# TrentMahaffey/NeuralStyleTransferV1

Measured on AMD Instinct MI355X. Metric: stylized 1080p frames/sec at 1/2/4/8 MI355X; SSIM vs CPU ref, higher is better.
Workload: dtype bf16; 1 GPU; configs[1]: TransformerNet (Johnson) forward, 1920x1080, batch 8 per GPU, bf16 MFMA / fp32 accumulate, io_preset imagenet_255, uint8 frames in/out resident in HBM; global_batch=8, parallelism=frames round-robin over 1 GPU(s), no data-path collective, ranks_per_gpu=1, step_launch=one HIP-graph replay of the captured forward per step

## Files before the change

include/nst_hip.h:

```cpp
#ifndef NST_HIP_H
#define NST_HIP_H

#include <stddef.h>
#include <stdint.h>

#ifdef __cplusplus
extern "C" {
#endif

#define NST_OK 0
#define NST_E_INVALID (-1)
#define NST_E_PARAM (-2)
#define NST_E_SHAPE (-3)
#define NST_E_HIP (-4)
#define NST_E_WORKSPACE (-5)
#define NST_E_RANGE (-6)

#define NST_ARCH_JOHNSON 0
#define NST_ARCH_NST 1
#define NST_ARCH_RECONET 2
#define NST_ARCH_RECONET_FRN 3
#define NST_ARCH_TORCH7_IN 4
#define NST_ARCH_TORCH7_BN 5

#define NST_DT_F32 0
#define NST_DT_BF16 1
#define NST_DT_F16 2
#define NST_DT_F32S 3
#define NST_DT_F16M 4

#define NST_IO_F32_NCHW 0
#define NST_IO_U8_NHWC 1

#define NST_PRESET_NONE 0
#define NST_PRESET_TANH 1
#define NST_PRESET_IMAGENET_01 2
#define NST_PRESET_IMAGENET_255 3
#define NST_PRESET_CAFFE_BGR 4
#define NST_PRESET_RAW_255 5
#define NST_PRESET_RAW_01 6
#define NST_PRESET_TORCH7 7

typedef struct nst_handle nst_handle;
typedef struct nst_lab nst_lab;

typedef struct nst_param {
  const char* name;
  const float* data;
  int64_t numel;
} nst_param;

const char* nst_last_error(void);

const char* nst_version(void);

int nst_create(int arch, const nst_param* params, int n_params, int compute_dtype, int device,
               nst_handle** out);

#define NST_KSEL_NO_WSTAT 0x1
#define NST_KSEL_NO_WPHASE 0x2
#define NST_KSEL_NO_WS2 0x4
#define NST_KSEL_NO_WS9 0x8
#define NST_KSEL_NO_KYROT 0x10
#define NST_KSEL_NO_PREPAD 0x20
#define NST_KSEL_NO_PERSISTENT 0x40
#define NST_KSEL_UNFUSED_RESIDUAL 0x80
#define NST_KSEL_NO_FOLD 0x100
#define NST_KSEL_F16M_TWO_BLOCKS 0x200
#define NST_KSEL_PAD_DECODER 0x400
#define NST_KSEL_PAD_ENCODER 0x800
#define NST_KSEL_PAD_48 0x1000
#define NST_KSEL_ALL 0x1fff
int nst_create_ex(int arch, const nst_param* params, int n_params, int compute_dtype, int device,
                  unsigned flags, nst_handle** out);
void nst_destroy(nst_handle* h);

int nst_output_hw(const nst_handle* h, int in_h, int in_w, int* out_h, int* out_w);

int nst_input_exact(const nst_handle* h, int x_fmt, int preset, int* exact);

int nst_workspace_bytes(const nst_handle* h, int n, int in_h, int in_w, size_t* out);

int nst_set_stream_split(nst_handle* h, int k);

int nst_forward(nst_handle* h, const void* x, int x_fmt, int n, int in_h, int in_w, int preset,
                void* y, int y_fmt, void* workspace, size_t workspace_bytes, void* stream);

#define NST_BUF_INPUT (-1)
#define NST_BUF_OUTPUT (-2)
typedef struct nst_op_desc {
  int kind;
  int layer;
  int src, dst;
  int in_norm;
  int in_relu;
  int res_buf;
  int res_norm;
  int res_out;
  int relu_out;
  int in_h, in_w;
  int conv_h, conv_w;
  int out_h, out_w;
  int cin_stride, cout_stride;
  int kernel_mode;
  int elem_bytes;
  int in_elem_bytes;
  int res_elem_bytes;
  int kernel_dtype;
} nst_op_desc;
int nst_num_ops(const nst_handle* h);
int nst_set_range_check(nst_handle* h, int enable);
int nst_op_describe(const nst_handle* h, int n, int in_h, int in_w, int op, nst_op_desc* out);
int nst_forward_capture(nst_handle* h, const void* x, int x_fmt, int n, int in_h, int in_w, int preset,
                        void* y, int y_fmt, void* workspace, size_t workspace_bytes, void* const* act,
                        void* const* res, void* const* stats, void* stream);

int nst_decode_resize_u8(const float* y, int n, int h, int w, int preset, uint8_t* out, int out_h,
                         int out_w, void* stream);

int nst_blend_models_u8(const float* const* ys, const int* presets, const float* weights, int m, int n,
                        int h, int w, uint8_t* out, int out_h, int out_w, void* stream);


int nst_lab_create(const uint8_t* rgb2lab, const uint8_t* lab2rgb, int device, nst_lab** out);
void nst_lab_destroy(nst_lab* lab);

int nst_lab_ema_u8(const nst_lab* lab, const uint8_t* rgb_in, uint8_t* rgb_out, int n, int h, int w,
                   int smooth_lightness, float alpha, float one_minus_alpha, int smooth_chroma,
                   float chroma_alpha, float one_minus_chroma_alpha, float* state, int first,
                   void* stream);

int nst_lab_planes_u8(const nst_lab* lab, const uint8_t* rgb_in, int n, int h, int w, int smooth_lightness,
                      int smooth_chroma, uint8_t* planes, void* stream);
int nst_lab_ema_planes(const uint8_t* planes_in, uint8_t* planes_out, int n, int h, int w, int smooth_lightness,
                       float alpha, float one_minus_alpha, int smooth_chroma, float chroma_alpha,
                       float one_minus_chroma_alpha, float* state, int first, void* stream);
int nst_lab_merge_u8(const nst_lab* lab, const uint8_t* rgb_in, const uint8_t* planes, int n, int h, int w,
                     int smooth_lightness, int smooth_chroma, uint8_t* rgb_out, void* stream);

int nst_blend_models_lab_u8(const nst_lab* lab, const uint8_t* const* frames, int m, const float* weights_rest,
                            int n_rest, float w_l, float w_ab, int n, int h, int w, uint8_t* out, void* stream);

int nst_mask_feather(const uint8_t* mask, int n, int h, int w, float sigma, float* scratch, float* alpha,
                     void* stream);

int nst_blend_u8(const uint8_t* styled, const uint8_t* orig, const float* mask, int composite_mode,
                 float blend, float one_minus_blend, uint8_t* out, int n, int h, int w,
                 void* stream);
int nst_blend_mask8_u8(const uint8_t* styled, const uint8_t* orig, const uint8_t* mask, int composite_mode, float blend,
                       float one_minus_blend, uint8_t* out, int n, int h, int w, void* stream);

int nst_profile_begin(nst_handle* h);
int nst_profile_end(nst_handle* h, int n_layers, float* total_ms, int* launches);
int nst_num_layers(const nst_handle* h);
const char* nst_layer_name(const nst_handle* h, int layer);

#define NST_GRAM_CHW 0
#define NST_GRAM_HWC 1
int nst_gram_workspace_bytes(int n, int c, int hw, size_t* out);
int nst_gram(const void* F, int dtype, int layout, int n, int c, int hw, float* G, void* workspace,
             size_t workspace_bytes, void* stream);

typedef struct nst_vgg nst_vgg;
int nst_vgg_create(const nst_param* params, int n_params, int device, nst_vgg** out);
#define NST_VGG_GENERIC_ONLY 0x1
int nst_vgg_create_ex(const nst_param* params, int n_params, int device, unsigned flags, nst_vgg** out);
void nst_vgg_destroy(nst_vgg* v);
int nst_gatys_buffer_bytes(const nst_vgg* v, int h, int w, size_t* workspace, size_t* state);
int nst_vgg_features(nst_vgg* v, const float* image, int h, int w, void* const* feats, void* workspace,
                     size_t workspace_bytes, void* stream);
int nst_gatys_targets(nst_vgg* v, const float* content, const float* style, int h, int w, void* state,
                      void* workspace, size_t workspace_bytes, void* stream);
int nst_gatys_grad(nst_vgg* v, const float* image, int h, int w, const float* style_layer_weights,
                   float content_weight, float style_weight, const void* state, float* grad, float* losses,
                   void* workspace, size_t workspace_bytes, void* stream);
int nst_gatys_grad_capture(nst_vgg* v, const float* image, int h, int w, const float* style_layer_weights,
                           float content_weight, float style_weight, const void* state, float* grad,
                           float* losses, void* workspace, size_t workspace_bytes, void* const* dz,
                           void* stream);
int nst_adam_step(float* x, const float* grad, float* m, float* v, int c, int hw, float lr, float beta1,
                  float beta2, float eps, int step, int clamp01, int grad_is_normalised, void* stream);

#define NST_SEG_RESNET101 0
#define NST_SEG_DRN_D54 1
typedef struct nst_seg nst_seg;
int nst_seg_create(const nst_param* params, int n_params, int num_classes, int compute_dtype, int device,
                   nst_seg** out);
int nst_seg_create_ex(const nst_param* params, int n_params, int num_classes, int compute_dtype, int device,
                      int backbone, nst_seg** out);
void nst_seg_destroy(nst_seg* s);
int nst_seg_num_classes(const nst_seg* s);
int nst_seg_workspace_bytes(const nst_seg* s, int n, int h, int w, size_t* out);
int nst_seg_forward(nst_seg* s, const void* x, int x_fmt, int n, int h, int w, float* logits, uint8_t* pred,
                    void* workspace, size_t workspace_bytes, void* stream);
int nst_seg_mask_scratch_bytes(int n, int h, int w, size_t* out);
int nst_seg_mask(const uint8_t* pred, int n, int h, int w, const int* target_ids, int n_ids, int close_ks,
                 int expand_px, int contract_px, int feather_px, uint8_t* mask, void* scratch, size_t scratch_bytes,
                 void* stream);

#define NST_RESIZE_PIL_LANCZOS 0
#define NST_RESIZE_CV_LINEAR 1
typedef struct nst_resize nst_resize;
int nst_resize_create(int kind, int h, int w, int oh, int ow, int device, nst_resize** out);
void nst_resize_destroy(nst_resize* r);
int nst_resize_scratch_bytes(const nst_resize* r, int n, size_t* out);
int nst_resize_u8(const nst_resize* r, const uint8_t* in, int n, int c, uint8_t* out, void* scratch,
                  size_t scratch_bytes, void* stream);

#define NST_REGION_MAX 32
#define NST_REGION_TERMS 9
#define NST_REGION_MAX_SRC 16
#define NST_RG_RECTS 0
#define NST_RG_DIAGONAL 1
#define NST_RG_VORONOI 2
#define NST_RG_RADIAL 3
#define NST_RG_WAVES 4
#define NST_RG_SPIRAL 5
#define NST_RG_CONCENTRIC 6
int nst_region_masks(int kind, int count, int n_gen, const int* ivals, const double* dvals, const double* lo,
                     const double* hi, const int* rects, const double* points, const double* divisor, int h, int w,
                     float* masks, float* scratch, void* stream);
int nst_region_feather(float* masks, int k, int h, int w, const float* taps, int ks, float* scratch, void* stream);
int nst_region_rotate(const float* in, int k, int h, int w, double angle_deg, float* out, void* stream);
int nst_region_morph_scratch_floats(int k, int h, int w, size_t* out);
int nst_region_morph(const float* in, int k, int h, int w, int mode, double frequency, double time_offset,
                     double max_disp, const double* offsets, float* out, float* scratch, size_t scratch_floats,
                     void* stream);
int nst_region_bbox(const float* masks, int k, int h, int w, float threshold, int* bbox, void* stream);
int nst_region_scratch_floats(int n, int h, int w, int crops, int with_orig, size_t* out);
int nst_region_composite_u8(const float* const* src_y, const int* src_hw, const int* src_preset, int n_src,
                            const int* n_terms, const int* term_src, const float* term_w, int n_regions,
                            const int* boxes, const uint8_t* orig, const float* masks, int n, int h, int w,
                            float* scratch, size_t scratch_floats, uint8_t* out, float* out_f32, void* stream);
int nst_region_crop_input(const uint8_t* frames, int n, int h, int w, const int* box, int out_h, int out_w, float* out,
                          void* stream);
int nst_region_resize(const float* y, int n, int h, int w, int preset, int fit_h, int fit_w, int out_h, int out_w,
                      float* out, void* stream);

int nst_gray_u8(const uint8_t* rgb, int n, int h, int w, uint8_t* gray, void* stream);
int nst_flow_scratch_floats(int h, int w, size_t* out);
int nst_flow_farneback(const uint8_t* prev, const uint8_t* next, int h, int w, double pyr_scale, int levels,
                       int winsize, int iterations, int poly_n, double poly_sigma, float* flow, float* scratch,
                       size_t scratch_floats, void* stream);
int nst_flow_dis_scratch_bytes(int n, int h, int w, size_t* out);
int nst_flow_dis(const uint8_t* prev, const uint8_t* next, int n, int h, int w, float* flow, void* scratch,
                 size_t scratch_bytes, void* stream);
int nst_flow_downscale_gray(const uint8_t* gray, int h, int w, int ds, uint8_t* out, void* stream);
int nst_resize_area_u8(const uint8_t* in, int n, int h, int w, int c, uint8_t* out, int out_h, int out_w, void* stream);
int nst_flow_upscale(const float* flow_small, int hs, int ws, int h, int w, float mul, float* flow, void* stream);
int nst_flow_fuse(const float* curr, const float* prev, const float* flow, int h, int w, float alpha,
                  float one_minus_alpha, float* out, void* stream);
int nst_motion_alpha(const float* flow, int h, int w, float motion_norm, double sigma, float max_alpha, float span,
                     float* alpha, float* scratch, void* stream);

int nst_png_bound(int h, int w, int c, size_t* out_stride);
int nst_png_workspace_bytes(int n, int h, int w, int c, size_t* out);
int nst_png_encode_u8(const uint8_t* frames, int n, int h, int w, int c, uint8_t* out, size_t out_stride,
                      int64_t* sizes, void* workspace, size_t workspace_bytes, void* stream);

#define NST_E_DATA (-7)
#define NST_JPEG_444 0
// ... 18 lines not shown
```

neuralstyletransferv1_amd/_lib.py:

```python
from __future__ import annotations

import ctypes
import os
import threading

import torch

_HERE = os.path.dirname(os.path.abspath(__file__))
LIB_PATH = os.environ.get("NST_HIP_LIB", os.path.join(_HERE, "libnst_hip.so"))

NST_OK = 0
NST_ARCH_JOHNSON, NST_ARCH_NST, NST_ARCH_RECONET, NST_ARCH_RECONET_FRN = 0, 1, 2, 3
NST_ARCH_TORCH7_IN, NST_ARCH_TORCH7_BN = 4, 5
NST_DT_F32, NST_DT_BF16, NST_DT_F16, NST_DT_F32S, NST_DT_F16M = 0, 1, 2, 3, 4
NST_KDT_SW_O32, NST_KDT_SW_O16, NST_KDT_SPLIT_O32, NST_KDT_SPLIT_O16, NST_KDT_SPLITO_O32 = 16, 17, 18, 19, 20
NST_VGG_GENERIC_ONLY = 0x1
NST_IO_F32_NCHW, NST_IO_U8_NHWC = 0, 1
NST_SEG_RESNET101, NST_SEG_DRN_D54 = 0, 1
PRESETS = {
    "none": 0,
    "tanh": 1,
    "imagenet_01": 2,
    "imagenet_255": 3,
    "caffe_bgr": 4,
    "raw_255": 5,
    "raw_01": 6,
}
NST_PRESET_TORCH7 = 7

EXPORTED_SYMBOLS = (
    "nst_last_error", "nst_version", "nst_create", "nst_destroy", "nst_output_hw",
    "nst_workspace_bytes", "nst_forward", "nst_decode_resize_u8", "nst_lab_create",
    "nst_lab_destroy", "nst_lab_ema_u8", "nst_blend_u8", "nst_gram", "nst_profile_begin",
    "nst_profile_end", "nst_num_layers", "nst_layer_name", "nst_blend_models_u8", "nst_blend_models_lab_u8",
    "nst_mask_feather", "nst_create_ex", "nst_num_ops", "nst_op_describe", "nst_forward_capture",
    "nst_gram_workspace_bytes", "nst_vgg_create", "nst_vgg_create_ex", "nst_vgg_destroy", "nst_gatys_buffer_bytes", "nst_vgg_features",
    "nst_gatys_targets", "nst_gatys_grad", "nst_adam_step", "nst_gatys_grad_capture",
    "nst_seg_create", "nst_seg_create_ex", "nst_seg_destroy", "nst_seg_num_classes", "nst_seg_workspace_bytes", "nst_seg_forward",
    "nst_seg_mask_scratch_bytes", "nst_seg_mask", "nst_resize_create", "nst_resize_destroy",
    "nst_resize_scratch_bytes", "nst_resize_u8", "nst_blend_mask8_u8",
    "nst_region_masks", "nst_region_feather", "nst_region_rotate", "nst_region_bbox", "nst_region_scratch_floats",
    "nst_region_composite_u8", "nst_region_crop_input", "nst_region_resize", "nst_region_morph",
    "nst_region_morph_scratch_floats", "nst_gray_u8", "nst_flow_scratch_floats", "nst_flow_farneback",
    "nst_flow_fuse", "nst_motion_alpha", "nst_flow_downscale_gray", "nst_flow_upscale", "nst_resize_area_u8",
    "nst_flow_dis_scratch_bytes", "nst_flow_dis", "nst_set_range_check", "nst_input_exact", "nst_set_stream_split",
    "nst_lab_planes_u8", "nst_lab_ema_planes", "nst_lab_merge_u8",
    "nst_png_bound", "nst_png_workspace_bytes", "nst_png_encode_u8",
    "nst_jpeg_probe", "nst_jpeg_entropy_decode", "nst_jpeg_workspace_bytes", "nst_jpeg_reconstruct_u8",
    "nst_jpeg_enc_bound", "nst_jpeg_enc_workspace_bytes", "nst_jpeg_encode_u8",
)
NST_E_INVALID, NST_E_SHAPE, NST_E_WORKSPACE, NST_E_DATA = -1, -3, -5, -7
NST_JPEG_444, NST_JPEG_422, NST_JPEG_420 = 0, 1, 2
NST_REGION_MAX, NST_REGION_TERMS, NST_REGION_MAX_SRC = 32, 9, 16
RG_KINDS = {"rects": 0, "diagonal": 1, "voronoi": 2, "radial": 3, "waves": 4, "spiral": 5, "concentric": 6}
NST_GRAM_CHW, NST_GRAM_HWC = 0, 1

KSEL = {
    "no_wstat": 0x1, "no_wphase": 0x2, "no_ws2": 0x4, "no_ws9": 0x8, "no_kyrot": 0x10, "no_prepad": 0x20,
    "no_persistent": 0x40, "unfused_residual": 0x80, "no_fold": 0x100, "f16m_two_blocks": 0x200,
    "pad_decoder": 0x400, "pad_encoder": 0x800, "pad_48": 0x1000,
}
NST_BUF_INPUT, NST_BUF_OUTPUT = -1, -2


class NstParam(ctypes.Structure):
    _fields_ = [("name", ctypes.c_char_p), ("data", ctypes.POINTER(ctypes.c_float)), ("numel", ctypes.c_int64)]


class NstOpDesc(ctypes.Structure):
    _fields_ = [(n, ctypes.c_int) for n in (
        "kind", "layer", "src", "dst", "in_norm", "in_relu", "res_buf", "res_norm", "res_out", "relu_out",
        "in_h", "in_w", "conv_h", "conv_w", "out_h", "out_w", "cin_stride", "cout_stride", "kernel_mode",
        "elem_bytes", "in_elem_bytes", "res_elem_bytes", "kernel_dtype")]

    def as_dict(self):
        return {n: getattr(self, n) for n, _ in self._fields_}


_lib = None
_lock = threading.Lock()


class NstError(RuntimeError):
    """Raised for any non-zero status from libnst_hip (message from nst_last_error)."""


TRUNK_KERNEL_SOURCES = ("csrc/conv_wst16.hip", "csrc/conv_ws_common.h", "csrc/conv_impl.h")


def kernel_sha(sources=TRUNK_KERNEL_SOURCES, obj: str = "conv_wstat") -> str:
    import hashlib
    import re
    h = hashlib.sha256()
    for rel in sources:
        with open(os.path.join(_HERE, rel), "rb") as f:
            h.update(f.read())
    pat = r"(HIPCC|ARCH|SLP|CXXFLAGS) |\$\(BUILD\)/" + re.escape(obj) + r"\.hip\.o: *(CXXFLAGS|SLP) "
    with open(os.path.join(_HERE, "..", "Makefile")) as f:
        h.update("".join(l for l in f if re.match(pat, l)).encode())
    return h.hexdigest()[:16]


def trunk_kernel_sha() -> str:
    return kernel_sha(TRUNK_KERNEL_SOURCES, "conv_wst16")


WS2_KERNEL_SOURCES = ("csrc/conv_ws2.hip", "csrc/conv_ws_common.h", "csrc/conv_impl.h")


def ws2_kernel_sha() -> str:
    return kernel_sha(WS2_KERNEL_SOURCES, "conv_ws2")


def lib() -> ctypes.CDLL:
    global _lib
    if _lib is not None:
        return _lib
    with _lock:
        if _lib is not None:
            return _lib
        if not os.path.exists(LIB_PATH):
            raise NstError(
                f"libnst_hip.so not found at {LIB_PATH}: build it with `make` (or __graft_entry__.build()); "
                "there is no CPU fallback")
        L = ctypes.CDLL(LIB_PATH)
        vp, i, f, sz = ctypes.c_void_p, ctypes.c_int, ctypes.c_float, ctypes.c_size_t
        L.nst_last_error.restype = ctypes.c_char_p
        L.nst_version.restype = ctypes.c_char_p
        L.nst_create.argtypes = [i, ctypes.POINTER(NstParam), i, i, i, ctypes.POINTER(vp)]
        L.nst_create_ex.argtypes = [i, ctypes.POINTER(NstParam), i, i, i, ctypes.c_uint, ctypes.POINTER(vp)]
        L.nst_num_ops.argtypes = [vp]
        L.nst_num_ops.restype = i
        L.nst_set_range_check.argtypes = [vp, i]
        L.nst_set_range_check.restype = i
        L.nst_set_stream_split.argtypes = [vp, i]
        L.nst_set_stream_split.restype = i
        L.nst_op_describe.argtypes = [vp, i, i, i, i, ctypes.POINTER(NstOpDesc)]
        L.nst_forward_capture.argtypes = [vp, vp, i, i, i, i, i, vp, i, vp, sz, ctypes.POINTER(vp), ctypes.POINTER(vp),
                                          ctypes.POINTER(vp), vp]
        L.nst_vgg_create.argtypes = [ctypes.POINTER(NstParam), i, i, ctypes.POINTER(vp)]
        L.nst_vgg_create_ex.argtypes = [ctypes.POINTER(NstParam), i, i, ctypes.c_uint, ctypes.POINTER(vp)]
        L.nst_vgg_destroy.argtypes = [vp]
        L.nst_vgg_destroy.restype = None
        L.nst_gatys_buffer_bytes.argtypes = [vp, i, i, ctypes.POINTER(sz), ctypes.POINTER(sz)]
        L.nst_vgg_features.argtypes = [vp, vp, i, i, ctypes.POINTER(vp), vp, sz, vp]
        L.nst_gatys_targets.argtypes = [vp, vp, vp, i, i, vp, vp, sz, vp]
        L.nst_gatys_grad.argtypes = [vp, vp, i, i, ctypes.POINTER(f), f, f, vp, vp, vp, vp, sz, vp]
        L.nst_gatys_grad_capture.argtypes = [vp, vp, i, i, ctypes.POINTER(f), f, f, vp, vp, vp, vp, sz,
                                             ctypes.POINTER(vp), vp]
        L.nst_gatys_grad_capture.restype = i
        L.nst_adam_step.argtypes = [vp, vp, vp, vp, i, i, f, f, f, f, i, i, i, vp]
        L.nst_destroy.argtypes = [vp]
        L.nst_destroy.restype = None
        L.nst_seg_create.argtypes = [ctypes.POINTER(NstParam), i, i, i, i, ctypes.POINTER(vp)]
        L.nst_seg_create_ex.argtypes = [ctypes.POINTER(NstParam), i, i, i, i, i, ctypes.POINTER(vp)]
        L.nst_seg_destroy.argtypes = [vp]
        L.nst_seg_destroy.restype = None
        L.nst_seg_num_classes.argtypes = [vp]
        L.nst_seg_workspace_bytes.argtypes = [vp, i, i, i, ctypes.POINTER(sz)]
        L.nst_seg_forward.argtypes = [vp, vp, i, i, i, i, vp, vp, vp, sz, vp]
        L.nst_seg_mask_scratch_bytes.argtypes = [i, i, i, ctypes.POINTER(sz)]
        L.nst_seg_mask.argtypes = [vp, i, i, i, ctypes.POINTER(i), i, i, i, i, i, vp, vp, sz, vp]
        L.nst_resize_create.argtypes = [i, i, i, i, i, i, ctypes.POINTER(vp)]
        L.nst_resize_destroy.argtypes = [vp]
        L.nst_resize_destroy.restype = None
        L.nst_resize_scratch_bytes.argtypes = [vp, i, ctypes.POINTER(sz)]
        L.nst_resize_u8.argtypes = [vp, vp, i, i, vp, vp, sz, vp]
        pi, pd, pf = ctypes.POINTER(i), ctypes.POINTER(ctypes.c_double), ctypes.POINTER(f)
        L.nst_region_masks.argtypes = [i, i, i, pi, pd, pd, pd, pi, pd, pd, i, i, vp, vp, vp]
        L.nst_region_feather.argtypes = [vp, i, i, i, pf, i, vp, vp]
        L.nst_region_rotate.argtypes = [vp, i, i, i, ctypes.c_double, vp, vp]
        L.nst_region_bbox.argtypes = [vp, i, i, i, f, vp, vp]
        dbl = ctypes.c_double
        L.nst_region_morph_scratch_floats.argtypes = [i, i, i, ctypes.POINTER(sz)]
        L.nst_region_morph.argtypes = [vp, i, i, i, i, dbl, dbl, dbl, pd, vp, vp, sz, vp]
        L.nst_region_scratch_floats.argtypes = [i, i, i, i, i, ctypes.POINTER(sz)]
        L.nst_region_composite_u8.argtypes = [ctypes.POINTER(vp), pi, pi, i, pi, pi, pf, i, pi, vp, vp, i, i, i, vp,
                                              sz, vp, vp, vp]
        L.nst_region_crop_input.argtypes = [vp, i, i, i, pi, i, i, vp, vp]
        L.nst_region_resize.argtypes = [vp, i, i, i, i, i, i, i, i, vp, vp]
        L.nst_gray_u8.argtypes = [vp, i, i, i, vp, vp]
        L.nst_flow_scratch_floats.argtypes = [i, i, ctypes.POINTER(sz)]
        L.nst_flow_farneback.argtypes = [vp, vp, i, i, dbl, i, i, i, i, dbl, vp, vp, sz, vp]
        L.nst_flow_fuse.argtypes = [vp, vp, vp, i, i, f, f, vp, vp]
        L.nst_motion_alpha.argtypes = [vp, i, i, f, dbl, f, f, vp, vp, vp]
        L.nst_flow_downscale_gray.argtypes = [vp, i, i, i, vp, vp]
        L.nst_flow_upscale.argtypes = [vp, i, i, i, i, f, vp, vp]
        L.nst_resize_area_u8.argtypes = [vp, i, i, i, i, vp, i, i, vp]
        L.nst_flow_dis_scratch_bytes.argtypes = [i, i, i, ctypes.POINTER(sz)]
        L.nst_flow_dis.argtypes = [vp, vp, i, i, i, vp, vp, sz, vp]
        for name in ("nst_gray_u8", "nst_flow_scratch_floats", "nst_flow_farneback", "nst_flow_fuse",
                     "nst_motion_alpha", "nst_flow_downscale_gray", "nst_flow_upscale", "nst_resize_area_u8",
                     "nst_flow_dis_scratch_bytes", "nst_flow_dis"):
            getattr(L, name).restype = i
        for name in ("nst_region_masks", "nst_region_feather", "nst_region_rotate", "nst_region_bbox",
                     "nst_region_morph", "nst_region_morph_scratch_floats",
                     "nst_region_scratch_floats", "nst_region_composite_u8", "nst_region_crop_input",
                     "nst_region_resize"):
            getattr(L, name).restype = i
        L.nst_output_hw.argtypes = [vp, i, i, ctypes.POINTER(i), ctypes.POINTER(i)]
        L.nst_workspace_bytes.argtypes = [vp, i, i, i, ctypes.POINTER(sz)]
        L.nst_forward.argtypes = [vp, vp, i, i, i, i, i, vp, i, vp, sz, vp]
        L.nst_decode_resize_u8.argtypes = [vp, i, i, i, i, vp, i, i, vp]
        L.nst_lab_create.argtypes = [vp, vp, i, ctypes.POINTER(vp)]
        L.nst_lab_destroy.argtypes = [vp]
        L.nst_lab_destroy.restype = None
        L.nst_lab_ema_u8.argtypes = [vp, vp, vp, i, i, i, i, f, f, i, f, f, vp, i, vp]
        L.nst_lab_planes_u8.argtypes = [vp, vp, i, i, i, i, i, vp, vp]
        L.nst_lab_ema_planes.argtypes = [vp, vp, i, i, i, i, f, f, i, f, f, vp, i, vp]
        L.nst_lab_merge_u8.argtypes = [vp, vp, vp, i, i, i, i, i, vp, vp]
        L.nst_input_exact.argtypes = [vp, i, i, ctypes.POINTER(i)]
        L.nst_png_bound.argtypes = [i, i, i, ctypes.POINTER(sz)]
        L.nst_png_workspace_bytes.argtypes = [i, i, i, i, ctypes.POINTER(sz)]
        L.nst_png_encode_u8.argtypes = [vp, i, i, i, i, vp, sz, vp, vp, sz, vp]
        psz = ctypes.POINTER(sz)
        L.nst_jpeg_probe.argtypes = [vp, sz, pi, pi, pi, pi, psz]
        L.nst_jpeg_entropy_decode.argtypes = [vp, sz, vp, sz]
        L.nst_jpeg_workspace_bytes.argtypes = [i, i, i, i, i, psz]
        L.nst_jpeg_reconstruct_u8.argtypes = [vp, sz, i, i, i, i, i, vp, vp, sz, vp]
        L.nst_jpeg_enc_bound.argtypes = [i, i, psz]
        L.nst_jpeg_enc_workspace_bytes.argtypes = [i, i, i, psz]
        L.nst_jpeg_encode_u8.argtypes = [vp, i, i, i, i, vp, sz, vp, vp, sz, vp]
        for name in ("nst_jpeg_probe", "nst_jpeg_entropy_decode", "nst_jpeg_workspace_bytes",
                     "nst_jpeg_reconstruct_u8", "nst_jpeg_enc_bound", "nst_jpeg_enc_workspace_bytes",
                     "nst_jpeg_encode_u8"):
            getattr(L, name).restype = i
# ... 46 lines not shown
```

neuralstyletransferv1_amd/csrc/conv_ws_common.h:

```cpp
#pragma once
#include "conv_impl.h"

namespace nst {

typedef unsigned int u32x2_t __attribute__((ext_vector_type(2)));
typedef unsigned int u32x4_t __attribute__((ext_vector_type(4)));

__device__ __forceinline__ f32x4_t add4(const f32x4_t& a, const f32x4_t& b) {
  f32x4_t r;
#pragma unroll
  for (int i = 0; i < 4; ++i) r[i] = a[i] + b[i];
  return r;
}
__device__ __forceinline__ void stat4(f32x4_t& s1, f32x4_t& s2, const f32x4_t& x) {
#pragma unroll
  for (int i = 0; i < 4; ++i) {
    s1[i] = s1[i] + x[i];
    s2[i] = __builtin_fmaf(x[i], x[i], s2[i]);
  }
}

template <typename T>
__device__ __forceinline__ void mfma_tied(f32x4_t& c, const uint4& a, const uint4& bop, bool first) {
  const u32x4_t av = __builtin_bit_cast(u32x4_t, a), bv = __builtin_bit_cast(u32x4_t, bop);
  if constexpr (IS_F16<T>) {
    if (first)
      asm volatile("v_mfma_f32_16x16x32_f16 %0, %1, %2, 0" : "=&v"(c) : "v"(av), "v"(bv));
    else
      asm volatile("v_mfma_f32_16x16x32_f16 %0, %1, %2, %0" : "+v"(c) : "v"(av), "v"(bv));
  } else {
    if (first)
      asm volatile("v_mfma_f32_16x16x32_bf16 %0, %1, %2, 0" : "=&v"(c) : "v"(av), "v"(bv));
    else
      asm volatile("v_mfma_f32_16x16x32_bf16 %0, %1, %2, %0" : "+v"(c) : "v"(av), "v"(bv));
  }
}

template <typename T>
__device__ __forceinline__ void mfma16x16x16_tied(f32x4_t& c, const uint2& a, const uint2& bop) {
  const u32x2_t av = __builtin_bit_cast(u32x2_t, a), bv = __builtin_bit_cast(u32x2_t, bop);
  if constexpr (IS_F16<T>)
    asm volatile("v_mfma_f32_16x16x16_f16 %0, %1, %2, %0" : "+v"(c) : "v"(av), "v"(bv));
  else
    asm volatile("v_mfma_f32_16x16x16_bf16 %0, %1, %2, %0" : "+v"(c) : "v"(av), "v"(bv));
}

template <typename T>
__device__ __forceinline__ void mfma_tied_c(f32x4_t& c, const uint4& a, const uint4& bop, bool first, const f32x4_t& cinit) {
  const u32x4_t av = __builtin_bit_cast(u32x4_t, a), bv = __builtin_bit_cast(u32x4_t, bop);
  if constexpr (IS_F16<T>) {
    if (first)
      asm volatile("v_mfma_f32_16x16x32_f16 %0, %1, %2, %3" : "=&v"(c) : "v"(av), "v"(bv), "v"(cinit));
    else
      asm volatile("v_mfma_f32_16x16x32_f16 %0, %1, %2, %0" : "+v"(c) : "v"(av), "v"(bv));
  } else {
    if (first)
      asm volatile("v_mfma_f32_16x16x32_bf16 %0, %1, %2, %3" : "=&v"(c) : "v"(av), "v"(bv), "v"(cinit));
    else
      asm volatile("v_mfma_f32_16x16x32_bf16 %0, %1, %2, %0" : "+v"(c) : "v"(av), "v"(bv));
  }
}

constexpr int ST_AUX = 2;

enum WsFill { WF_NORM = 0, WF_RAW = 1, WF_RES = 2, WF_RESRN = 3 };

template <int N>
__device__ __forceinline__ void vm_wait() {
  asm volatile("s_waitcnt vmcnt(%0)" ::"n"(N) : "memory");
}
__device__ __forceinline__ void lds_barrier() {
  asm volatile("s_waitcnt lgkmcnt(0)\n\ts_barrier" ::: "memory");
}

__device__ __forceinline__ void dma16(const __amdgpu_buffer_rsrc_t& rs, uint32_t voff, uint32_t lds, int soff) {
  uint32_t keep;
  asm volatile(
      "s_mov_b32 %0, m0\n\ts_mov_b32 m0, %2\n\ts_nop 0\n\tbuffer_load_dwordx4 %1, %3, %4 offen lds\n\ts_mov_b32 m0, %0"
      : "=&s"(keep)
      : "v"(voff), "s"(lds), "s"(rs), "s"(soff)
      : "memory");
}

}
```

neuralstyletransferv1_amd/csrc/conv_wst16.hip:

```cpp
#include <algorithm>
#include <cstdlib>
#include <cstring>

#include "conv_ws_common.h"

namespace nst {

constexpr uint32_t OOB = 0xFFFFFF00u;
#ifndef NST_W32_ST
#define NST_W32_ST 0
#endif

#ifndef NST_WST32_STAMP
#define NST_WST32_STAMP 0
#endif
#ifndef NST_W32_MIN
#define NST_W32_MIN 0
#endif
#if NST_WST32_STAMP
constexpr int STAMP_IT = 1, STAMP_PT = 16;
__device__ long long g_w16_stamp[256 * 4 * STAMP_IT * STAMP_PT];
#endif

template <int TH, int FILL>
struct W16Cfg {
  static constexpr bool RES = FILL == WF_RES;
  static constexpr int NW = 4, NT = 256;
  static constexpr int TW = 32;
  static constexpr int CINP = 128;
  static constexpr int LH = TH + 2, LW = TW + 2;
  static constexpr int NENT = LH * LW;
  static constexpr int EB = 288;
  static constexpr int NKS = 72;
  static constexpr int NA = 64;
  static constexpr int NV = NKS - NA;
  static constexpr int NIT = (NENT + 63) / 64;
  static constexpr int LASTN = NENT - 64 * (NIT - 1);
  static constexpr int NFMAX = RES ? 8 : 16;
  static constexpr int DPU = RES ? 2 : 1;
  static constexpr int SLOTB = DPU * 1024;
  static constexpr int MAPB = ((LH + LW) * 4 + 15) / 16 * 16;
  static constexpr int MAP_OFF = NENT * EB;
  static constexpr int NORM_OFF = MAP_OFF + 2 * MAPB;
  static constexpr int NORM_TAB = NFMAX * CINP * 8;
  static constexpr int BIAS_OFF = NORM_OFF + NORM_TAB;
  static constexpr int DUMMY_OFF = BIAS_OFF + CINP * 4;
  static constexpr int STG_OFF = DUMMY_OFF + 64 * 16;
  static constexpr int LDS = STG_OFF + NIT * NW * SLOTB;
  static constexpr int SST = TH * TW * 4 / NT;
  static constexpr int EPI = 2 * TH + 1;
  static_assert(LDS <= 160 * 1024, "LDS budget");
  static_assert(TH * TW * 4 % NT == 0 && TW == 32, "pixel-quarter stores");
};

template <typename T>
__device__ __forceinline__ void mfma16_a(f32x4_t& c, const u32x4_t& a, const u32x4_t& b, bool first) {
  if constexpr (IS_F16<T>) {
    if (first) asm volatile("v_mfma_f32_16x16x32_f16 %0, %1, %2, 0" : "=&v"(c) : "a"(a), "v"(b));
    else asm volatile("v_mfma_f32_16x16x32_f16 %0, %1, %2, %0" : "+v"(c) : "a"(a), "v"(b));
  } else {
    if (first) asm volatile("v_mfma_f32_16x16x32_bf16 %0, %1, %2, 0" : "=&v"(c) : "a"(a), "v"(b));
    else asm volatile("v_mfma_f32_16x16x32_bf16 %0, %1, %2, %0" : "+v"(c) : "a"(a), "v"(b));
  }
}
template <typename T>
__device__ __forceinline__ void mfma16_v(f32x4_t& c, const u32x4_t& a, const u32x4_t& b, bool first) {
  if constexpr (IS_F16<T>) {
    if (first) asm volatile("v_mfma_f32_16x16x32_f16 %0, %1, %2, 0" : "=&v"(c) : "v"(a), "v"(b));
    else asm volatile("v_mfma_f32_16x16x32_f16 %0, %1, %2, %0" : "+v"(c) : "v"(a), "v"(b));
  } else {
    if (first) asm volatile("v_mfma_f32_16x16x32_bf16 %0, %1, %2, 0" : "=&v"(c) : "v"(a), "v"(b));
    else asm volatile("v_mfma_f32_16x16x32_bf16 %0, %1, %2, %0" : "+v"(c) : "v"(a), "v"(b));
  }
}

template <typename T, int TH, int FILL, bool ZPAD, bool XO>
__global__ __launch_bounds__(256) void wst16_kernel(ConvParams p) {
  using C = W16Cfg<TH, FILL>;
  constexpr bool RES = C::RES;
  static_assert(!XO || FILL == WF_NORM, "x_0 export is a normalising fill");
  constexpr bool SOUT = RES || XO;
  __shared__ __attribute__((aligned(16))) char smem[C::LDS];
  const int tid = threadIdx.x, lane = tid & 63;
  const int wv = __builtin_amdgcn_readfirstlane(tid >> 6);
  const int g4 = lane >> 4, p16 = lane & 15;

  struct Work {
    int n, tile, ty0, tx0;
  };
  const int ntile = p.tiles_x * p.tiles_y;
  const int nfr = p.n_work / ntile;
  auto decode = [&](int wi) {
    Work r;
    r.n = wi / ntile;
    r.tile = wi - r.n * ntile;
    const int ty = r.tile / p.tiles_x;
    r.ty0 = ty * TH;
    r.tx0 = (r.tile - ty * p.tiles_x) * C::TW;
    return r;
  };
  const int G = (int)gridDim.x, b = (int)blockIdx.x;
  const int w0 = (G % 8 == 0) ? (b % 8) * (G / 8) + b / 8 : b;
  if (w0 >= p.n_work) return;

  u32x4_t wa[C::NA];
  u32x4_t wvr[C::NV];
  {
    const u32x4_t* wsrc = (const u32x4_t*)p.wpk + (size_t)wv * C::NKS * 64 + lane;
#pragma unroll
    for (int s = 0; s < C::NA; ++s) asm volatile("global_load_dwordx4 %0, %1, off" : "=a"(wa[s]) : "v"(wsrc + s * 64) : "memory");
#pragma unroll
    for (int s = 0; s < C::NV; ++s) wvr[s] = wsrc[(C::NA + s) * 64];
  }
  float* norm_y = (float*)(smem + C::NORM_OFF);
  if (FILL != WF_RAW) {
    for (int t = tid; t < nfr * C::CINP; t += C::NT) {
      const int f = t / C::CINP, c = t - f * C::CINP;
      const int o = (f * 16 + (c >> 3)) * 16 + 4 * ((c & 7) >> 1) + (c & 1);
      const float2 v = p.in_norm[(size_t)f * p.cs + c];
      norm_y[o] = v.x;
      norm_y[o + 2] = v.y;
    }
  }
  if (tid < C::CINP) ((float*)(smem + C::BIAS_OFF))[tid] = p.bias[tid];

  const uint32_t fb = (uint32_t)p.hs * p.ws * p.cs * 2;
  const uint32_t ob = (uint32_t)p.oh * p.ow * p.cout_stride * 2;
  auto launch_rsrc = [&](const void* base, uint32_t frame) {
    return __builtin_amdgcn_make_buffer_rsrc((void*)base, (short)0, (int)(frame * (uint32_t)nfr), 0x00020000);
  };
  auto build_maps = [&](const Work& wk, int slot) {
    int* rowmap = (int*)(smem + C::MAP_OFF + slot * C::MAPB);
    int* colmap = rowmap + C::LH;
    const int vy0 = wk.ty0 - p.pad, vx0 = wk.tx0 - p.pad;
    const int pix = p.cs * 2;
    auto axis = [&](int v, int L) { return ZPAD ? map_axis(v, L, p.axis_mode, p.pre) : reflect_idx(v, L); };
    static_assert(C::LH + C::LW <= 64, "one wave builds the maps");
    const int t = tid;
    if (t < C::LH) {
      const int sy = axis(vy0 + t, p.hs);
      rowmap[t] = sy < 0 ? -1 : sy * p.ws * pix;
    } else if (t < C::LH + C::LW) {
      const int sx = axis(vx0 + t - C::LH, p.ws);
      colmap[t - C::LH] = sx < 0 ? -1 : sx * pix;
    }
  };
  constexpr int IT_STRIDE = 64;
  auto item_entry = [&](int k) { return 64 * k + lane; };
  auto item_chunk = [&](int R) { return 4 * R + wv; };
  struct Src {
    uint32_t voff[C::NIT];
    uint32_t pad;
  };
  auto sources = [&](const Work& wk, int slot) {
    const int* rowmap = (const int*)(smem + C::MAP_OFF + slot * C::MAPB);
    const int* colmap = rowmap + C::LH;
    Src s;
    s.pad = 0;
#pragma unroll
    for (int k = 0; k < C::NIT; ++k) {
      const int e0 = item_entry(k);
      const bool valid = k < C::NIT - 1 || lane < C::LASTN;
      const int e = valid ? e0 : 0;
      const int ly = e / C::LW, lx = e - ly * C::LW;
      const int ro = rowmap[ly], co = colmap[lx];
      const bool in = valid && ro >= 0 && co >= 0;
      s.voff[k] = in ? (uint32_t)(ro + co) + (uint32_t)wk.n * fb : OOB;
      if (valid && !in) s.pad |= 1u << k;
    }
    return s;
  };
  const uint32_t stg = (uint32_t)(uintptr_t)(smem + C::STG_OFF) + wv * C::SLOTB;
  const __amdgpu_buffer_rsrc_t rs_in = launch_rsrc(p.in, fb);
  const __amdgpu_buffer_rsrc_t rs_r = launch_rsrc(RES ? p.res_r : p.in, fb);
  auto request = [&](int k, int R, uint32_t voff) {
    const uint32_t lds = stg + k * C::NW * C::SLOTB;
    const int soff = (4 * R + wv) * 16;
    dma16(rs_in, voff, lds, soff);
    if constexpr (RES) dma16(rs_r, voff, lds + 1024, soff);
  };
  struct Staged {
    uint4 y, r;
  };
  auto stage_read = [&](int k) {
    const char* sp = smem + C::STG_OFF + (k * C::NW + wv) * C::SLOTB + lane * 16;
    Staged st;
    st.y = *(const uint4*)sp;
    st.r = RES ? *(const uint4*)(sp + 1024) : make_uint4(0u, 0u, 0u, 0u);
    return st;
  };
  auto consume = [&](int n, int k, int R, uint32_t padbits, const Staged& st) {
    const int ch = item_chunk(R);
    const uint4 y = st.y, rr = st.r;
    const float4* ny = (const float4*)(norm_y + (n * 16 + ch) * 16);
    const uint32_t w[4] = {y.x, y.y, y.z, y.w};
    uint32_t o[4];
    if constexpr (RES) {
      const uint32_t w2[4] = {rr.x, rr.y, rr.z, rr.w};
#pragma unroll
      for (int j = 0; j < 4; ++j) {
        const float4 nn = ny[j];
        const float a = lo16<T>(w[j]) * nn.x + nn.z;
        const float bb = hi16<T>(w[j]) * nn.y + nn.w;
        o[j] = pack16<T>(lo16<T>(w2[j]) + a, hi16<T>(w2[j]) + bb);
      }
    } else if constexpr (FILL == WF_RAW) {
#pragma unroll
      for (int j = 0; j < 4; ++j) o[j] = w[j];
    } else {
#pragma unroll
      for (int j = 0; j < 4; ++j) {
        const float4 nn = ny[j];
        const float a = __builtin_fmaf(lo16<T>(w[j]), nn.x, nn.z);
        const float bb = __builtin_fmaf(hi16<T>(w[j]), nn.y, nn.w);
        const i16x2_t r = __builtin_bit_cast(i16x2_t, pack16<T>(a, bb));
        o[j] = __builtin_bit_cast(uint32_t, __builtin_elementwise_max(r, (i16x2_t){0, 0}));
      }
    }
    const bool pad = ZPAD && ((padbits >> k) & 1u);
    const u32x4_t v = {pad ? 0u : o[0], pad ? 0u : o[1], pad ? 0u : o[2], pad ? 0u : o[3]};
    const bool valid = k < C::NIT - 1 || lane < C::LASTN;
    int eb = item_entry(0) * C::EB + ch * 16;
    asm volatile("" : "+v"(eb));
    *(u32x4_t*)(smem + (valid ? eb + k * IT_STRIDE * C::EB : C::DUMMY_OFF + lane * 16)) = v;
  };
  constexpr int KIN = (C::NIT - 1) * C::DPU + (SOUT ? C::SST : 0);
  constexpr int KEP = KIN + C::EPI;

  typedef f32x4_t Acc[TH][2][2];
  const int lbase = p16 * C::EB + g4 * 16;
  constexpr int NRD = 2 * C::LH;
  constexpr int PRD = 3 * NRD;
  auto bread = [&](int i) -> u32x4_t {
    const int q = i / PRD, rem = i - q * PRD;
    const int dx = rem / NRD, y = (rem % NRD) >> 1, hx = rem & 1;
    return *(const u32x4_t*)(smem + lbase + (y * C::LW + dx + 16 * hx) * C::EB + 4 * q * 16);
  };
  auto kloop = [&](Acc& acc, auto&& filler, auto&& bound) {
    constexpr int NI = 4 * PRD, D = SOUT ? 2 : 3;
    u32x4_t ring[D];
#pragma unroll
    for (int i = 0; i < D; ++i) ring[i] = bread(i);
    int slot = 0;
#pragma unroll
    for (int i = 0; i < NI; ++i) {
      const int q = i / PRD, rem = i - q * PRD;
      const int dx = rem / NRD, y = (rem % NRD) >> 1, hx = rem & 1;
      if (rem == 0) slot = 0;
      const u32x4_t bcur = ring[i % D];
      if (i + D < NI) ring[i % D] = bread(i + D);
#pragma unroll
      for (int dy = 0; dy < 3; ++dy) {
        const int r = y - dy;
        if (r < 0 || r >= TH) continue;
#pragma unroll
        for (int bb = 0; bb < 2; ++bb) {
          const int s = 2 * (q * 9 + 3 * dy + dx) + bb;
          const bool first = q == 0 && dx == 0 && dy == 0;
          if (s < C::NA) mfma16_a<T>(acc[r][bb][hx], wa[s], bcur, first);
          else mfma16_v<T>(acc[r][bb][hx], wvr[s - C::NA], bcur, first);
          filler(q, slot);
          ++slot;
          __builtin_amdgcn_sched_barrier(0);
        }
      }
      if (rem == PRD - 1) {
        lds_barrier();
        bound(q);
      }
      __builtin_amdgcn_sched_barrier(0);
    }
  };

  const float* biasl = (const float*)(smem + C::BIAS_OFF) + 32 * wv + 4 * g4;
  auto epilogue = [&](const Work& wk, Acc& acc) {
    asm volatile("s_nop 7\n\ts_nop 7\n\ts_nop 7" ::: "memory");
    const __amdgpu_buffer_rsrc_t ors = launch_rsrc(p.out, ob);
    const uint32_t row_bytes = (uint32_t)p.ow * p.cout_stride * 2;
    const int spx = wk.tx0 + ((g4 & 1) ? 16 : 0) + p16;
    const uint32_t soff = (uint32_t)wk.n * ob + (uint32_t)(((wk.ty0 * p.ow + spx) * p.cout_stride + 32 * wv + 8 * (g4 >> 1)) * 2);
    const bool sok = spx < p.ow;
    const bool ok0 = wk.tx0 + p16 < p.ow, ok1 = wk.tx0 + 16 + p16 < p.ow;
    const f32x4_t bias0 = *(const f32x4_t*)(biasl), bias1 = *(const f32x4_t*)(biasl + 16);
    f32x4_t s1[2], s2[2];
    auto rows = [&](auto all_valid) {
#pragma unroll
      for (int r = 0; r < TH; ++r) {
        const bool rv = decltype(all_valid)::value || wk.ty0 + r < p.oh;
#pragma unroll
        for (int bb = 0; bb < 2; ++bb) {
          const f32x4_t v0 = acc[r][bb][0] + (bb ? bias1 : bias0), v1 = acc[r][bb][1] + (bb ? bias1 : bias0);
          const auto sx = __builtin_amdgcn_permlane16_swap(pack16<T>(v0[0], v0[1]), pack16<T>(v1[0], v1[1]), false, false);
          const auto sy = __builtin_amdgcn_permlane16_swap(pack16<T>(v0[2], v0[3]), pack16<T>(v1[2], v1[3]), false, false);
          const u32x4_t pk = {sx[0], sy[0], sx[1], sy[1]};
          __builtin_amdgcn_raw_buffer_store_b128(pk, ors, (rv && sok) ? soff + r * row_bytes + 32 * bb : OOB, 0, NST_W32_ST);
          const f32x4_t x0 = (decltype(all_valid)::value || (rv && ok0)) ? v0 : (f32x4_t){0.f, 0.f, 0.f, 0.f};
          const f32x4_t x1 = (decltype(all_valid)::value || (rv && ok1)) ? v1 : (f32x4_t){0.f, 0.f, 0.f, 0.f};
          if (r == 0) {
            s1[bb] = x0 + x1;
            s2[bb] = __builtin_elementwise_fma(x1, x1, x0 * x0);
          } else {
            s1[bb] = (s1[bb] + x0) + x1;
            s2[bb] = __builtin_elementwise_fma(x1, x1, __builtin_elementwise_fma(x0, x0, s2[bb]));
          }
        }
      }
    };
    if (wk.ty0 + TH <= p.oh && wk.tx0 + C::TW <= p.ow) rows(std::true_type{});
    else rows(std::false_type{});
    const float v[16] = {s1[0][0], s2[0][0], s1[0][1], s2[0][1], s1[0][2], s2[0][2], s1[0][3], s2[0][3],
                         s1[1][0], s2[1][0], s1[1][1], s2[1][1], s1[1][2], s2[1][2], s1[1][3], s2[1][3]};
    float a8[8], a4[4], a2[2], a1[1];
    rs_step<8, 0x140>(v, a8, p16 >= 8);
    rs_step<4, 0x141>(a8, a4, (p16 & 4) != 0);
    rs_step<2, 0x1b>(a4, a2, (p16 & 2) != 0);
    rs_step<1, 0xb1>(a2, a1, (p16 & 1) != 0);
    const int idx = (p16 >= 8 ? 8 : 0) + ((p16 & 4) ? 4 : 0) + ((p16 & 2) ? 2 : 0) + (p16 & 1);
    const int co = 32 * wv + 16 * (idx >> 3) + 4 * g4 + ((idx >> 1) & 3);
    const __amdgpu_buffer_rsrc_t prs = __builtin_amdgcn_make_buffer_rsrc(
        (void*)(p.partial + ((size_t)wk.n * ntile + wk.tile) * p.cout_stride * 2), (short)0, p.cout_stride * 8, 0x00020000);
    __builtin_amdgcn_raw_buffer_store_b32(__float_as_uint(a1[0]), prs, (uint32_t)((co * 2 + (idx & 1)) * 4), 0, 0);
  };

  Work cur = decode(w0);
  int wn = w0 + G;
  const int last = p.n_work - 1;
  build_maps(cur, 0);
  build_maps(decode(min(wn, last)), 1);
  asm volatile("s_waitcnt vmcnt(0)" ::: "memory");
  __syncthreads();
  uint32_t pad3;
  {
    const Src s0 = sources(cur, 0);
    pad3 = s0.pad;
#pragma unroll
    for (int k = 0; k < C::NIT; ++k) request(k, 0, s0.voff[k]);
#pragma unroll
    for (int R = 0; R < 3; ++R) {
      vm_wait<0>();
#pragma unroll
      for (int k = 0; k < C::NIT; ++k) {
        consume(cur.n, k, R, s0.pad, stage_read(k));
        request(k, R + 1, s0.voff[k]);
      }
    }
  }
  vm_wait<0>();
  __syncthreads();
  constexpr int SLOTS_PER_ITEM = 48;
  static_assert(SLOTS_PER_ITEM * C::NIT <= 9 * TH * 4 && C::SST <= C::NIT, "micro-step slots");
  Acc acc;
  Staged sy;
  float4 n0;
  float tl, th;
  uint32_t o4[4];
  int mro = 0, mco = 0;
  bool padk = false;
  bool mok = false;
  uint32_t rvoff = OOB;
  u32x4_t sv;
#if NST_WST32_STAMP
  unsigned st_acc[7] = {0, 0, 0, 0, 0, 0, 0};
  unsigned st_prev = (unsigned)__builtin_amdgcn_s_memtime();
#endif
  auto stamp = [&](int it, int pt) {
#if NST_WST32_STAMP
    const unsigned t = (unsigned)__builtin_amdgcn_s_memtime();
    st_acc[pt == 0 ? 5 : pt - 1] += t - st_prev;
    st_prev = t;
    if (pt == 0) st_acc[6] += 1;
#endif
  };
  for (int it = 0;; ++it) {
    stamp(it, 0);
    const bool more = wn < p.n_work;
    const Work nxt = more ? decode(wn) : cur;
    const Work nxt2 = decode(min(wn + G, last));
    const int cs = it & 1, ns = cs ^ 1;
    kloop(
        acc,
        [&](int q, int slot) {
          const int k = slot / SLOTS_PER_ITEM, o = slot - k * SLOTS_PER_ITEM;
          if (k >= C::NIT) return;
          const int R = q == 0 ? 3 : q - 1;
          const int n = q == 0 ? cur.n : nxt.n;
          const int ch = item_chunk(R);
          const float4* ny = (const float4*)(norm_y + (n * 16 + ch) * 16);
          auto pair_step = [&](int j, int st) {
            const uint32_t wy = j == 0 ? sy.y.x : j == 1 ? sy.y.y : j == 2 ? sy.y.z : sy.y.w;
            if constexpr (RES) {
              const uint32_t wr = j == 0 ? sy.r.x : j == 1 ? sy.r.y : j == 2 ? sy.r.z : sy.r.w;
              if (st == 0) tl = lo16<T>(wy) * n0.x;
              else if (st == 1) tl = lo16<T>(wr) + (tl + n0.z);
              else if (st == 2) th = hi16<T>(wy) * n0.y;
              else o4[j] = pack16<T>(tl, hi16<T>(wr) + (th + n0.w));
            } else if constexpr (FILL == WF_RAW) {
              if (st == 3) o4[j] = wy;
            } else {
              if (st == 0) tl = __builtin_fmaf(lo16<T>(wy), n0.x, n0.z);
              else if (st == 1) th = __builtin_fmaf(hi16<T>(wy), n0.y, n0.w);
              else if (st == 3) {
                const i16x2_t r = __builtin_bit_cast(i16x2_t, pack16<T>(tl, th));
                o4[j] = __builtin_bit_cast(uint32_t, __builtin_elementwise_max(r, (i16x2_t){0, 0}));
              }
            }
          };
          if (o == 0) {
            if (q == 0) vm_wait<KEP>(); else vm_wait<KIN>();
            sy = stage_read(k);
          } else if (o >= 4 && o < 36 && (o - 4) % 8 == 0) {
            if (FILL != WF_RAW) n0 = ny[(o - 4) / 8];
          } else if (o >= 8 && o < 36 && (o - 4) % 8 >= 4) {
            pair_step((o - 4) / 8, (o - 4) % 8 - 4);
          } else if (o == 2) {
            const int* rowmap = (const int*)(smem + C::MAP_OFF + ns * C::MAPB);
            const bool valid = k < C::NIT - 1 || lane < C::LASTN;
            const int e = valid ? item_entry(k) : 0;
            const int ly = e / C::LW, lx = e - ly * C::LW;
            mro = rowmap[ly];
            mco = rowmap[C::LH + lx];
          } else if (o == 36) {
            const bool valid = k < C::NIT - 1 || lane < C::LASTN;
            mok = valid && mro >= 0 && mco >= 0;
            if (ZPAD) {
              padk = valid && !mok;
              if (q == 3) pad3 = (pad3 & ~(1u << k)) | (padk ? 1u << k : 0u);
            }
          } else if (o == 37) {
            rvoff = mok ? (uint32_t)(mro + mco) + (uint32_t)nxt.n * fb : OOB;
          } else if (o == 38) {
            const bool pad = ZPAD && (q == 0 ? ((pad3 >> k) & 1u) != 0 : padk);
            const u32x4_t v = {pad ? 0u : o4[0], pad ? 0u : o4[1], pad ? 0u : o4[2], pad ? 0u : o4[3]};
            const bool valid = k < C::NIT - 1 || lane < C::LASTN;
            int eb = item_entry(0) * C::EB + ch * 16;
            asm volatile("" : "+v"(eb));
            *(u32x4_t*)(smem + (valid ? eb + k * IT_STRIDE * C::EB : C::DUMMY_OFF + lane * 16)) = v;
          } else if (o == 40) {
            request(k, q, rvoff);
          }
          if (q == 1 && k == 0 && o == 44) build_maps(nxt2, cs);
          if (SOUT && k < C::SST && o == 42) {
            const int cl = lane >> 4, x16 = ((lane & 15) - cl) & 15;
            const int P = 16 * (C::SST * wv + k) + x16;
            sv = *(const u32x4_t*)(smem + (((P >> 5) + 1) * C::LW + (P & 31) + 1) * C::EB + (4 * q + cl) * 16);
          }
          if (SOUT && k < C::SST && o == 47) {
            const int cl = lane >> 4, x16 = ((lane & 15) - cl) & 15;
            const int P = 16 * (C::SST * wv + k) + x16;
            const int c = 4 * q + cl, oy = cur.ty0 + (P >> 5), ox = cur.tx0 + (P & 31);
            const bool ok = oy < p.oh && ox < p.ow;
            __builtin_amdgcn_raw_buffer_store_b128(sv, launch_rsrc(p.res_out, fb),
                                                   ok ? (uint32_t)cur.n * fb + (uint32_t)(((oy * p.ws + ox) * p.cs + c * 8) * 2) : OOB,
                                                   0, NST_W32_ST);
          }
        },
        [&](int q) { stamp(it, 1 + q); });
    epilogue(cur, acc);
    stamp(it, 5);
    if (!more) break;
    cur = nxt;
    wn += G;
  }
  vm_wait<0>();
#if NST_WST32_STAMP
  if (lane == 0 && b < 256)
    for (int i = 0; i < 7; ++i) g_w16_stamp[(b * 4 + wv) * STAMP_PT + i] = st_acc[i];
#endif
}

template <typename T, int TH, bool RES>
struct Wst16Inst {
  using C = W16Cfg<TH, RES ? WF_RES : WF_NORM>;
  static int cus() {
    static const int v = [] {
      int dev = 0, c = 0;
      if (hipGetDevice(&dev) != hipSuccess || hipDeviceGetAttribute(&c, hipDeviceAttributeMultiprocessorCount, dev) != hipSuccess)
        c = 256;
      return c;
    }();
    return v;
  }
  template <int FILL, bool ZPAD, bool XO = false>
  static void go(const ConvParams& p, int nb, hipStream_t st) {
    hipLaunchKernelGGL((wst16_kernel<T, TH, FILL, ZPAD, XO>), dim3(nb), dim3(C::NT), 0, st, p);
  }
  static void launch(const ConvParams& p0, dim3 grid, hipStream_t st) {
    const int ntile = (int)grid.x, n = (int)grid.y;
    const size_t fin = (size_t)p0.hs * p0.ws * p0.cs * 2, fout = (size_t)p0.oh * p0.ow * p0.cout_stride * 2;
    const int fmax = (int)std::min<size_t>(C::NFMAX, (size_t)OOB / std::max(fin, fout));
    if (fmax < 1) return;
    for (int f0 = 0; f0 < n; f0 += fmax) {
      const int nf = std::min(fmax, n - f0);
      ConvParams p = p0;
      p.in = (const char*)p0.in + f0 * fin;
      p.out = (char*)p0.out + f0 * fout;
      if (p0.res_r) p.res_r = (const char*)p0.res_r + f0 * fin;
      if (p0.res_out) p.res_out = (char*)p0.res_out + f0 * fin;
      if (p0.in_norm) p.in_norm = p0.in_norm + (size_t)f0 * p0.cs;
      p.partial = p0.partial + (size_t)f0 * ntile * p0.cout_stride * 2;
      p.n_work = nf * ntile;
      const int nb = std::min(p.n_work, cus());
      const bool zp = p.axis_mode != AX_REFLECT;
#if NST_W32_MIN
      if (zp) return;
      if constexpr (RES) go<WF_RES, false>(p, nb, st);
      else if (p.res_out != nullptr) go<WF_NORM, false, true>(p, nb, st);
      else go<WF_NORM, false>(p, nb, st);
#else
      if constexpr (RES) {
        zp ? go<WF_RES, true>(p, nb, st) : go<WF_RES, false>(p, nb, st);
      } else {
        if (p.in_norm != nullptr && p.res_out != nullptr)
          zp ? go<WF_NORM, true, true>(p, nb, st) : go<WF_NORM, false, true>(p, nb, st);
        else if (p.in_norm != nullptr)
          zp ? go<WF_NORM, true>(p, nb, st) : go<WF_NORM, false>(p, nb, st);
        else
          zp ? go<WF_RAW, true>(p, nb, st) : go<WF_RAW, false>(p, nb, st);
      }
#endif
    }
  }
  static ConvKernelInfo info() {
    ConvKernelInfo k;
    std::memset(&k, 0, sizeof(k));
    k.dtype = dtype_code<T>();
    k.mode = MODE_WSTAT;
    k.ks = 3; k.stride = 1; k.cinp = C::CINP; k.bn = 128; k.th = TH; k.tw = C::TW; k.wm = C::NW; k.wn = 2;
    k.in_kind = IN_ACT; k.out_kind = OUT_ACT;
    k.cpc = 8; k.nch = 16; k.lds_bytes = C::LDS;
    k.wbytes = C::NW * C::NKS * 1024;
    k.persistent = 1;
    k.part_rows = 1;
    k.res = RES ? 1 : 0;
    k.launch = &launch;
    return k;
  }
};

#ifndef NST_WST16_TH
#define NST_WST16_TH 8
#endif
#ifndef NST_W16_PART
#define NST_W16_PART -1
#endif
#define W16_KERNELS(X, T)                                                                                     \
  X(T, WF_NORM, false, false) X(T, WF_NORM, false, true) X(T, WF_NORM, true, false) X(T, WF_NORM, true, true) \
  X(T, WF_RAW, false, false) X(T, WF_RAW, true, false) X(T, WF_RES, false, false) X(T, WF_RES, true, false)
#define W16_EXTERN(T, F, Z, X_) extern template __global__ void wst16_kernel<T, NST_WST16_TH, F, Z, X_>(ConvParams);
#define W16_INST(T, F, Z, X_) template __global__ void wst16_kernel<T, NST_WST16_TH, F, Z, X_>(ConvParams);
#if NST_W16_PART >= 0 && NST_W16_PART < 8
#define W16_T_ __bf16
#if NST_W16_PART >= 4
#undef W16_T_
#define W16_T_ _Float16
#endif
#if NST_W16_PART % 4 == 0
W16_INST(W16_T_, WF_NORM, false, false)
W16_INST(W16_T_, WF_NORM, false, true)
#elif NST_W16_PART % 4 == 1
W16_INST(W16_T_, WF_NORM, true, false)
W16_INST(W16_T_, WF_NORM, true, true)
#elif NST_W16_PART % 4 == 2
W16_INST(W16_T_, WF_RAW, false, false)
W16_INST(W16_T_, WF_RAW, true, false)
#else
W16_INST(W16_T_, WF_RES, false, false)
W16_INST(W16_T_, WF_RES, true, false)
#endif
#else
#if NST_W16_PART == 8
W16_KERNELS(W16_EXTERN, __bf16)
W16_KERNELS(W16_EXTERN, _Float16)
#endif
const ConvKernelInfo* conv_table_wst16(int* count) {
  static const ConvKernelInfo table[] = {
      Wst16Inst<__bf16, NST_WST16_TH, false>::info(),
      Wst16Inst<__bf16, NST_WST16_TH, true>::info(),
#if !NST_W32_MIN
      Wst16Inst<_Float16, NST_WST16_TH, false>::info(),
      Wst16Inst<_Float16, NST_WST16_TH, true>::info(),
#endif
  };
  const char* env = std::getenv("NST_WST16");
  *count = (env != nullptr && env[0] == '0') ? 0 : (int)(sizeof(table) / sizeof(table[0]));
  return table;
}
#endif

}

#if NST_WST32_STAMP
extern "C" int nst_debug_w16_stamps(long long* host, int n) {
  const int cap = 256 * 4 * nst::STAMP_IT * nst::STAMP_PT;
  if (n > cap) n = cap;
  return hipMemcpyFromSymbol(host, HIP_SYMBOL(nst::g_w16_stamp), (size_t)n * 8, 0, hipMemcpyDeviceToHost) == hipSuccess ? n : -1;
}
#endif
```

neuralstyletransferv1_amd/csrc/nst_api.cpp:

```cpp
#include <hip/hip_runtime.h>

#include <cmath>
#include <cstdio>
#include <algorithm>
#include <cstring>
#include <cstdlib>
#include <map>
#include <string>
#include <vector>

#include "nst_hip.h"
#include "nst_internal.h"
#include "post_common.h"

namespace nst {

static thread_local std::string g_last_error;
void set_error(const std::string& msg) { g_last_error = msg; }

const ConvKernelInfo* conv_table_bf16(int* count);
const ConvKernelInfo* conv_table_f16(int* count);
const ConvKernelInfo* conv_table_bf16_wl(int* count);
const ConvKernelInfo* conv_table_f32(int* count);
const ConvKernelInfo* conv_table_f32s(int* count);
// ... 79 lines not shown
  int shave = 0;
};

static int round_up(int v, int a) { return (v + a - 1) / a * a; }
static bool is_reconet(int arch) { return arch == NST_ARCH_RECONET || arch == NST_ARCH_RECONET_FRN; }
static bool is_torch7(int arch) { return arch == NST_ARCH_TORCH7_IN || arch == NST_ARCH_TORCH7_BN; }

static void build_program(int arch, bool fuse_res, bool x0_export, std::vector<LayerDef>& L, std::vector<Op>& P,
                          int split_blocks = 0) {
  L.clear();
  P.clear();
  auto conv = [&](int layer, int src, int dst, int in_norm) {
    P.push_back(Op{OP_CONV, layer, src, dst, in_norm, 0, 0, 0, 0});
  };
  auto convres = [&](int layer, int y, int y_norm, int r_buf, int r_norm, int res_out, int relu_out, int dst) {
    Op o{OP_CONV, layer, y, dst, y_norm, r_buf, r_norm, r_norm >= 0 ? 1 : 0, relu_out};
    o.res_buf = r_buf;
    o.res_out = res_out;
    P.push_back(o);
  };
  auto resadd = [&](int layer, int y, int dst, int r_buf, int r_norm, int relu_out) {
    P.push_back(Op{OP_RESADD, layer, y, dst, -1, r_buf, r_norm, r_norm >= 0 ? 1 : 0, relu_out});
  };
  if (arch == NST_ARCH_JOHNSON) {
    L.push_back({"conv1.conv2d", "in1", 3, 32, 9, 1, AX_REFLECT, 4, 0, false});
    L.push_back({"conv2.conv2d", "in2", 32, 64, 3, 2, AX_REFLECT, 1, 0, false});
    L.push_back({"conv3.conv2d", "in3", 64, 128, 3, 2, AX_REFLECT, 1, 0, false});
    for (int r = 1; r <= 5; ++r) {
      const std::string p = "res" + std::to_string(r);
      L.push_back({p + ".conv1.conv2d", p + ".in1", 128, 128, 3, 1, AX_REFLECT, 1, 0, false});
      L.push_back({p + ".conv2.conv2d", p + ".in2", 128, 128, 3, 1, AX_REFLECT, 1, 0, false});
    }
    L.push_back({"deconv1.conv2d", "in4", 128, 64, 3, 1, AX_REFLECT_UP2, 1, 0, false});
    L.push_back({"deconv2.conv2d", "in5", 64, 32, 3, 1, AX_REFLECT_UP2, 1, 0, false});
    L.push_back({"deconv3.conv2d", "", 32, 3, 9, 1, AX_REFLECT, 4, 0, false});
  } else if (arch == NST_ARCH_NST) {
    L.push_back({"down1.conv", "down1.norm", 3, 32, 9, 1, AX_ZERO_PREREFLECT, 4, 40, false});
    L.push_back({"down2.conv", "down2.norm", 32, 64, 3, 2, AX_ZERO, 1, 0, false});
    L.push_back({"down3.conv", "down3.norm", 64, 128, 3, 2, AX_ZERO, 1, 0, false});
    for (int r = 1; r <= 5; ++r) {
      const std::string p = "res" + std::to_string(r);
      L.push_back({p + ".conv1", p + ".norm1", 128, 128, 3, 1, AX_ZERO, 1, 0, false});
      L.push_back({p + ".conv2", p + ".norm2", 128, 128, 3, 1, AX_ZERO, 1, 0, false});
    }
    L.push_back({"up1.conv", "up1.norm", 128, 64, 3, 1, AX_ZINSERT, 1, 0, true});
    L.push_back({"up2.conv", "up2.norm", 64, 32, 3, 1, AX_ZINSERT, 1, 0, true});
    L.push_back({"final", "", 32, 3, 9, 1, AX_ZERO, 4, 0, false});
  } else if (is_torch7(arch)) {
    L.push_back({"down1.conv", "down1.norm", 3, 32, 9, 1, AX_ZERO_PREREFLECT, 4, 40, false});
    L.push_back({"down2.conv", "down2.norm", 32, 64, 3, 2, AX_ZERO, 1, 0, false});
    L.push_back({"down3.conv", "down3.norm", 64, 128, 3, 2, AX_ZERO, 1, 0, false});
    for (int r = 1; r <= 5; ++r) {
      const std::string p = "res" + std::to_string(r);
      L.push_back({p + ".conv1", p + ".norm1", 128, 128, 3, 1, AX_ZERO, 0, 0, false});
      L.push_back({p + ".conv2", p + ".norm2", 128, 128, 3, 1, AX_ZERO, 0, 0, false});
    }
    L.push_back({"up1.conv", "up1.norm", 128, 64, 3, 1, AX_ZINSERT, 1, 0, true});
    L.push_back({"up2.conv", "up2.norm", 64, 32, 3, 1, AX_ZINSERT, 1, 0, true});
    L.push_back({"final", "", 32, 3, 9, 1, AX_ZERO, 4, 0, false});
  } else {
    L.push_back({"encoder.layers.0.layers.0.layers.1", "encoder.layers.0.layers.1", 3, 48, 9, 1, AX_REFLECT, 4, 0, false});
    L.push_back({"encoder.layers.1.layers.0.layers.1", "encoder.layers.1.layers.1", 48, 96, 3, 2, AX_REFLECT, 1, 0, false});
    L.push_back({"encoder.layers.2.layers.0.layers.1", "encoder.layers.2.layers.1", 96, 192, 3, 2, AX_REFLECT, 1, 0, false});
    for (int r = 3; r <= 6; ++r) {
      const std::string p = "encoder.layers." + std::to_string(r) + ".branch.";
      L.push_back({p + "0.layers.0.layers.1", p + "0.layers.1", 192, 192, 3, 1, AX_REFLECT, 1, 0, false});
      L.push_back({p + "1.layers.0.layers.1", p + "1.layers.1", 192, 192, 3, 1, AX_REFLECT, 1, 0, false});
    }
    L.push_back({"decoder.layers.1.layers.0.layers.1", "decoder.layers.1.layers.1", 192, 96, 3, 1, AX_REFLECT_UP2, 1, 0, false});
    L.push_back({"decoder.layers.3.layers.0.layers.1", "decoder.layers.3.layers.1", 96, 48, 3, 1, AX_REFLECT_UP2, 1, 0, false});
    L.push_back({"decoder.layers.4.layers.0.layers.1", "", 48, 3, 9, 1, AX_REFLECT, 4, 0, false});
  }
  const int nres = is_reconet(arch) ? 4 : 5;
  const int relu_out = is_reconet(arch) ? 1 : 0;
  const int u1 = 3 + 2 * nres, u2 = u1 + 1, fin = u1 + 2;
  conv(0, B_IMG, B_A, -1);
  conv(1, B_A, B_B, 0);
  conv(2, B_B, B_C, 1);
  if (is_torch7(arch)) {
    int xbuf = B_C, xnorm = 2;
    for (int r = 0; r < nres; ++r) {
      const int l1 = 3 + 2 * r, l2 = 4 + 2 * r;
      conv(l1, xbuf, B_D, xnorm);
      conv(l2, B_D, B_E, l1);
      const int xout = (r & 1) ? B_G : B_F;
      resadd(l2, B_E, xout, xbuf, xnorm, 0);
      P.back().shave = 2;
      xbuf = xout;
      xnorm = -1;
    }
    conv(u1, xbuf, B_A, -1);
  } else if (split_blocks > 0) {
    conv(3, B_C, B_D, 2);
    conv(4, B_D, B_E, 3);
    if (split_blocks >= 2) {
      resadd(4, B_E, B_F, B_C, 2, relu_out);
      P.back().out_esz = 4;
      conv(5, B_F, B_D, -1);
      conv(6, B_D, B_E, 5);
      resadd(6, B_E, B_G, B_F, -1, relu_out);
    } else {
      resadd(4, B_E, B_G, B_C, 2, relu_out);
    }
    P.back().out_esz = 2;
    int xbuf = B_G;
    for (int r = split_blocks; r < nres; ++r) {
      const int l1 = 3 + 2 * r, l2 = 4 + 2 * r;
      if (r == split_blocks) {
        conv(l1, B_G, B_D, -1);
      } else {
        const int xout = xbuf == B_F ? B_G : B_F;
        convres(l1, B_E, l2 - 2, xbuf, -1, xout, relu_out, B_D);
        xbuf = xout;
      }
      conv(l2, B_D, B_E, l1);
    }
    convres(u1, B_E, u1 - 1, xbuf, -1, -1, relu_out, B_A);
  } else if (!fuse_res) {
    for (int r = 0; r < nres; ++r) {
      const int l1 = 3 + 2 * r, l2 = 4 + 2 * r;
      conv(l1, B_C, B_D, r == 0 ? 2 : -1);
      conv(l2, B_D, B_E, l1);
      resadd(l2, B_E, B_C, B_C, r == 0 ? 2 : -1, relu_out);
    }
    conv(u1, B_C, B_A, -1);
  } else {
    int xbuf = x0_export ? B_F : B_C, xnorm = x0_export ? -1 : 2;
    for (int r = 0; r < nres; ++r) {
      const int l1 = 3 + 2 * r, l2 = 4 + 2 * r;
      if (r == 0) {
        conv(l1, B_C, B_D, 2);
        if (x0_export) P.back().res_out = B_F;
      } else {
        const int xout = ((r & 1) != 0) != x0_export ? B_F : B_G;
        convres(l1, B_E, l2 - 2, xbuf, xnorm, xout, relu_out, B_D);
        xbuf = xout;
        xnorm = -1;
      }
      conv(l2, B_D, B_E, l1);
    }
    convres(u1, B_E, u1 - 1, xbuf, xnorm, -1, relu_out, B_A);
  }
  conv(u2, B_A, B_B, u1);
  conv(fin, B_B, B_OUT, u2);
}

}

using namespace nst;

struct nst_handle {
  int arch, dtype, device;
  int* range_flag = nullptr;
  std::vector<Layer> layers;
  std::vector<Op> prog;
  bool profiling = false;
  struct Rec { int layer; hipEvent_t a, b; };
  std::vector<Rec> recs;
  int split = 1;
  float t7_mul = 0.f;
  hipStream_t sub[NST_MAX_STREAM_SPLIT] = {};
  hipEvent_t fork = nullptr, join[NST_MAX_STREAM_SPLIT] = {};
};

struct nst_lab {
  int device;
  uint32_t* rgb2lab = nullptr;
  uint32_t* lab2rgb = nullptr;
};

namespace {


int upload_weights(int dtype, const std::vector<float>& pk, void** dst);

int phase_taps(bool convT, int a, int t, int* ks_out) {
  if (convT) {
    if (a == 0) { if (t == 0) { ks_out[0] = 1; return 1; } return 0; }
    ks_out[0] = t == 0 ? 2 : 0;
    return 1;
  }
  if (a == 0) {
    if (t == 0) { ks_out[0] = 0; return 1; }
    ks_out[0] = 1; ks_out[1] = 2; return 2;
  }
  if (t == 0) { ks_out[0] = 0; ks_out[1] = 1; return 2; }
  ks_out[0] = 2;
  return 1;
}

double phase_weight(const LayerDef& d, const float* W, int co, int ci, int ph, int tap) {
  int ky[2], kx[2];
  const int ny = phase_taps(d.convT, ph >> 1, tap >> 1, ky), nx = phase_taps(d.convT, ph & 1, tap & 1, kx);
  double sum = 0.0;
  for (int yy = 0; yy < ny; ++yy)
    for (int xx = 0; xx < nx; ++xx)
      sum += d.convT ? (double)W[(((size_t)ci * d.cout + co) * d.ks + ky[yy]) * d.ks + kx[xx]]
                     : (double)W[(((size_t)co * d.cin + ci) * d.ks + ky[yy]) * d.ks + kx[xx]];
  return sum;
}

std::vector<float> pack_weights(const ConvKernelInfo& k, const LayerDef& d, const float* W, int coutp,
                                bool reverse_channels = false) {
  const int ncblk = coutp / k.bn;
  const size_t per_frag = 64 * (size_t)k.cpc;
  std::vector<float> out((size_t)ncblk * k.nstep_pack * k.nsubt * per_frag, 0.f);
  auto w_at = [&](int co, int ci, int dy, int dx) -> double {
    if (d.convT)
      return W[(((size_t)ci * d.cout + co) * d.ks + (d.ks - 1 - dy)) * d.ks + (d.ks - 1 - dx)];
    return W[(((size_t)co * d.cin + ci) * d.ks + dy) * d.ks + dx];
  };
  for (int cb = 0; cb < ncblk; ++cb)
    for (int s = 0; s < k.nstep; ++s)
      for (int tg = 0; tg < k.nsubt; ++tg)
        for (int lane = 0; lane < 64; ++lane) {
          const int q = lane & 15, g = lane >> 4;
          const int taps = k.nchunk / k.nch;
          const int sl = k.korder ? (s % taps) * (k.nch / 4) + s / taps : s;
          const int i = 4 * sl + g;
          float* dst = &out[((((size_t)cb * k.nstep_pack + s) * k.nsubt + tg) * 64 + lane) * k.cpc];
          if (i >= k.nchunk) continue;
          const int tap = i / k.nch, c = i % k.nch;
          if (k.mode == MODE_PHASE) {
            const int ph = tg / k.nsub, t = tg % k.nsub;
            const int co = cb * k.bn + 4 * k.nsub * (q >> 2) + 4 * t + (q & 3);
            if (co >= d.cout) continue;
            for (int j = 0; j < k.cpc; ++j) {
              const int ci = c * k.cpc + j;
              if (ci < d.cin) dst[j] = (float)phase_weight(d, W, co, ci, ph, tap);
            }
          } else if (k.mode == MODE_XSHIFT) {
            if (q >= 15) continue;
            const int sft = q / 3, ch = q % 3;
            const int co = reverse_channels ? 2 - ch : ch;
            const int dy = tap / k.kp, u = tap % k.kp, dx = u - sft;
            if (dx < 0 || dx >= d.ks || co >= d.cout) continue;
            for (int j = 0; j < k.cpc; ++j) {
              const int ci = c * k.cpc + j;
              if (ci < d.cin) dst[j] = (float)w_at(co, ci, dy, dx);
            }
          } else {
            const int wn = tg / k.nsub, t = tg % k.nsub;
            const int co = cb * k.bn + wn * k.nsub * 16 + 4 * k.nsub * (q >> 2) + 4 * t + (q & 3);
            if (co >= d.cout) continue;
            const int dy = tap / k.kp, dxp = tap % k.kp;
            for (int j = 0; j < k.cpc; ++j) {
              int dx, ci;
              if (k.pair) { dx = 2 * dxp + (j >= 4 ? 1 : 0); ci = j & 3; }
              else { dx = dxp; ci = c * k.cpc + j; }
              if (dx < d.ks && ci < d.cin) dst[j] = (float)w_at(co, ci, dy, dx);
            }
          }
        }
  return out;
}

std::vector<float> split_weight_frags(const ConvKernelInfo& k, const std::vector<float>& pk) {
  std::vector<float> out(pk.size() * 2);
  size_t o = 0;
  auto put = [&](const float* f, size_t n, bool lo) {
    for (size_t i = 0; i < n; ++i) {
      const float hi = f16_to_f32(f32_to_f16_rne(f[i]));
      out[o++] = lo ? f[i] - hi : hi;
    }
  };
  if (k.mode == MODE_WS9) {
    const size_t fm = 64 * 8, fk = 64 * 4;
    const float* k8 = pk.data() + 18 * fm;
    for (int mh = 0; mh < 2; ++mh) {
      for (int ky = 0; ky < 9; ++ky)
        for (int hl = 0; hl < 2; ++hl) put(pk.data() + (2 * ky + mh) * fm, fm, hl == 1);
      for (int j = 0; j < 3; ++j)
        for (int hl = 0; hl < 2; ++hl) put(k8 + (2 * j + mh) * fk, fk, hl == 1);
    }
  } else {
    const size_t per_cg = pk.size() / (k.bn / 16);
    for (int cg = 0; cg < k.bn / 16; ++cg)
      for (int hl = 0; hl < 2; ++hl) put(pk.data() + cg * per_cg, per_cg, hl == 1);
  }
  return out;
}

std::vector<float> pack_kyrot_weights(const ConvKernelInfo& k, const LayerDef& d, const float* W) {
  const bool split = k.dtype == NST_DT_F32S;
  const int cpb = split ? 8 : 16, kc_n = (k.cinp_k ? k.cinp_k : k.cinp) / cpb, nblk = 9 * kc_n;
  std::vector<float> out((size_t)k.wbytes / 2, 0.f);
  for (int pp = 0; pp < 2; ++pp)
    for (int ky = 0; ky < 9; ++ky)
      for (int kx = 0; kx < 9; ++kx)
        for (int kc = 0; kc < kc_n; ++kc)
          for (int hh = 0; hh < 2; ++hh)
            for (int c = 0; c < 3; ++c)
              for (int j = 0; j < 4; ++j) {
                const int ci = split ? kc * 8 + 4 * hh + j : kc * 16 + 8 * hh + 4 * pp + j;
                if (ci >= d.cin) continue;
                const size_t row = (((size_t)pp * nblk + kx * kc_n + kc) * 2 + hh) * 27 + 3 * ky + c;
                const float w = W[(((size_t)c * d.cin + ci) * d.ks + ky) * d.ks + kx];
                const float hi = f16_to_f32(f32_to_f16_rne(w));
                out[row * 4 + j] = split ? (pp == 0 ? hi : w - hi) : w;
              }
  return out;
}

std::vector<float> pack_wstat_weights(const LayerDef& d, const float* W) {
  std::vector<float> out((size_t)8 * 36 * 64 * 8, 0.f);
  for (int w = 0; w < 8; ++w)
// ... 48 lines not shown
  std::vector<float> out((size_t)8 * nstep * ns * 64 * 8, 0.f);
  for (int w = 0; w < 8; ++w)
    for (int s = 0; s < nstep; ++s)
      for (int t = 0; t < ns; ++t)
        for (int l = 0; l < 64; ++l) {
          const int q = s / 4, tap = s % 4;
          const int co = (w >> 2) * (bn / 2) + 16 * t + (l & 15);
          for (int i = 0; i < 8; ++i) {
            const int ci = 32 * q + 8 * (l >> 4) + i;
            if (co < d.cout && ci < d.cin)
              out[((((size_t)w * nstep + s) * ns + t) * 64 + l) * 8 + i] = (float)phase_weight(d, W, co, ci, w & 3, tap);
          }
        }
  return out;
}

std::vector<float> pack_ws2_weights(const ConvKernelInfo& k, const LayerDef& d, const float* W) {
  const int ncg = k.bn / 16, nstep = 9 * ((k.cinp_k ? k.cinp_k : k.cinp) / 32);
  std::vector<float> out((size_t)ncg * nstep * 64 * 8, 0.f);
  for (int cg = 0; cg < ncg; ++cg)
    for (int s = 0; s < nstep; ++s)
      for (int l = 0; l < 64; ++l) {
        const int q = s / 9, t = s % 9, dy = t / 3, dx = t % 3;
        const int co = 16 * cg + (l & 15);
        for (int i = 0; i < 8; ++i) {
          const int ci = 32 * q + 8 * (l >> 4) + i;
          if (co < d.cout && ci < d.cin)
            out[(((size_t)cg * nstep + s) * 64 + l) * 8 + i] = W[(((size_t)co * d.cin + ci) * d.ks + dy) * d.ks + dx];
        }
      }
  return out;
}

std::vector<float> pack_ws9_weights(const ConvKernelInfo& k, const LayerDef& d, const float* W) {
  const int bnk = k.bn_k ? k.bn_k : k.bn;
  if (bnk > 32) {
    std::vector<float> all;
    for (int h = 0; h < bnk / 32; ++h) {
      ConvKernelInfo kh = k;
      kh.bn = 32;
      kh.bn_k = 0;
      LayerDef dh = d;
      dh.cout = std::max(0, std::min(32, d.cout - 32 * h));
      const std::vector<float> part =
          dh.cout > 0 ? pack_ws9_weights(kh, dh, W + (size_t)32 * h * d.cin * 81) : pack_ws9_weights(kh, dh, W);
      all.insert(all.end(), part.begin(), part.end());
    }
    return all;
  }
  const bool pair = k.korder == 1;
  std::vector<float> out((size_t)18 * 64 * 8 + (pair ? 4 * 64 * 8 : 6 * 64 * 4), 0.f);
  auto w = [&](int co, int ci, int ky, int kx) -> float {
    return (co < d.cout && ci < d.cin && ky < 9) ? W[(((size_t)co * d.cin + ci) * 9 + ky) * 9 + kx] : 0.f;
  };
  for (int ky = 0; ky < 9; ++ky)
    for (int m = 0; m < 2; ++m)
      for (int l = 0; l < 64; ++l)
        for (int i = 0; i < 8; ++i)
          out[(((size_t)ky * 2 + m) * 64 + l) * 8 + i] = w(16 * m + (l & 15), i & 3, ky, 2 * (l >> 4) + (i >> 2));
  float* k8 = out.data() + (size_t)18 * 64 * 8;
  if (pair) {
    for (int m = 0; m < 2; ++m)
      for (int l = 0; l < 64; ++l)
        for (int i = 0; i < 8; ++i) {
          const int co = 16 * m + (l & 15);
          k8[(((size_t)0 * 2 + m) * 64 + l) * 8 + i] = w(co, i & 3, 2 * (l >> 4) + (i >> 2), 8);
          k8[(((size_t)1 * 2 + m) * 64 + l) * 8 + i] = ((l >> 4) == 0 && i < 4) ? w(co, i & 3, 8, 8) : 0.f;
        }
  } else {
    for (int j = 0; j < 3; ++j)
      for (int m = 0; m < 2; ++m)
        for (int l = 0; l < 64; ++l)
          for (int i = 0; i < 4; ++i) k8[(((size_t)j * 2 + m) * 64 + l) * 4 + i] = w(16 * m + (l & 15), i, 4 * j + (l >> 4), 8);
  }
  return out;
}

std::vector<float> xshift_bias(const float* b, bool reverse_channels) {
  std::vector<float> r(16, 0.f);
  for (int q = 0; q < 15; ++q) r[q] = b[reverse_channels ? 2 - q % 3 : q % 3];
  return r;
}

int upload(const void* host, size_t bytes, void** dev) {
  NST_HIP_CHECK(hipMalloc(dev, bytes));
  NST_HIP_CHECK(hipMemcpy(*dev, host, bytes, hipMemcpyHostToDevice));
  return NST_OK;
}
int upload_weights(int dtype, const std::vector<float>& pk, void** dst) {
  if (dtype == NST_DT_F32) return upload(pk.data(), pk.size() * 4, dst);
  if (dtype == NST_DT_F32S) {
    const size_t nfrag = pk.size() / 256;
    std::vector<uint16_t> pb(nfrag * 2 * 64 * 8, 0);
    for (size_t f = 0; f < nfrag; ++f)
      for (int lane = 0; lane < 64; ++lane)
        for (int j = 0; j < 4; ++j) {
          const float w = pk[(f * 64 + lane) * 4 + j];
          const uint16_t hi = f32_to_f16_rne(w);
          const uint16_t lo = f32_to_f16_rne(w - f16_to_f32(hi));
          pb[((f * 2) * 64 + lane) * 8 + j] = hi;
          pb[((f * 2) * 64 + lane) * 8 + 4 + j] = hi;
          pb[((f * 2 + 1) * 64 + lane) * 8 + j] = lo;
        }
    return upload(pb.data(), pb.size() * 2, dst);
  }
  std::vector<uint16_t> pb(pk.size());
  for (size_t i = 0; i < pk.size(); ++i) pb[i] = dtype == NST_DT_F16 ? f32_to_f16_rne(pk[i]) : f32_to_bf16_rne(pk[i]);
  return upload(pb.data(), pb.size() * 2, dst);
}

struct DeviceGuard {
  int prev = -1;
  bool changed = false;
  explicit DeviceGuard(int dev) {
    if (hipGetDevice(&prev) == hipSuccess && prev != dev) {
      changed = hipSetDevice(dev) == hipSuccess;
    }
  }
  ~DeviceGuard() {
    if (changed) (void)hipSetDevice(prev);
  }
};

int conv_out_dim(const LayerDef& d, int L) {
  switch (d.axis_mode) {
    case AX_REFLECT_UP2: return (2 * L + 2 * d.pad - d.ks) / d.stride + 1;
    case AX_ZERO_PREREFLECT: return (L + 2 * d.pre + 2 * d.pad - d.ks) / d.stride + 1;
    case AX_ZINSERT: return 2 * L;
    default: return (L + 2 * d.pad - d.ks) / d.stride + 1;
  }
}

bool layer_input_ok(const LayerDef& d, int L) {
  if (d.axis_mode == AX_REFLECT) return L > d.pad;
  if (d.axis_mode == AX_REFLECT_UP2) return 2 * L > d.pad;
  if (d.axis_mode == AX_ZERO_PREREFLECT) return L > d.pre;
  if (d.axis_mode == AX_ZERO) return L + 2 * d.pad >= d.ks;
  return L >= 1;
}

struct Plan {
  bool ok = false;
  std::string err;
  std::vector<int> ih, iw, oh, ow, ch, cw;
  std::vector<int> in_esz, out_esz, res_esz;
  size_t buf_bytes[NBUF] = {0, 0, 0, 0, 0, 0, 0};
  size_t partial_floats = 0;
  int out_h = 0, out_w = 0;
  size_t ws_bytes = 0;
  size_t seg_bytes = 0;
  size_t off_buf[NBUF], off_partial, off_seg, off_stats, off_pre = 0;
  size_t pre_bytes = 0;
  size_t off_tail = 0, tail_bytes = 0;
};

size_t align256(size_t v) { return (v + 255) / 256 * 256; }

void tile_grid(const ConvKernelInfo& k, int sh, int sw, int oh, int ow, int* tx, int* ty) {
  if (k.mode == MODE_PHASE || k.mode == MODE_WPHASE) {
    *tx = (sw + k.tw - 1) / k.tw;
    *ty = (sh + k.th - 1) / k.th;
  } else {
    *tx = (ow + k.tw - 1) / k.tw;
    *ty = (oh + k.th - 1) / k.th;
  }
}

Plan make_plan(const nst_handle* h, int n, int H, int W) {
  Plan P;
  int bh[NBUF], bw[NBUF], be[NBUF];
  for (int b = 0; b < NBUF; ++b) be[b] = (int)act_elem_bytes(h->dtype);
  const size_t nops = h->prog.size();
  P.ih.resize(nops); P.iw.resize(nops); P.oh.resize(nops); P.ow.resize(nops); P.ch.resize(nops); P.cw.resize(nops);
  P.in_esz.assign(nops, 0); P.out_esz.assign(nops, 0); P.res_esz.assign(nops, 0);
  for (size_t i = 0; i < nops; ++i) {
    const Op& op = h->prog[i];
    const Layer& Ly = h->layers[op.layer];
    if (op.kind == OP_CONV) {
      const int sh = op.src == B_IMG ? H : bh[op.src];
      const int sw = op.src == B_IMG ? W : bw[op.src];
      if (!layer_input_ok(Ly.d, sh) || !layer_input_ok(Ly.d, sw)) {
        P.err = "input " + std::to_string(H) + "x" + std::to_string(W) + " too small for layer " + Ly.d.conv +
                " (padding must be smaller than its input " + std::to_string(sh) + "x" + std::to_string(sw) + ")";
        return P;
      }
      const int ch = conv_out_dim(Ly.d, sh), cw = conv_out_dim(Ly.d, sw);
      const int iesz = op.src == B_IMG ? 2 : be[op.src];
      if (op.src != B_IMG && iesz != Ly.in_esz) {
        P.err = "internal: layer " + Ly.d.conv + " reads " + std::to_string(iesz) + "-byte activations, its kernel " +
                std::to_string(Ly.in_esz);
        return P;
      }
      P.in_esz[i] = iesz;
      P.out_esz[i] = Ly.out_esz;
      const size_t fin = (size_t)sh * sw * (op.src == B_IMG ? 4 : Ly.cinp) * iesz;
      const size_t fout = (size_t)ch * cw * Ly.coutp * Ly.out_esz;
      if (std::max(fin, fout) >= (size_t)0x7FFFFF00u) {
        P.err = "input " + std::to_string(H) + "x" + std::to_string(W) + " too large: layer " + Ly.d.conv +
                " needs " + std::to_string(std::max(fin, fout)) + " bytes per frame (limit 2^31)";
        return P;
      }
      if (op.src == B_IMG && (Ly.prepad || Ly.k_u8fold)) {
        const int wpad = cw + Ly.d.ks - 1;
        const size_t pb = ((size_t)n * (ch + Ly.d.ks - 1) + prepad_slack_rows(wpad)) * wpad * 8;
        if (pb > P.pre_bytes) P.pre_bytes = pb;
      }
      if (op.res_buf >= 0) P.res_esz[i] = be[op.res_buf];
      if (op.res_out >= 0) {
        bh[op.res_out] = sh; bw[op.res_out] = sw; be[op.res_out] = iesz;
        P.res_esz[i] = iesz;
        const size_t rb = (size_t)n * sh * sw * Ly.cinp * iesz;
        if (rb > P.buf_bytes[op.res_out]) P.buf_bytes[op.res_out] = rb;
      }
      P.ih[i] = sh; P.iw[i] = sw; P.ch[i] = ch; P.cw[i] = cw;
      if (op.dst == B_OUT) {
        if (h->arch == NST_ARCH_NST) {
          P.oh[i] = H; P.ow[i] = W;
        } else {
          P.oh[i] = ch; P.ow[i] = cw;
        }
        P.out_h = P.oh[i]; P.out_w = P.ow[i];
      } else {
        P.oh[i] = ch; P.ow[i] = cw;
        bh[op.dst] = ch; bw[op.dst] = cw; be[op.dst] = Ly.out_esz;
        const size_t bytes = (size_t)n * ch * cw * Ly.coutp * Ly.out_esz;
        if (bytes > P.buf_bytes[op.dst]) P.buf_bytes[op.dst] = bytes;
        for (const ConvKernelInfo* kk : {Ly.k_main, Ly.k_u8fold}) {
          if (!kk) continue;
          int ttx, tty;
          tile_grid(*kk, sh, sw, ch, cw, &ttx, &tty);
          const size_t pf = (size_t)n * ttx * tty * kk->part_rows * Ly.coutp * 2;
          if (pf > P.partial_floats) P.partial_floats = pf;
        }
        const size_t sb = (size_t)n * IN_MAX_SEGMENTS * Ly.coutp * 16;
        if (sb > P.seg_bytes) P.seg_bytes = sb;
      }
    } else {
      if (bh[op.r_buf] != bh[op.src] + 2 * op.shave || bw[op.r_buf] != bw[op.src] + 2 * op.shave) {
        P.err = "internal: residual join of a " + std::to_string(bh[op.src]) + "x" + std::to_string(bw[op.src]) +
                " map with a " + std::to_string(bh[op.r_buf]) + "x" + std::to_string(bw[op.r_buf]) + " stream";
        return P;
      }
      P.ih[i] = P.oh[i] = bh[op.src];
      P.iw[i] = P.ow[i] = bw[op.src];
      P.in_esz[i] = be[op.src];
      P.res_esz[i] = be[op.r_buf];
      P.out_esz[i] = op.out_esz ? op.out_esz : be[op.src];
      be[op.dst] = P.out_esz[i];
      const size_t rb = (size_t)n * bh[op.src] * bw[op.src] * Ly.coutp * P.out_esz[i];
      if (rb > P.buf_bytes[op.dst]) P.buf_bytes[op.dst] = rb;
      bh[op.dst] = bh[op.src];
      bw[op.dst] = bw[op.src];
    }
  }
  size_t off = 0;
  for (int b = 0; b < NBUF; ++b) { P.off_buf[b] = off; off += align256(P.buf_bytes[b]); }
  P.off_partial = off;
  off += align256(P.partial_floats * 4);
  P.off_seg = off;
  off += align256(P.seg_bytes);
  P.off_pre = off;
  off += align256(P.pre_bytes);
  if (is_torch7(h->arch)) P.tail_bytes = (size_t)n * 3 * P.out_h * P.out_w * 4;
  P.off_tail = off;
  off += align256(P.tail_bytes);
  P.off_stats = off;
  for (const Layer& Ly : h->layers) off += align256((size_t)n * Ly.coutp * 8);
  P.ws_bytes = off;
  P.ok = true;
  return P;
}

struct PresetConsts {
  float ea[3], eb[3], ed[3];
  int eperm[3];
  float dp[3], dq[3], dr[3], ds[3];
  int dperm[3];
};

bool preset_consts(int preset, PresetConsts& c) {
  const float mean[3] = {0.485f, 0.456f, 0.406f}, stdv[3] = {0.229f, 0.224f, 0.225f};
  const float caffe[3] = {103.939f, 116.779f, 123.68f};
  for (int i = 0; i < 3; ++i) {
    c.ea[i] = 1.f; c.eb[i] = 0.f; c.ed[i] = 1.f; c.eperm[i] = i;
    c.dp[i] = 0.f; c.dq[i] = 1.f; c.dr[i] = 1.f; c.ds[i] = 0.f; c.dperm[i] = i;
  }
  switch (preset) {
    case NST_PRESET_NONE: case NST_PRESET_RAW_01: return true;
    case NST_PRESET_TANH:
      for (int i = 0; i < 3; ++i) { c.ea[i] = 2.f; c.eb[i] = 1.f; c.dp[i] = 1.f; c.dq[i] = 0.5f; }
      return true;
    case NST_PRESET_IMAGENET_01:
      for (int i = 0; i < 3; ++i) { c.eb[i] = mean[i]; c.ed[i] = stdv[i]; c.dq[i] = stdv[i]; c.ds[i] = mean[i]; }
      return true;
    case NST_PRESET_IMAGENET_255:
      for (int i = 0; i < 3; ++i) {
        volatile float m = mean[i] * 255.0f, s = stdv[i] * 255.0f;
        c.ea[i] = 255.f; c.eb[i] = m; c.ed[i] = s; c.dr[i] = 255.f;
      }
      return true;
    case NST_PRESET_CAFFE_BGR:
    case NST_PRESET_TORCH7:
      for (int i = 0; i < 3; ++i) {
        c.ea[i] = 255.f; c.eb[i] = caffe[i]; c.eperm[i] = 2 - i; c.dr[i] = 255.f; c.dperm[i] = 2 - i;
      }
      return true;
    case NST_PRESET_RAW_255:
      for (int i = 0; i < 3; ++i) { c.ea[i] = 255.f; c.dr[i] = 255.f; }
      return true;
    default: return false;
  }
}

bool fold_first_layer(const LayerDef& d, const float* W, const float* b, int preset, std::vector<float>& Wf,
                      std::vector<float>& bf) {
  PresetConsts pc;
  if (preset == NST_PRESET_NONE || !preset_consts(preset, pc)) return false;
  if (d.axis_mode != AX_REFLECT)
    for (int c = 0; c < 3; ++c)
      if (pc.eb[c] != 0.f) return false;
  const int kk = d.ks * d.ks;
  Wf.assign(W, W + (size_t)d.cout * d.cin * kk);
  bf.assign(b, b + d.cout);
  for (int o = 0; o < d.cout; ++o) {
    double sb = b[o];
    for (int c = 0; c < d.cin; ++c) {
      const double sc = 256.0 * (double)pc.ea[c] / (255.0 * (double)pc.ed[c]), sh = (double)pc.eb[c] / (double)pc.ed[c];
      for (int t = 0; t < kk; ++t) {
        const size_t i = ((size_t)o * d.cin + c) * kk + t;
        Wf[i] = (float)((double)W[i] * sc);
        sb -= (double)W[i] * sh;
      }
    }
    bf[o] = (float)sb;
  }
  return true;
}

}

namespace nst {
int pack_upload_conv(const ConvKernelInfo& k, int cin, int cout, int ks, const float* W, int coutp, void** dev) {
  LayerDef d{"", "", cin, cout, ks, 1, AX_ZERO, ks / 2, 0, false};
  return upload_weights(k.dtype, pack_weights(k, d, W, coutp), dev);
}
int upload_floats(const float* host, size_t n, float** dev) { return upload(host, n * 4, (void**)dev); }
bool decode_consts_for_preset(int preset, DecodeConsts& d) {
  PresetConsts pc;
  if (!preset_consts(preset, pc)) return false;
  for (int c = 0; c < 3; ++c) {
    d.p[c] = pc.dp[c]; d.q[c] = pc.dq[c]; d.r[c] = pc.dr[c]; d.s[c] = pc.ds[c]; d.perm[c] = pc.dperm[c];
  }
  return true;
}
void tile_grid_of(const ConvKernelInfo& k, int sh, int sw, int oh, int ow, int* tx, int* ty) {
  tile_grid(k, sh, sw, oh, ow, tx, ty);
}
template <typename Get>
int frn_layer(Get& get, int li, const LayerDef& d, const float* W, const float* b, const float* bt,
              std::vector<float>& b_fold, std::vector<float>& bt_fold, float& eps) {
  auto act_tau = [](int l) -> std::string {
    if (l <= 2) return "encoder.layers." + std::to_string(l) + ".layers.2.tau";
    if (l <= 10) return "encoder.layers." + std::to_string(3 + (l - 3) / 2) + ".branch.0.layers.2.tau";
    return l == 11 ? "decoder.layers.1.layers.2.tau" : "decoder.layers.3.layers.2.tau";
  };
  auto block_tau = [](int r) { return "encoder.layers." + std::to_string(3 + r) + ".activation.tau"; };
  auto stream_tau = [&](int r) { return r == 0 ? act_tau(2) : block_tau(r - 1); };
  std::string in_tau;
  if (li == 1 || li == 2) in_tau = act_tau(li - 1);
  else if (li >= 3 && li <= 10) in_tau = (li - 3) % 2 == 0 ? stream_tau((li - 3) / 2) : act_tau(li - 1);
  else if (li == 11) in_tau = block_tau(3);
  else if (li >= 12) in_tau = act_tau(li - 1);
  const float* tin = nullptr;
  int rc = NST_OK;
  if (!in_tau.empty() && (rc = get(in_tau, d.cin, &tin)) != NST_OK) return rc;
  b_fold.assign(b, b + d.cout);
  if (tin) {
    const int kk = d.ks * d.ks;
    for (int o = 0; o < d.cout; ++o) {
      double s = b[o];
      for (int c = 0; c < d.cin; ++c) {
        double wsum = 0.0;
        for (int t = 0; t < kk; ++t) wsum += W[((size_t)o * d.cin + c) * kk + t];
        s += wsum * (double)tin[c];
      }
      b_fold[o] = (float)s;
    }
  }
  if (d.norm.empty()) return NST_OK;
  const float* e = nullptr;
  if ((rc = get(d.norm + ".eps", 1, &e)) != NST_OK) return rc;
  eps = std::fabs(e[0]);
  bt_fold.assign(bt, bt + d.cout);
  const bool join = li >= 3 && li <= 10 && (li - 3) % 2 == 1;
  const float *t_own = nullptr, *t_prev = nullptr;
  if (join) {
    const int r = (li - 3) / 2;
    if ((rc = get(block_tau(r), d.cout, &t_own)) != NST_OK) return rc;
    if ((rc = get(stream_tau(r), d.cout, &t_prev)) != NST_OK) return rc;
  } else if ((rc = get(act_tau(li), d.cout, &t_own)) != NST_OK) {
    return rc;
  }
  for (int c = 0; c < d.cout; ++c)
    bt_fold[c] = (float)((double)bt[c] - (double)t_own[c] + (t_prev ? (double)t_prev[c] : 0.0));
  return NST_OK;
}

}

extern "C" {

const char* nst_last_error(void) { return g_last_error.c_str(); }
const char* nst_version(void) { return "nst_hip 0.1.0 (gfx950)"; }

int nst_create(int arch, const nst_param* params, int n_params, int compute_dtype, int device,
               nst_handle** out) {
  return nst_create_ex(arch, params, n_params, compute_dtype, device, 0u, out);
}

int nst_create_ex(int arch, const nst_param* params, int n_params, int compute_dtype, int device,
                  unsigned flags, nst_handle** out) {
  if (!out || arch < 0 || arch > NST_ARCH_TORCH7_BN || (compute_dtype != NST_DT_F32 && compute_dtype != NST_DT_BF16 && compute_dtype != NST_DT_F16 &&
                                           compute_dtype != NST_DT_F32S && compute_dtype != NST_DT_F16M) ||
      (flags & ~(unsigned)NST_KSEL_ALL) != 0) {
    set_error("nst_create: invalid arguments");
    return NST_E_INVALID;
  }
  const bool f16m = compute_dtype == NST_DT_F16M;
  const int split_blocks = !f16m ? 0 : ((flags & NST_KSEL_F16M_TWO_BLOCKS) ? 2 : 1);
  if (f16m && is_torch7(arch)) {
    set_error("nst_create: NST_DT_F16M is not built for the Torch7 nets (use NST_DT_F32S or NST_DT_F32)");
    return NST_E_INVALID;
  }
  if (f16m && (is_reconet(arch) || (flags & (NST_KSEL_UNFUSED_RESIDUAL | NST_KSEL_NO_WS9 | NST_KSEL_NO_WS2 | NST_KSEL_NO_PREPAD)))) {
    set_error("nst_create: NST_DT_F16M is built for the Johnson / NST nets with the default kernel selection");
    return NST_E_INVALID;
  }
  auto layer_kdt = [&](size_t li) -> int {
    if (!f16m) return compute_dtype;
    if (li == 0) return NST_KDT_SW_O32;
    if (li == 1 || li == 2) return NST_KDT_SPLIT_O32;
    if (li >= 3 && li < 3 + 2 * (size_t)split_blocks) return NST_KDT_SPLITO_O32;
    return NST_DT_F16;
  };
  const bool no_pers = (flags & NST_KSEL_NO_PERSISTENT) != 0;
  *out = nullptr;
  std::map<std::string, const nst_param*> byname;
  for (int i = 0; i < n_params; ++i)
    if (params[i].name) byname[params[i].name] = &params[i];
  auto get = [&](const std::string& name, int64_t numel, const float** p) -> int {
    auto it = byname.find(name);
    if (it == byname.end()) { set_error("missing checkpoint tensor: " + name); return NST_E_PARAM; }
    if (it->second->numel != numel) {
      set_error("checkpoint tensor " + name + " has " + std::to_string(it->second->numel) +
                " elements, expected " + std::to_string(numel));
      return NST_E_PARAM;
    }
    *p = it->second->data;
    return NST_OK;
  };
  DeviceGuard guard(device);
  auto* h = new nst_handle();
  h->arch = arch; h->dtype = compute_dtype; h->device = device;
  std::vector<LayerDef> defs;
  const bool fuse_res = (flags & NST_KSEL_UNFUSED_RESIDUAL) == 0 && !is_torch7(arch);
  build_program(arch, fuse_res, fuse_res, defs, h->prog, split_blocks);
  std::vector<int> res_layer(defs.size(), 0);
  for (const Op& op : h->prog)
    if (op.kind == OP_CONV && op.res_buf >= 0) res_layer[op.layer] = 1;
  auto pad_ch = [&](int c) {
    if (f32_storage(compute_dtype)) return round_up(c, 16);
    return c <= 32 ? 32 : round_up(c, 64);
  };
  int rc = NST_OK;
  for (size_t li = 0; li < defs.size() && rc == NST_OK; ++li) {
    Layer Ly;
    Ly.d = defs[li];
    const LayerDef& d = Ly.d;
    const int kdt = layer_kdt(li);
    Ly.kdt = kdt;
    const bool image_in = li == 0;
    const bool final_layer = d.norm.empty();
    Ly.cinp = image_in ? 4 : pad_ch(d.cin);
    Ly.coutp = final_layer ? 16 : pad_ch(d.cout);
    if (is_reconet(arch) && !f32_storage(compute_dtype) && !(flags & NST_KSEL_PAD_DECODER)) {
      if (li == 11) Ly.coutp = 96;
      if (li == 12) Ly.cinp = 96;
    }
    if (is_reconet(arch) && !f32_storage(compute_dtype) &&
        !(flags & (NST_KSEL_PAD_48 | NST_KSEL_PAD_ENCODER | NST_KSEL_NO_WS9 | NST_KSEL_NO_WS2 | NST_KSEL_NO_PREPAD))) {
      if (li == 0) Ly.coutp = 48;
      if (li == 1) Ly.cinp = 48;
    }
    if (is_reconet(arch) && !f32_storage(compute_dtype) &&
        !(flags & (NST_KSEL_PAD_48 | NST_KSEL_PAD_DECODER | NST_KSEL_NO_WPHASE | NST_KSEL_NO_KYROT))) {
      if (li == 12) Ly.coutp = 48;
      if (li == 13) Ly.cinp = 48;
    }
    if (is_reconet(arch) && !f32_storage(compute_dtype) && !(flags & NST_KSEL_PAD_ENCODER)) {
      if (li == 1) Ly.coutp = 96;
      if (li == 2) Ly.cinp = 96;
    }
    const int ink = image_in ? IN_U8_NHWC : IN_ACT;
    const int outk = final_layer ? OUT_U8_NHWC : OUT_ACT;
    const bool up = d.axis_mode == AX_REFLECT_UP2 || d.axis_mode == AX_ZINSERT;
    std::vector<int> modes;
    if (up && !(res_layer[li] && is_reconet(arch)) && !(flags & NST_KSEL_NO_WPHASE))
      modes.push_back(MODE_WPHASE);
    if (up) modes.push_back(MODE_PHASE);
    if (final_layer && d.cout == 3) {
      if (!(flags & NST_KSEL_NO_KYROT)) modes.push_back(MODE_KYROT);
      modes.push_back(MODE_XSHIFT);
    }
    if (!up && !final_layer && !image_in && d.ks == 3 && d.stride == 1 && !is_reconet(arch) && !is_torch7(arch) &&
        !(flags & NST_KSEL_NO_WSTAT))
      modes.push_back(MODE_WSTAT);
    if (!up && !final_layer && !image_in && d.ks == 3 && d.stride == 2 && !(flags & NST_KSEL_NO_WS2))
      modes.push_back(MODE_WS2);
    if (kdt == NST_KDT_SPLITO_O32) modes.insert(modes.begin(), MODE_WS1S);
    modes.push_back(MODE_STD);
    if (image_in && !(flags & NST_KSEL_NO_PREPAD)) {
      Ly.k_main = (flags & NST_KSEL_NO_WS9)
                      ? nullptr
                      : find_conv_kernel(kdt, MODE_WS9, d.ks, d.stride, Ly.cinp, Ly.coutp, IN_ACT, outk, 0, no_pers);
      if (Ly.k_main) Ly.mode = MODE_WS9;
      else Ly.k_main = find_conv_kernel(kdt, MODE_STD, d.ks, d.stride, Ly.cinp, Ly.coutp, IN_ACT, outk, 0, no_pers);
      if (Ly.k_main && d.stride == 1) { Ly.prepad = true; Ly.k_alt = Ly.k_main; modes.clear(); }
      else Ly.k_main = nullptr;
    }
    for (int mode : modes) {
      Ly.k_main = find_conv_kernel(kdt, mode, d.ks, d.stride, Ly.cinp, Ly.coutp, ink, outk, res_layer[li], no_pers);
      Ly.k_alt = nullptr;
      if (image_in) Ly.k_alt = find_conv_kernel(kdt, mode, d.ks, d.stride, Ly.cinp, Ly.coutp, IN_F32_NCHW, outk, 0, no_pers);
      if (final_layer) Ly.k_alt = find_conv_kernel(kdt, mode, d.ks, d.stride, Ly.cinp, Ly.coutp, ink, OUT_F32_NCHW, 0, no_pers);
      const bool tanh_ok = mode != MODE_KYROT || !Ly.k_main ||
                           (Ly.k_main->tanh_out == (is_reconet(arch) ? 1 : 0) && Ly.k_alt &&
                            Ly.k_alt->tanh_out == Ly.k_main->tanh_out);
      if (Ly.k_main && tanh_ok && (!(image_in || final_layer) || Ly.k_alt)) { Ly.mode = mode; break; }
      Ly.k_main = nullptr;
    }
    if (!Ly.k_main || ((image_in || final_layer) && !Ly.k_alt)) {
      set_error("no compiled conv kernel for layer " + d.conv + " (ks " + std::to_string(d.ks) + " stride " +
                std::to_string(d.stride) + " cin " + std::to_string(Ly.cinp) + " cout " + std::to_string(Ly.coutp) + ")");
      rc = NST_E_SHAPE;
      break;
    }
    const float *W = nullptr, *b = nullptr, *gm = nullptr, *bt = nullptr;
    const int64_t wn = (int64_t)d.cout * d.cin * d.ks * d.ks;
    if ((rc = get(d.conv + ".weight", wn, &W)) != NST_OK) break;
    if ((rc = get(d.conv + ".bias", d.cout, &b)) != NST_OK) break;
    if (!final_layer) {
      if ((rc = get(d.norm + ".weight", d.cout, &gm)) != NST_OK) break;
      if ((rc = get(d.norm + ".bias", d.cout, &bt)) != NST_OK) break;
    }
    std::vector<float> b_fold, bt_fold;
    if (is_torch7(arch) && !final_layer) {
      const float* e = nullptr;
      if ((rc = get(d.norm + ".eps", 1, &e)) != NST_OK) break;
      if (!(e[0] >= 0.f)) { set_error("checkpoint tensor " + d.norm + ".eps is negative or NaN"); rc = NST_E_PARAM; break; }
      Ly.eps = e[0];
      if (arch == NST_ARCH_TORCH7_BN) {
        const float *rm = nullptr, *rv = nullptr;
        if ((rc = get(d.norm + ".running_mean", d.cout, &rm)) != NST_OK) break;
        if ((rc = get(d.norm + ".running_var", d.cout, &rv)) != NST_OK) break;
        std::vector<float2> tab(Ly.coutp, make_float2(0.f, 0.f));
        for (int c = 0; c < d.cout; ++c) {
          const double scale = (double)gm[c] / std::sqrt((double)rv[c] + (double)Ly.eps);
          tab[c] = make_float2((float)scale, (float)((double)bt[c] - (double)rm[c] * scale));
        }
        if ((rc = upload(tab.data(), tab.size() * sizeof(float2), (void**)&Ly.bn_tab)) != NST_OK) break;
      }
    }
    if (arch == NST_ARCH_RECONET_FRN) {
      if ((rc = frn_layer(get, (int)li, d, W, b, bt, b_fold, bt_fold, Ly.eps)) != NST_OK) break;
      b = b_fold.data();
      if (!final_layer) bt = bt_fold.data();
      Ly.frn = final_layer ? 0 : 1;
    }
    auto upload_packed = [&](const std::vector<float>& pk, void** dst) -> int {
      if (Ly.k_main->split_w) return upload_weights(NST_DT_F16, split_weight_frags(*Ly.k_main, pk), dst);
      return upload_weights(kdt >= NST_KDT_SW_O32 ? NST_DT_F16 : kdt, pk, dst);
    };
    Ly.in_esz = Ly.k_main->in_esz ? Ly.k_main->in_esz : (int)act_elem_bytes(kdt);
    Ly.out_esz = Ly.k_main->out_esz ? Ly.k_main->out_esz : (int)act_elem_bytes(kdt);
    if (Ly.mode == MODE_KYROT) {
      const std::vector<float> pk = pack_kyrot_weights(*Ly.k_main, d, W);
      if ((rc = Ly.k_main->dtype == NST_DT_F32S ? upload_weights(NST_DT_F16, pk, &Ly.wpk) : upload_packed(pk, &Ly.wpk)) != NST_OK)
        break;
    } else if (Ly.mode == MODE_WSTAT) {
      if ((rc = upload_packed(Ly.k_main->tw != 32 ? pack_wstat_weights(d, W)
                                                   : Ly.k_main->wn == 2 ? pack_wst16_weights(d, W) : pack_wst32_weights(d, W),
                              &Ly.wpk)) != NST_OK)
        break;
    } else if (Ly.mode == MODE_WPHASE) {
      if ((rc = upload_packed(pack_wphase_weights(*Ly.k_main, d, W), &Ly.wpk)) != NST_OK) break;
    } else if (Ly.mode == MODE_WS2 || Ly.mode == MODE_WS1S) {
      if ((rc = upload_packed(pack_ws2_weights(*Ly.k_main, d, W), &Ly.wpk)) != NST_OK) break;
    } else if (Ly.mode == MODE_WS9) {
      if ((rc = upload_packed(pack_ws9_weights(*Ly.k_main, d, W), &Ly.wpk)) != NST_OK) break;
    } else if ((rc = upload_packed(pack_weights(*Ly.k_main, d, W, Ly.coutp), &Ly.wpk)) != NST_OK) {
      break;
    }
    if (Ly.prepad && !f32_storage(compute_dtype) && !(flags & NST_KSEL_NO_FOLD)) {
      for (int pr = 1; pr < NST_PRESET_TORCH7 && rc == NST_OK; ++pr) {
        std::vector<float> Wf, bfo;
        if (!fold_first_layer(d, W, b, pr, Wf, bfo)) continue;
        std::vector<float> pk = Ly.mode == MODE_WS9 ? pack_ws9_weights(*Ly.k_main, d, Wf.data())
                                                    : pack_weights(*Ly.k_main, d, Wf.data(), Ly.coutp);
        std::vector<float> bpad(Ly.coutp, 0.f);
        std::copy(bfo.begin(), bfo.end(), bpad.begin());
        if ((rc = upload_packed(pk, &Ly.wpk_fold[pr])) != NST_OK) break;
        rc = upload(bpad.data(), bpad.size() * 4, (void**)&Ly.bias_fold[pr]);
      }
      if (rc != NST_OK) break;
    }
    if (image_in && compute_dtype == NST_DT_F32S && d.stride == 1 &&
// ... 149 lines not shown
              " differs from the input; request F32 output and use nst_decode_resize_u8");
    return NST_E_SHAPE;
  }
  if (!workspace || workspace_bytes < P.ws_bytes) {
    set_error("nst_forward: workspace too small (" + std::to_string(workspace_bytes) + " < " + std::to_string(P.ws_bytes) + ")");
    return NST_E_WORKSPACE;
  }
  DeviceGuard guard(h->device);
  hipStream_t st = (hipStream_t)stream;
  char* ws = (char*)workspace;
  void* bufs[NBUF];
  for (int b = 0; b < NBUF; ++b) bufs[b] = ws + P.off_buf[b];
  float* partial = (float*)(ws + P.off_partial);
  std::vector<float2*> stats(h->layers.size());
  {
    size_t off = P.off_stats;
    for (size_t li = 0; li < h->layers.size(); ++li) {
      stats[li] = (float2*)(ws + off);
      off += align256((size_t)n * h->layers[li].coutp * 8);
    }
  }
  auto run_op = [&](size_t i) -> int {
    const Op& op = h->prog[i];
    const Layer& Ly = h->layers[op.layer];
    auto tab = [&](int layer) { return layer >= 0 ? stats[layer] : nullptr; };
    if (op.kind == OP_RESADD) {
      const int hw = P.oh[i] * P.ow[i];
      const int rdt = P.out_esz[i] == 4 ? NST_DT_F32 : h->dtype;
      hipError_t e = op.shave > 0
                         ? launch_residual_shave(rdt, bufs[op.src], tab(op.layer), bufs[op.r_buf], tab(op.r_norm), op.r_relu,
                                                 bufs[op.dst], n, P.oh[i], P.ow[i], op.shave, Ly.coutp, st)
                     : (P.in_esz[i] == 4 && P.res_esz[i] == 4 && P.out_esz[i] == 2)
                         ? launch_residual_f32_to_f16(bufs[op.src], tab(op.layer), bufs[op.r_buf], tab(op.r_norm),
                                                      op.r_relu, op.relu_out, bufs[op.dst], n, hw, Ly.coutp, st)
                         : launch_residual(rdt, bufs[op.src], tab(op.layer), bufs[op.r_buf], tab(op.r_norm), op.r_relu,
                                           op.relu_out, bufs[op.dst], n, hw, Ly.coutp, st);
      if (e != hipSuccess) { set_error(std::string("residual launch: ") + hipGetErrorString(e)); return NST_E_HIP; }
      if (cap && cap->act && cap->act[i])
        NST_HIP_CHECK(hipMemcpyAsync(cap->act[i], bufs[op.dst], (size_t)n * hw * Ly.coutp * P.out_esz[i],
                                     hipMemcpyDeviceToDevice, st));
      return NST_OK;
    }
    const bool image_in = op.src == B_IMG, final_out = op.dst == B_OUT;
    const ConvKernelInfo* k = Ly.k_main;
    if (image_in && x_fmt == NST_IO_F32_NCHW) k = Ly.k_alt;
    if (final_out && (y_fmt == NST_IO_F32_NCHW || t7)) k = Ly.k_alt;
    const bool fold = image_in && x_fmt == NST_IO_U8_NHWC && preset >= 0 && preset < 8 && Ly.wpk_fold[preset] != nullptr &&
                      (Ly.prepad || Ly.k_u8fold);
    if (fold && Ly.k_u8fold) k = Ly.k_u8fold;
    const bool prepad = Ly.prepad || (fold && Ly.k_u8fold);
    const int mode = fold && Ly.k_u8fold ? MODE_WS9 : Ly.mode;
    const int kdt = fold && Ly.k_u8fold ? NST_KDT_SW_O32 : Ly.kdt;
    ConvParams p;
    std::memset(&p, 0, sizeof(p));
    p.in = image_in ? x : bufs[op.src];
    p.hs = P.ih[i];
    p.ws = P.iw[i];
    p.cs = image_in ? 3 : Ly.cinp;
    p.axis_mode = Ly.d.axis_mode;
    p.pad = Ly.d.axis_mode == AX_ZINSERT ? 1 : Ly.d.pad;
    if (mode == MODE_PHASE || mode == MODE_WPHASE) {
      p.axis_mode = Ly.d.axis_mode == AX_ZINSERT ? AX_ZERO : AX_CLAMP;
      p.pad = 1;
      p.ph_off[0] = Ly.d.axis_mode == AX_ZINSERT ? 1 : 0;
      p.ph_off[1] = 1;
    }
    p.pre = Ly.d.pre;
    p.in_norm = tab(op.in_norm);
    p.in_relu = op.in_norm >= 0 && op.res_buf < 0 ? 1 : 0;
    if (op.res_buf >= 0) {
      p.res_r = bufs[op.res_buf];
      p.res_rnorm = tab(op.r_norm);
      p.res_relu = op.relu_out;
    }
    p.res_out = op.res_out >= 0 ? bufs[op.res_out] : nullptr;
    for (int c = 0; c < 3; ++c) {
      p.enc_a[c] = pc.ea[c]; p.enc_b[c] = pc.eb[c]; p.enc_d[c] = pc.ed[c]; p.enc_perm[c] = pc.eperm[c];
      p.dec_p[c] = pc.dp[c]; p.dec_q[c] = pc.dq[c]; p.dec_r[c] = pc.dr[c]; p.dec_s[c] = pc.ds[c]; p.dec_perm[c] = pc.dperm[c];
    }
    if (image_in && x_fmt == NST_IO_F32_NCHW && preset == NST_PRESET_NONE) {
      for (int c = 0; c < 3; ++c) { p.enc_a[c] = 1.f; p.enc_b[c] = 0.f; p.enc_d[c] = 1.f; p.enc_perm[c] = c; }
    }
    p.enc_raw = fold ? 1 : 0;
    if (image_in && prepad) {
      const int hp = P.ch[i] + Ly.d.ks - 1, wp = P.cw[i] + Ly.d.ks - 1;
      void* pre = ws + P.off_pre;
      const int pdt = (kdt == NST_DT_F16 || kdt == NST_KDT_SW_O32 || kdt == NST_KDT_SW_O16) ? NST_DT_F16 : NST_DT_BF16;
      hipError_t e = launch_prepad_encode(pdt, p, x_fmt == NST_IO_U8_NHWC ? IN_U8_NHWC : IN_F32_NCHW, n, hp, wp, pre, st);
      if (e != hipSuccess) { set_error(std::string("prepad launch: ") + hipGetErrorString(e)); return NST_E_HIP; }
      p.in = pre;
      p.hs = hp;
      p.ws = wp;
      p.cs = 4;
      p.axis_mode = AX_ZERO;
      p.pad = 0;
      p.pre = 0;
    }
    p.dec_tanh = (is_reconet(h->arch) && final_out) ? 1 : 0;
    p.wpk = fold ? Ly.wpk_fold[preset] : Ly.wpk;
    p.bias = fold ? Ly.bias_fold[preset] : Ly.bias;
    if (mode == MODE_XSHIFT && final_out && y_fmt == NST_IO_U8_NHWC && pc.dperm[0] == 2 && !t7) {
      p.wpk = Ly.wpk_rev;
      p.bias = Ly.bias_rev;
    }
    p.hconv = P.ch[i];
    p.wconv = P.cw[i];
    p.oh = P.oh[i];
    p.ow = P.ow[i];
    p.crop_y = (P.ch[i] - P.oh[i]) / 2;
    p.crop_x = (P.cw[i] - P.ow[i]) / 2;
    p.out = final_out ? (t7 ? (void*)(ws + P.off_tail) : y) : bufs[op.dst];
    p.cout_real = Ly.d.cout;
    p.cout_stride = Ly.coutp;
    tile_grid(*k, p.hs, p.ws, p.oh, p.ow, &p.tiles_x, &p.tiles_y);
    p.n_cblk = Ly.coutp / k->bn;
    if (p.res_out != nullptr && p.res_r == nullptr &&
        ((mode != MODE_WSTAT && mode != MODE_STD) || p.in_norm == nullptr || Ly.d.stride != 1)) {
      set_error("conv " + Ly.d.conv + ": only the trunk kernels (weight-stationary / generic stride-1) write their "
                "normalised input");
      return NST_E_SHAPE;
    }
    if (mode == MODE_WSTAT && p.res_r != nullptr && (p.in_norm == nullptr || p.res_out == nullptr || p.res_relu)) {
      set_error("conv " + Ly.d.conv + ": weight-stationary kernel joins IN(y) + r into a residual-stream buffer");
      return NST_E_SHAPE;
    }
    if (mode == MODE_WS2 && k->cinp_k && (p.axis_mode != AX_REFLECT)) {
      set_error("conv " + Ly.d.conv + ": the narrow-input down-conv is built for reflection padding");
      return NST_E_SHAPE;
    }
    if (mode == MODE_WS2 && (p.in_norm == nullptr || p.res_r != nullptr || p.crop_x || p.crop_y)) {
      set_error("conv " + Ly.d.conv + ": weight-stationary down-conv reads a normalized activation, uncropped");
      return NST_E_SHAPE;
    }
    if (mode == MODE_WS9 && (!prepad || p.in_norm != nullptr || p.res_r != nullptr || p.crop_x || p.crop_y || final_out)) {
      set_error("conv " + Ly.d.conv + ": weight-stationary 9x9 kernel reads the pre-padded frame, uncropped");
      return NST_E_SHAPE;
    }
    if (mode == MODE_WS1S && (p.res_r != nullptr || p.res_out != nullptr || p.crop_x || p.crop_y)) {
      set_error("conv " + Ly.d.conv + ": split-operand trunk kernel runs plain convs, uncropped");
      return NST_E_SHAPE;
    }
    if ((mode == MODE_WPHASE || mode == MODE_WSTAT || mode == MODE_WS2 || mode == MODE_WS9 ||
         mode == MODE_WS1S) && p.cout_stride != k->bn) {
      set_error("conv " + Ly.d.conv + ": weight-stationary kernels store whole pixels of bn channels");
      return NST_E_SHAPE;
    }
    if (mode == MODE_WPHASE && p.res_r != nullptr &&
        (p.in_norm == nullptr || p.res_out != nullptr || p.res_relu || p.res_rnorm != nullptr)) {
      set_error("conv " + Ly.d.conv + ": weight-stationary phase kernel joins IN(y) + r without writing the stream");
      return NST_E_SHAPE;
    }
    if (k->persistent && p.n_cblk != 1) { set_error("conv " + Ly.d.conv + ": persistent kernel needs one channel block"); return NST_E_SHAPE; }
    p.partial = final_out ? nullptr : partial;
    dim3 grid(p.tiles_x * p.tiles_y, n * p.n_cblk);
    nst_handle::Rec rec{op.layer, nullptr, nullptr};
    if (h->profiling) {
      NST_HIP_CHECK(hipEventCreate(&rec.a));
      NST_HIP_CHECK(hipEventCreate(&rec.b));
      NST_HIP_CHECK(hipEventRecord(rec.a, st));
    }
    k->launch(p, grid, st);
    hipError_t e = hipGetLastError();
    if (h->profiling && e == hipSuccess) {
      NST_HIP_CHECK(hipEventRecord(rec.b, st));
      h->recs.push_back(rec);
    }
    if (e != hipSuccess) { set_error("conv " + Ly.d.conv + " launch: " + hipGetErrorString(e)); return NST_E_HIP; }
    if (final_out && t7) {
      const int tmode = preset == NST_PRESET_NONE ? 0 : (y_fmt == NST_IO_F32_NCHW ? 1 : 2);
      e = launch_t7_tail((const float*)(ws + P.off_tail), n, P.out_h, P.out_w, h->t7_mul, tmode, y, st);
      if (e != hipSuccess) { set_error(std::string("torch7 tail launch: ") + hipGetErrorString(e)); return NST_E_HIP; }
    }
    if (!final_out && Ly.bn_tab) {
      e = launch_norm_table_fill(Ly.bn_tab, n, Ly.coutp, tab(op.layer), st);
      if (e != hipSuccess) { set_error(std::string("norm table launch: ") + hipGetErrorString(e)); return NST_E_HIP; }
    } else if (!final_out) {
      e = launch_in_finalize(partial, n, p.tiles_x * p.tiles_y * k->part_rows, Ly.coutp, (double)p.hconv * (double)p.wconv,
                             Ly.gamma, Ly.beta, Ly.eps, Ly.frn, tab(op.layer), ws + P.off_seg, st);
      if (e == hipSuccess && h->range_flag)
        e = launch_check_finite((const float*)tab(op.layer), (size_t)n * Ly.coutp * 2, h->range_flag, st);
      if (e != hipSuccess) { set_error(std::string("finalize launch: ") + hipGetErrorString(e)); return NST_E_HIP; }
    }
    if (cap && !final_out) {
      if (cap->act && cap->act[i])
        NST_HIP_CHECK(hipMemcpyAsync(cap->act[i], bufs[op.dst], (size_t)n * P.oh[i] * P.ow[i] * Ly.coutp * P.out_esz[i],
                                     hipMemcpyDeviceToDevice, st));
      if (cap->res && cap->res[i] && op.res_out >= 0)
        NST_HIP_CHECK(hipMemcpyAsync(cap->res[i], bufs[op.res_out], (size_t)n * P.ih[i] * P.iw[i] * Ly.cinp * P.res_esz[i],
                                     hipMemcpyDeviceToDevice, st));
      if (cap->stats && cap->stats[i])
        NST_HIP_CHECK(hipMemcpyAsync(cap->stats[i], stats[op.layer], (size_t)n * Ly.coutp * 8, hipMemcpyDeviceToDevice, st));
    }
    return NST_OK;
  };
  if (h->range_flag) NST_HIP_CHECK(hipMemsetAsync(h->range_flag, 0, sizeof(int), st));
  for (size_t i = 0; i < h->prog.size(); ++i) {
    const int rc = run_op(i);
    if (rc != NST_OK) return rc;
  }
  if (h->range_flag) {
    if (y_fmt == NST_IO_F32_NCHW)
      NST_HIP_CHECK(launch_check_finite((const float*)y, (size_t)n * 3 * P.out_h * P.out_w, h->range_flag, st));
    int bad = 0;
    NST_HIP_CHECK(hipMemcpyAsync(&bad, h->range_flag, sizeof(int), hipMemcpyDeviceToHost, st));
    NST_HIP_CHECK(hipStreamSynchronize(st));
    if (bad) {
      set_error("nst_forward: a non-finite InstanceNorm statistic or output value (an activation left the range of "
                "the compute dtype: fp16 / split-fp16 operands hold |v| <= 65504)");
      return NST_E_RANGE;
    }
  }
  return NST_OK;
}

}

extern "C" {

int nst_forward(nst_handle* h, const void* x, int x_fmt, int n, int in_h, int in_w, int preset, void* y,
                int y_fmt, void* workspace, size_t workspace_bytes, void* stream) {
  const int k = (!h || h->profiling || h->range_flag || n <= 1) ? 1 : std::min(h->split, n);
  if (k == 1 || !x || !y || in_h <= 0 || in_w <= 0 || (x_fmt != NST_IO_F32_NCHW && x_fmt != NST_IO_U8_NHWC) ||
      (y_fmt != NST_IO_F32_NCHW && y_fmt != NST_IO_U8_NHWC))
    return forward_impl(h, x, x_fmt, n, in_h, in_w, preset, y, y_fmt, workspace, workspace_bytes, stream, nullptr);
  const int nb = (n + k - 1) / k, parts = (n + nb - 1) / nb;
  const Plan Q = make_plan(h, nb, in_h, in_w);
  if (!Q.ok) { set_error(Q.err); return NST_E_SHAPE; }
  const size_t per = align256(Q.ws_bytes);
  const Plan Pn = make_plan(h, n, in_h, in_w);
  if (!Pn.ok) { set_error(Pn.err); return NST_E_SHAPE; }
  const size_t need = std::max(Pn.ws_bytes, per * parts);
  if (!workspace || workspace_bytes < need) {
    set_error("nst_forward: workspace too small (" + std::to_string(workspace_bytes) + " < " + std::to_string(need) + ")");
    return NST_E_WORKSPACE;
  }
  DeviceGuard guard(h->device);
  if (!h->fork) NST_HIP_CHECK(hipEventCreateWithFlags(&h->fork, hipEventDisableTiming));
  for (int i = 0; i < parts; ++i) {
    if (!h->sub[i]) NST_HIP_CHECK(hipStreamCreateWithFlags(&h->sub[i], hipStreamNonBlocking));
    if (!h->join[i]) NST_HIP_CHECK(hipEventCreateWithFlags(&h->join[i], hipEventDisableTiming));
  }
  const hipStream_t st = (hipStream_t)stream;
  const size_t fx = x_fmt == NST_IO_U8_NHWC ? (size_t)in_h * in_w * 3 : (size_t)3 * in_h * in_w * 4;
  const size_t fy = y_fmt == NST_IO_U8_NHWC ? (size_t)Q.out_h * Q.out_w * 3 : (size_t)3 * Q.out_h * Q.out_w * 4;
  NST_HIP_CHECK(hipEventRecord(h->fork, st));
  int rc = NST_OK;
  for (int i = 0; i < parts; ++i) {
    NST_HIP_CHECK(hipStreamWaitEvent(h->sub[i], h->fork, 0));
    const int f0 = i * nb, m = std::min(nb, n - f0);
    if (rc == NST_OK)
      rc = forward_impl(h, (const char*)x + f0 * fx, x_fmt, m, in_h, in_w, preset, (char*)y + f0 * fy, y_fmt,
                        (char*)workspace + i * per, per, h->sub[i], nullptr);
    NST_HIP_CHECK(hipEventRecord(h->join[i], h->sub[i]));
    NST_HIP_CHECK(hipStreamWaitEvent(st, h->join[i], 0));
  }
  return rc;
}

int nst_forward_capture(nst_handle* h, const void* x, int x_fmt, int n, int in_h, int in_w, int preset, void* y,
                        int y_fmt, void* workspace, size_t workspace_bytes, void* const* act, void* const* res,
                        void* const* stats, void* stream) {
  const Capture cap{act, res, stats};
  return forward_impl(h, x, x_fmt, n, in_h, in_w, preset, y, y_fmt, workspace, workspace_bytes, stream, &cap);
}

int nst_set_range_check(nst_handle* h, int enable) {
  if (!h) { set_error("nst_set_range_check: null handle"); return NST_E_INVALID; }
  DeviceGuard guard(h->device);
  if (enable && !h->range_flag) {
    if (hipMalloc(&h->range_flag, sizeof(int)) != hipSuccess) {
      h->range_flag = nullptr;
      set_error("nst_set_range_check: hipMalloc failed");
      return NST_E_HIP;
    }
  } else if (!enable && h->range_flag) {
    (void)hipFree(h->range_flag);
    h->range_flag = nullptr;
  }
  return NST_OK;
}

int nst_num_ops(const nst_handle* h) { return h ? (int)h->prog.size() : 0; }

int nst_op_describe(const nst_handle* h, int n, int in_h, int in_w, int op_index, nst_op_desc* out) {
  if (!h || !out || n <= 0 || in_h <= 0 || in_w <= 0 || op_index < 0 || op_index >= (int)h->prog.size()) {
    set_error("nst_op_describe: invalid arguments");
    return NST_E_INVALID;
  }
  Plan P = make_plan(h, n, in_h, in_w);
  if (!P.ok) { set_error(P.err); return NST_E_SHAPE; }
  const Op& op = h->prog[op_index];
  const Layer& Ly = h->layers[op.layer];
  std::memset(out, 0, sizeof(*out));
  out->kind = op.kind;
  out->layer = op.layer;
  out->src = op.src;
  out->dst = op.dst;
  if (op.kind == OP_CONV) {
    out->in_norm = op.in_norm;
    out->in_relu = op.in_norm >= 0 && op.res_buf < 0 ? 1 : 0;
    out->res_buf = op.res_buf;
    out->res_norm = op.res_buf >= 0 ? op.r_norm : -1;
    out->res_out = op.res_out;
    out->relu_out = op.res_buf >= 0 ? op.relu_out : 0;
  } else {
    out->in_norm = op.layer;
    out->in_relu = 0;
    out->res_buf = op.r_buf;
    out->res_norm = op.r_norm;
    out->res_out = -1;
    out->relu_out = op.relu_out;
  }
  out->in_h = P.ih[op_index];
  out->in_w = P.iw[op_index];
  out->out_h = P.oh[op_index];
  out->out_w = P.ow[op_index];
  out->conv_h = P.ch[op_index];
  out->conv_w = P.cw[op_index];
  out->cin_stride = op.src == B_IMG ? 3 : Ly.cinp;
  out->cout_stride = Ly.coutp;
  out->kernel_mode = Ly.mode;
  out->elem_bytes = P.out_esz[op_index];
  out->in_elem_bytes = P.in_esz[op_index];
  out->res_elem_bytes = P.res_esz[op_index];
  out->kernel_dtype = op.kind == OP_CONV ? Ly.kdt : h->dtype;
  return NST_OK;
}

int nst_profile_begin(nst_handle* h) {
  if (!h) { set_error("nst_profile_begin: null handle"); return NST_E_INVALID; }
  h->profiling = true;
  return NST_OK;
}

int nst_profile_end(nst_handle* h, int n_layers, float* total_ms, int* launches) {
  if (!h || n_layers < 0 || (n_layers > 0 && (!total_ms || !launches))) {
    set_error("nst_profile_end: invalid arguments");
    return NST_E_INVALID;
  }
  DeviceGuard guard(h->device);
  for (int i = 0; i < n_layers; ++i) { total_ms[i] = 0.f; launches[i] = 0; }
  int rc = NST_OK;
  for (auto& r : h->recs) {
    float ms = 0.f;
    hipError_t e = hipEventElapsedTime(&ms, r.a, r.b);
    if (e != hipSuccess && rc == NST_OK) {
      set_error(std::string("hipEventElapsedTime: ") + hipGetErrorString(e));
      rc = NST_E_HIP;
    }
    if (r.layer < n_layers) { total_ms[r.layer] += ms; launches[r.layer] += 1; }
    (void)hipEventDestroy(r.a);
    (void)hipEventDestroy(r.b);
  }
  h->recs.clear();
  h->profiling = false;
  return rc;
}

int nst_num_layers(const nst_handle* h) { return h ? (int)h->layers.size() : 0; }

const char* nst_layer_name(const nst_handle* h, int layer) {
  if (!h || layer < 0 || layer >= (int)h->layers.size()) return "";
  return h->layers[layer].d.conv.c_str();
}

int nst_decode_resize_u8(const float* y, int n, int h, int w, int preset, uint8_t* out, int out_h, int out_w,
                         void* stream) {
  PresetConsts pc;
  if (!y || !out || n <= 0 || h <= 0 || w <= 0 || out_h <= 0 || out_w <= 0 || !preset_consts(preset, pc)) {
    set_error("nst_decode_resize_u8: invalid arguments");
    return NST_E_INVALID;
  }
  hipError_t e = launch_decode_resize_u8(y, n, h, w, pc.dp, pc.dq, pc.dr, pc.ds, pc.dperm, out, out_h, out_w,
                                         (hipStream_t)stream);
  if (e != hipSuccess) { set_error(std::string("decode_resize launch: ") + hipGetErrorString(e)); return NST_E_HIP; }
  return NST_OK;
}

int nst_blend_models_u8(const float* const* ys, const int* presets, const float* weights, int m, int n, int h,
                        int w, uint8_t* out, int out_h, int out_w, void* stream) {
  if (!ys || !presets || !weights || !out || m <= 0 || m > NST_MAX_MODELS || n <= 0 || h <= 0 || w <= 0 ||
      out_h <= 0 || out_w <= 0) {
    set_error("nst_blend_models_u8: invalid arguments");
    return NST_E_INVALID;
  }
  float dp[NST_MAX_MODELS][3], dq[NST_MAX_MODELS][3], dr[NST_MAX_MODELS][3], ds[NST_MAX_MODELS][3];
  int perm[NST_MAX_MODELS][3];
  for (int k = 0; k < m; ++k) {
    PresetConsts pc;
    if (!ys[k] || !preset_consts(presets[k], pc)) {
      set_error("nst_blend_models_u8: bad model output or preset for slot " + std::to_string(k));
      return NST_E_INVALID;
    }
    for (int c = 0; c < 3; ++c) {
      dp[k][c] = pc.dp[c]; dq[k][c] = pc.dq[c]; dr[k][c] = pc.dr[c]; ds[k][c] = pc.ds[c]; perm[k][c] = pc.dperm[c];
    }
  }
  hipError_t e = launch_blend_models_u8(ys, dp, dq, dr, ds, perm, weights, m, n, h, w, out, out_h, out_w,
                                        (hipStream_t)stream);
  if (e != hipSuccess) { set_error(std::string("blend_models launch: ") + hipGetErrorString(e)); return NST_E_HIP; }
  return NST_OK;
}

int nst_lab_create(const uint8_t* rgb2lab, const uint8_t* lab2rgb, int device, nst_lab** out) {
  if (!rgb2lab || !lab2rgb || !out) { set_error("nst_lab_create: invalid arguments"); return NST_E_INVALID; }
  DeviceGuard guard(device);
  auto* l = new nst_lab();
  l->device = device;
  const size_t entries = (size_t)1 << 24;
  std::vector<uint32_t> wide(entries);
  auto widen = [&](const uint8_t* t) {
    for (size_t i = 0; i < entries; ++i)
      wide[i] = (uint32_t)t[3 * i] | ((uint32_t)t[3 * i + 1] << 8) | ((uint32_t)t[3 * i + 2] << 16);
  };
  widen(rgb2lab);
  int rc = upload(wide.data(), entries * 4, (void**)&l->rgb2lab);
  if (rc == NST_OK) {
    widen(lab2rgb);
    rc = upload(wide.data(), entries * 4, (void**)&l->lab2rgb);
  }
  if (rc != NST_OK) { nst_lab_destroy(l); return rc; }
  *out = l;
  return NST_OK;
}

void nst_lab_destroy(nst_lab* l) {
  if (!l) return;
  DeviceGuard guard(l->device);
  if (l->rgb2lab) (void)hipFree(l->rgb2lab);
  if (l->lab2rgb) (void)hipFree(l->lab2rgb);
  delete l;
}

int nst_lab_ema_u8(const nst_lab* lab, const uint8_t* rgb_in, uint8_t* rgb_out, int n, int h, int w,
                   int smooth_lightness, float alpha, float one_minus_alpha, int smooth_chroma, float chroma_alpha,
                   float one_minus_chroma_alpha, float* state, int first, void* stream) {
  if (!lab || !rgb_in || !rgb_out || !state || n <= 0 || h <= 0 || w <= 0) {
    set_error("nst_lab_ema_u8: invalid arguments");
    return NST_E_INVALID;
  }
  hipError_t e = launch_lab_ema(lab->rgb2lab, lab->lab2rgb, rgb_in, rgb_out, n, h * w, smooth_lightness, alpha,
                                one_minus_alpha, smooth_chroma, chroma_alpha, one_minus_chroma_alpha, state, first,
                                (hipStream_t)stream);
  if (e != hipSuccess) { set_error(std::string("lab_ema launch: ") + hipGetErrorString(e)); return NST_E_HIP; }
  return NST_OK;
}

int nst_lab_planes_u8(const nst_lab* lab, const uint8_t* rgb_in, int n, int h, int w, int smooth_lightness,
                      int smooth_chroma, uint8_t* planes, void* stream) {
  const int sl = smooth_lightness ? 1 : 0, sc = smooth_chroma ? 1 : 0;
  if (!lab || !rgb_in || !planes || n <= 0 || h <= 0 || w <= 0 || !(sl || sc)) {
    set_error("nst_lab_planes_u8: invalid arguments");
    return NST_E_INVALID;
  }
  hipError_t e = launch_lab_planes(lab->rgb2lab, rgb_in, planes, n, h * w, sl, sc, (hipStream_t)stream);
  if (e != hipSuccess) { set_error(std::string("lab_planes launch: ") + hipGetErrorString(e)); return NST_E_HIP; }
  return NST_OK;
}

int nst_lab_ema_planes(const uint8_t* planes_in, uint8_t* planes_out, int n, int h, int w, int smooth_lightness,
                       float alpha, float one_minus_alpha, int smooth_chroma, float chroma_alpha,
                       float one_minus_chroma_alpha, float* state, int first, void* stream) {
  const int sl = smooth_lightness ? 1 : 0, sc = smooth_chroma ? 1 : 0;
  if (!planes_in || !planes_out || !state || n <= 0 || h <= 0 || w <= 0 || !(sl || sc)) {
    set_error("nst_lab_ema_planes: invalid arguments");
    return NST_E_INVALID;
  }
  hipError_t e = launch_lab_ema_planes(planes_in, planes_out, n, h * w, sl, alpha, one_minus_alpha, sc, chroma_alpha,
                                       one_minus_chroma_alpha, state, first, (hipStream_t)stream);
  if (e != hipSuccess) { set_error(std::string("lab_ema_planes launch: ") + hipGetErrorString(e)); return NST_E_HIP; }
  return NST_OK;
}

int nst_lab_merge_u8(const nst_lab* lab, const uint8_t* rgb_in, const uint8_t* planes, int n, int h, int w,
                     int smooth_lightness, int smooth_chroma, uint8_t* rgb_out, void* stream) {
  const int sl = smooth_lightness ? 1 : 0, sc = smooth_chroma ? 1 : 0;
  if (!lab || !rgb_in || !planes || !rgb_out || n <= 0 || h <= 0 || w <= 0 || !(sl || sc)) {
    set_error("nst_lab_merge_u8: invalid arguments");
// ... 91 lines not shown
```

neuralstyletransferv1_amd/csrc/nst_internal.h:

```cpp
#pragma once

#include <hip/hip_runtime.h>
#include <stdint.h>
#include <stddef.h>
#include <cmath>
#include <cstring>
#include <string>

#include "nst_hip.h"

namespace nst {

inline uint16_t f32_to_f16_rne(float f) {
  uint32_t u;
  std::memcpy(&u, &f, 4);
  const uint16_t sign = (uint16_t)((u >> 16) & 0x8000u);
  uint32_t a = u & 0x7fffffffu;
  if (a > 0x7f800000u) return sign | 0x7e00u;
  if (a >= 0x477ff000u) return sign | 0x7c00u;
  if (a >= 0x38800000u) {
    a -= 0x38000000u;
    a += 0xfffu + ((a >> 13) & 1u);
    return sign | (uint16_t)(a >> 13);
  }
  float af;
  std::memcpy(&af, &a, 4);
  return sign | (uint16_t)std::nearbyint(af * 16777216.0f);
}
inline uint16_t f32_to_bf16_rne(float f) {
  uint32_t u;
  std::memcpy(&u, &f, 4);
  if ((u & 0x7fffffffu) > 0x7f800000u) return (uint16_t)((u >> 16) | 0x40);
  u += 0x7fffu + ((u >> 16) & 1u);
  return (uint16_t)(u >> 16);
}
inline float f16_to_f32(uint16_t h) {
  const int e = (h >> 10) & 31, m = h & 1023;
  float v = e == 0 ? std::ldexp((float)m, -24) : (e == 31 ? INFINITY : std::ldexp((float)(m | 1024), e - 25));
  return (h & 0x8000u) ? -v : v;
}
inline bool f32_storage(int dtype) { return dtype == NST_DT_F32 || dtype == NST_DT_F32S; }
inline size_t act_elem_bytes(int dtype) { return f32_storage(dtype) ? 4 : 2; }

void set_error(const std::string& msg);
#define NST_HIP_CHECK(expr)                                                               \
  do {                                                                                    \
    hipError_t _e = (expr);                                                               \
    if (_e != hipSuccess) {                                                               \
      ::nst::set_error(std::string(#expr) + " failed: " + hipGetErrorString(_e));         \
      return NST_E_HIP;                                                                   \
    }                                                                                     \
  } while (0)

enum InKind { IN_ACT = 0, IN_U8_NHWC = 1, IN_F32_NCHW = 2 };
enum OutKind { OUT_ACT = 0, OUT_U8_NHWC = 1, OUT_F32_NCHW = 2 };

enum AxisMode { AX_REFLECT = 0, AX_REFLECT_UP2 = 1, AX_ZERO = 2, AX_ZERO_PREREFLECT = 3, AX_ZINSERT = 4, AX_CLAMP = 5 };

enum ConvMode { MODE_STD = 0, MODE_PHASE = 1, MODE_XSHIFT = 2, MODE_KYROT = 3, MODE_WSTAT = 4, MODE_WPHASE = 5, MODE_WS2 = 6, MODE_WS9 = 7,
                MODE_WS1S = 8 };

struct ConvParams {
  const void* in;
  int hs, ws;
  int cs;
  int axis_mode, pad, pre;
  const float2* in_norm;
  int in_relu;
  const void* res_r;
  const float2* res_rnorm;
  void* res_out;
  int res_relu;
  float enc_a[3], enc_b[3], enc_d[3];
  int enc_perm[3];
  int enc_raw;
  const void* wpk;
  const float* bias;
  int hconv, wconv;
  int crop_y, crop_x;
  int oh, ow;
  void* out;
  int cout_real;
  int cout_stride;
  float* partial;
  int tiles_x, tiles_y, n_cblk;
  int n_work;
  float dec_p[3], dec_q[3], dec_r[3], dec_s[3];
  int dec_perm[3];
  int dec_tanh;
  int seg_len;
  int ph_off[2];
};

constexpr int NST_MAX_STREAM_SPLIT = 4;
enum KernelDtype { NST_KDT_SW_O32 = 16, NST_KDT_SW_O16 = 17, NST_KDT_SPLIT_O32 = 18, NST_KDT_SPLIT_O16 = 19,
                   NST_KDT_SPLITO_O32 = 20 };

struct ConvKernelInfo {
  int dtype;
  int mode;
  int ks, stride, cinp, bn, th, tw, wm, wn, in_kind, out_kind;
  int pair, nch, cpc, kp, nchunk, nstep, nstep_pack, nsubt, nsub, lds_bytes;
  int persistent;
  int korder;
  int part_rows;
  int wbytes;
  int res;
  int tanh_out;
  int in_esz, out_esz;
  int split_w;
  int cinp_k, bn_k;
  void (*launch)(const ConvParams&, dim3 grid, hipStream_t);
};

const ConvKernelInfo* find_conv_kernel(int dtype, int mode, int ks, int stride, int cinp, int bn, int in_kind,
                                       int out_kind, int res = 0, bool no_persistent = false);

int pack_upload_conv(const ConvKernelInfo& k, int cin, int cout, int ks, const float* W, int coutp, void** dev);
int upload_floats(const float* host, size_t n, float** dev);
void tile_grid_of(const ConvKernelInfo& k, int sh, int sw, int oh, int ow, int* tx, int* ty);
const ConvKernelInfo* conv_table_vgg(int* count);

hipError_t launch_vgg_pool(const void* z, int h, int w, int c, void* out, hipStream_t st);
hipError_t launch_vgg_pool_bwd(const void* z, const void* gp, int h, int w, int c, void* gz, hipStream_t st);
hipError_t launch_vgg_relu_bwd(const void* z, const void* ga, const void* P, float cw, size_t elems, void* gz,
                               hipStream_t st);
hipError_t launch_vgg_gram_bwd(const void* z, const void* ga, const void* P, float cw, const void* Mb, int hw, int c,
                               void* gz, hipStream_t st);
int vgg_content_parts(size_t elems);
hipError_t launch_vgg_losses(const void* z, const void* P, size_t elems, float* part, float* style_raw,
                             float cscale, const float* sscale, float* losses, hipStream_t st,
                             const float* spart = nullptr, const int* snparts = nullptr, int sstride = 0);
hipError_t launch_adam(float* x, const float* g, float* m, float* v, int hw, int n, const float* inv_std, float lr,
                       float b1, float b2, float eps, float bc1, float bc2, int clamp01, hipStream_t st);

constexpr int IN_MAX_SEGMENTS = 128;
int in_finalize_segments(int tiles);
hipError_t launch_check_finite(const float* v, size_t n, int* flag, hipStream_t st);
hipError_t launch_in_finalize(const float* partial, int n, int tiles, int cstride, double count,
                              const float* gamma, const float* beta, float eps, int frn, float2* out,
                              void* seg_ws, hipStream_t st);
hipError_t launch_residual(int dtype, const void* y, const float2* ys, const void* r,
                           const float2* rs, int r_relu, int relu_out, void* out, int n, int hw,
                           int c, hipStream_t st);
hipError_t launch_residual_f32_to_f16(const void* y, const float2* ys, const void* r, const float2* rs, int r_relu,
                                      int relu_out, void* out, int n, int hw, int c, hipStream_t st);
hipError_t launch_residual_shave(int dtype, const void* y, const float2* ys, const void* r, const float2* rs, int r_relu,
                                 void* out, int n, int oh, int ow, int shave, int c, hipStream_t st);
hipError_t launch_norm_table_fill(const float2* tab, int n, int c, float2* out, hipStream_t st);
hipError_t launch_t7_tail(const float* t, int n, int h, int w, float mul, int mode, void* out, hipStream_t st);
hipError_t launch_decode_resize_u8(const float* y, int n, int h, int w, const float* p,
                                   const float* q, const float* r, const float* s, const int* perm,
                                   uint8_t* out, int oh, int ow, hipStream_t st);
constexpr int NST_MAX_MODELS = 8;
hipError_t launch_blend_models_u8(const float* const* ys, const float (*dp)[3], const float (*dq)[3],
                                  const float (*dr)[3], const float (*ds)[3], const int (*perm)[3], const float* wts,
                                  int m, int n, int h, int w, uint8_t* out, int oh, int ow, hipStream_t st);
hipError_t launch_lab_ema(const uint32_t* rgb2lab, const uint32_t* lab2rgb, const uint8_t* in,
                          uint8_t* out, int n, int hw, int sl, float a, float oma, int sc, float ca,
                          float coma, float* state, int first, hipStream_t st);
hipError_t launch_lab_planes(const uint32_t* rgb2lab, const uint8_t* in, uint8_t* planes, int n, int hw, int sl, int sc,
                             hipStream_t st);
hipError_t launch_lab_ema_planes(const uint8_t* in, uint8_t* out, int n, int hw, int sl, float a, float oma, int sc,
                                 float ca, float coma, float* state, int first, hipStream_t st);
hipError_t launch_lab_merge(const uint32_t* rgb2lab, const uint32_t* lab2rgb, const uint8_t* in, const uint8_t* planes,
                            uint8_t* out, int n, int hw, int sl, int sc, hipStream_t st);
hipError_t launch_lab_blend(const uint32_t* rgb2lab, const uint32_t* lab2rgb, const uint8_t* const* frames,
                            const float* wrest, int nrest, float wL, float wab, size_t npix, uint8_t* out,
                            hipStream_t st);
hipError_t launch_mask_feather(const uint8_t* m, int n, int h, int w, float sigma, float* tmp, float* alpha,
                               hipStream_t st);
__host__ __device__ inline int prepad_slack_rows(int wp) { return 18 + (1024 + wp - 1) / wp; }
hipError_t launch_prepad_encode(int dtype, const ConvParams& p, int in_kind, int n, int hp, int wp, void* out,
                                hipStream_t st);
hipError_t launch_blend(const uint8_t* s, const uint8_t* o, const float* mask, int mode, float b,
                        float omb, uint8_t* out, int n, int hw, hipStream_t st, const uint8_t* mask8 = nullptr);
size_t gram_workspace_bytes(int n, int c, int hw);
constexpr int GRAM_DELTA_MAX_PARTS = 512 * 512 / 64;
int gram_delta_parts(int n, int c, int hw);
struct GramDelta {
  const float* A;
  float k;
  __bf16* Mb;
  float* parts;
  float* loss_out;
};
hipError_t launch_vgg_sum_parts(const float* parts, int n, float* out, hipStream_t st);
hipError_t launch_gram(const void* F, int dtype, int layout_hwc, int n, int c, int hw, float* G, void* ws,
                       hipStream_t st, int relu = 0, const GramDelta* delta = nullptr);

}
```

neuralstyletransferv1_amd/csrc/nst_ops.hip:

```cpp
#include <algorithm>
#include <cstdlib>

#include "nst_internal.h"
#include "seg_internal.h"
#include "nst_hip.h"
#include "post_common.h"
#include "conv_impl.h"

namespace nst {

typedef __bf16 bf16x8_t __attribute__((ext_vector_type(8)));
typedef float f32x4_t __attribute__((ext_vector_type(4)));

template <int CH>
__global__ __launch_bounds__(256) void in_partial_reduce_kernel(const float* __restrict__ partial, int tiles,
                                                                int cstride, int per_seg,
                                                                double2* __restrict__ seg) {
  constexpr int PH = 256 / CH;
  __shared__ double red[4][CH][2];
  const int n = blockIdx.x, s = blockIdx.z;
  const int cl = threadIdx.x & (CH - 1), q = threadIdx.x / CH;
  const int c = blockIdx.y * CH + cl;
  const int t0 = s * per_seg, t1 = min(tiles, t0 + per_seg);
  double s1 = 0.0, s2 = 0.0;
  if (c < cstride) {
    const float2* p = (const float2*)partial + (size_t)n * tiles * cstride + c;
    int t = t0 + q;
    for (; t + 3 * PH < t1; t += 4 * PH) {
      const float2 a = p[(size_t)t * cstride], b = p[(size_t)(t + PH) * cstride];
      const float2 d = p[(size_t)(t + 2 * PH) * cstride], e = p[(size_t)(t + 3 * PH) * cstride];
      s1 += (double)a.x + (double)b.x + (double)d.x + (double)e.x;
      s2 += (double)a.y + (double)b.y + (double)d.y + (double)e.y;
    }
    for (; t < t1; t += PH) {
      const float2 a = p[(size_t)t * cstride];
      s1 += a.x;
      s2 += a.y;
    }
  }
#pragma unroll
  for (int o = CH; o < 64; o <<= 1) {
    s1 += __shfl_xor(s1, o);
    s2 += __shfl_xor(s2, o);
  }
  const int wv = threadIdx.x >> 6;
  if ((threadIdx.x & 63) < CH) {
    red[wv][cl][0] = s1;
    red[wv][cl][1] = s2;
  }
  __syncthreads();
  if (threadIdx.x < CH && c < cstride) {
    s1 = red[0][cl][0] + red[1][cl][0] + red[2][cl][0] + red[3][cl][0];
    s2 = red[0][cl][1] + red[1][cl][1] + red[2][cl][1] + red[3][cl][1];
    seg[((size_t)n * gridDim.z + s) * cstride + c] = make_double2(s1, s2);
  }
}

template <int CH>
__global__ __launch_bounds__(256) void in_finalize_kernel(const double2* __restrict__ seg, int nseg, int cstride,
                                                          double count, const float* __restrict__ gamma,
                                                          const float* __restrict__ beta, float eps, int frn,
                                                          float2* __restrict__ out) {
  constexpr int PH = 256 / CH;
  __shared__ double red[4][CH][2];
  const int n = blockIdx.x;
  const int cl = threadIdx.x & (CH - 1), q = threadIdx.x / CH;
  const int c = blockIdx.y * CH + cl;
  double s1 = 0.0, s2 = 0.0;
  if (c < cstride) {
    for (int s = q; s < nseg; s += PH) {
      const double2 v = seg[((size_t)n * nseg + s) * cstride + c];
      s1 += v.x;
      s2 += v.y;
    }
  }
#pragma unroll
  for (int o = CH; o < 64; o <<= 1) {
    s1 += __shfl_xor(s1, o);
    s2 += __shfl_xor(s2, o);
  }
  const int wv = threadIdx.x >> 6;
  if ((threadIdx.x & 63) < CH) {
    red[wv][cl][0] = s1;
    red[wv][cl][1] = s2;
  }
  __syncthreads();
  if (threadIdx.x >= CH || c >= cstride) return;
  s1 = red[0][cl][0] + red[1][cl][0] + red[2][cl][0] + red[3][cl][0];
  s2 = red[0][cl][1] + red[1][cl][1] + red[2][cl][1] + red[3][cl][1];
  const double mean = frn ? 0.0 : s1 / count;
  double var = s2 / count - mean * mean;
  var = var < 0.0 ? 0.0 : var;
  const double rstd = 1.0 / sqrt(var + (double)eps);
  const double scale = (double)gamma[c] * rstd;
  out[(size_t)n * cstride + c] = make_float2((float)scale, (float)((double)beta[c] - mean * scale));
}
constexpr int IN_RED_CH = 16, IN_FIN_CH = 4;

constexpr int IN_ONE_MAX_TILES = 2048;
template <int CH>
__global__ __launch_bounds__(1024) void in_stats_kernel(const float* __restrict__ partial, int tiles, int cstride,
                                                        double count, const float* __restrict__ gamma,
                                                        const float* __restrict__ beta, float eps, int frn,
                                                        float2* __restrict__ out) {
  constexpr int PH = 1024 / CH, NL = IN_ONE_MAX_TILES / PH;
  __shared__ double red[16][CH][2];
  const int n = blockIdx.x;
  const int cl = threadIdx.x & (CH - 1), q = threadIdx.x / CH;
  const int c = min(blockIdx.y * CH + cl, cstride - 1);
  const float2* p = (const float2*)partial + (size_t)n * tiles * cstride + c;
  float2 v[NL];
#pragma unroll
  for (int k = 0; k < NL; ++k) v[k] = p[(size_t)min(q + k * PH, tiles - 1) * cstride];
  double s1 = 0.0, s2 = 0.0;
#pragma unroll
  for (int k = 0; k < NL; ++k) {
    const bool in = q + k * PH < tiles;
    s1 += in ? (double)v[k].x : 0.0;
    s2 += in ? (double)v[k].y : 0.0;
  }
#pragma unroll
  for (int o = CH; o < 64; o <<= 1) {
    s1 += __shfl_xor(s1, o);
    s2 += __shfl_xor(s2, o);
  }
  const int wv = threadIdx.x >> 6;
  if ((threadIdx.x & 63) < CH) {
    red[wv][cl][0] = s1;
    red[wv][cl][1] = s2;
  }
  __syncthreads();
  if (threadIdx.x >= CH || blockIdx.y * CH + cl >= cstride) return;
  s1 = red[0][cl][0];
  s2 = red[0][cl][1];
  for (int w = 1; w < 16; ++w) {
    s1 += red[w][cl][0];
    s2 += red[w][cl][1];
  }
  const double mean = frn ? 0.0 : s1 / count;
  double var = s2 / count - mean * mean;
  var = var < 0.0 ? 0.0 : var;
  const double rstd = 1.0 / sqrt(var + (double)eps);
  const double scale = (double)gamma[c] * rstd;
  out[(size_t)n * cstride + c] = make_float2((float)scale, (float)((double)beta[c] - mean * scale));
}

static int in_one_ch() {
  static const int v = [] {
    const char* e = std::getenv("NST_IN_ONE_CH");
    const int x = e ? std::atoi(e) : 4;
    return (x == 2 || x == 8 || x == 16) ? x : 4;
  }();
  return v;
}

int in_finalize_segments(int tiles) { return max(1, min(IN_MAX_SEGMENTS, tiles / 64)); }

__global__ __launch_bounds__(256) void check_finite_kernel(const float* __restrict__ v, size_t n, int* __restrict__ flag) {
  bool bad = false;
  for (size_t i = (size_t)blockIdx.x * blockDim.x + threadIdx.x; i < n; i += (size_t)gridDim.x * blockDim.x)
    bad |= !__builtin_isfinite(v[i]);
  if (bad) atomicOr(flag, 1);
}
hipError_t launch_check_finite(const float* v, size_t n, int* flag, hipStream_t st) {
  const unsigned blocks = (unsigned)std::min<size_t>((n + 255) / 256, 1024);
  hipLaunchKernelGGL(check_finite_kernel, dim3(std::max(1u, blocks)), dim3(256), 0, st, v, n, flag);
  return hipGetLastError();
}

hipError_t launch_in_finalize(const float* partial, int n, int tiles, int cstride, double count,
                              const float* gamma, const float* beta, float eps, int frn, float2* out,
                              void* seg_ws, hipStream_t st) {
  if (tiles <= IN_ONE_MAX_TILES) {
    const int ch = in_one_ch();
    const dim3 grid(n, (cstride + ch - 1) / ch);
    if (ch == 2)
      hipLaunchKernelGGL(in_stats_kernel<2>, grid, dim3(1024), 0, st, partial, tiles, cstride, count, gamma, beta, eps, frn, out);
    else if (ch == 4)
      hipLaunchKernelGGL(in_stats_kernel<4>, grid, dim3(1024), 0, st, partial, tiles, cstride, count, gamma, beta, eps, frn, out);
    else if (ch == 8)
      hipLaunchKernelGGL(in_stats_kernel<8>, grid, dim3(1024), 0, st, partial, tiles, cstride, count, gamma, beta, eps, frn, out);
    else
      hipLaunchKernelGGL(in_stats_kernel<16>, grid, dim3(1024), 0, st, partial, tiles, cstride, count, gamma, beta, eps, frn, out);
    return hipGetLastError();
  }
  const int nseg = in_finalize_segments(tiles);
  const int per_seg = (tiles + nseg - 1) / nseg;
  hipLaunchKernelGGL(in_partial_reduce_kernel<IN_RED_CH>, dim3(n, (cstride + IN_RED_CH - 1) / IN_RED_CH, nseg),
                     dim3(256), 0, st, partial, tiles, cstride, per_seg, (double2*)seg_ws);
  hipError_t e = hipGetLastError();
  if (e != hipSuccess) return e;
  hipLaunchKernelGGL(in_finalize_kernel<IN_FIN_CH>, dim3(n, (cstride + IN_FIN_CH - 1) / IN_FIN_CH), dim3(256), 0, st,
                     (const double2*)seg_ws, nseg, cstride, count, gamma, beta, eps, frn, out);
  return hipGetLastError();
}

constexpr int RES_UNROLL = 4;
template <typename T>
__global__ __launch_bounds__(256) void residual_kernel(const T* __restrict__ y, const float2* __restrict__ ys,
                                                       const T* r, const float2* __restrict__ rs,
                                                       int r_relu, int relu_out, T* out, int hw, int c) {
  constexpr int CPC = 16 / (int)sizeof(T);
  const int cv_n = c / CPC;
  const int tpp = blockDim.x / cv_n;
  const int cv = threadIdx.x % cv_n, pl = threadIdx.x / cv_n;
  const int n = blockIdx.y;
  const int ch0 = cv * CPC;
  float ysc[CPC], ysh[CPC], rsc[CPC], rsh[CPC];
#pragma unroll
  for (int j = 0; j < CPC; ++j) {
    const float2 a = ys[(size_t)n * c + ch0 + j];
    ysc[j] = a.x; ysh[j] = a.y;
    rsc[j] = 1.f; rsh[j] = 0.f;
    if (rs) { const float2 b = rs[(size_t)n * c + ch0 + j]; rsc[j] = b.x; rsh[j] = b.y; }
  }
  const size_t base = (size_t)n * hw * c + ch0;
  const int px0 = blockIdx.x * tpp * RES_UNROLL + pl;
  uint4 va[RES_UNROLL], vb[RES_UNROLL];
#pragma unroll
  for (int u = 0; u < RES_UNROLL; ++u) {
    const int px = px0 + u * tpp;
    if (px < hw) {
      va[u] = *(const uint4*)(y + base + (size_t)px * c);
      vb[u] = *(const uint4*)(r + base + (size_t)px * c);
    }
  }
#pragma unroll
  for (int u = 0; u < RES_UNROLL; ++u) {
    const int px = px0 + u * tpp;
    if (px >= hw) continue;
    float vy[CPC], vr[CPC];
    if constexpr (sizeof(T) == 2) {
      const uint32_t wa[4] = {va[u].x, va[u].y, va[u].z, va[u].w}, wb[4] = {vb[u].x, vb[u].y, vb[u].z, vb[u].w};
#pragma unroll
      for (int j = 0; j < 4; ++j) {
        vy[2 * j] = lo16<T>(wa[j]);
        vy[2 * j + 1] = hi16<T>(wa[j]);
        vr[2 * j] = lo16<T>(wb[j]);
        vr[2 * j + 1] = hi16<T>(wb[j]);
      }
    } else {
      vy[0] = __uint_as_float(va[u].x); vy[1] = __uint_as_float(va[u].y);
      vy[2] = __uint_as_float(va[u].z); vy[3] = __uint_as_float(va[u].w);
      vr[0] = __uint_as_float(vb[u].x); vr[1] = __uint_as_float(vb[u].y);
      vr[2] = __uint_as_float(vb[u].z); vr[3] = __uint_as_float(vb[u].w);
    }
    float o[CPC];
#pragma unroll
    for (int j = 0; j < CPC; ++j) {
      float rr = vr[j];
      if (rs) {
        if constexpr (sizeof(T) == 2)
          rr = lo16<T>(pack16<T>(__builtin_fmaf(rr, rsc[j], rsh[j]), 0.f));
        else
          rr = rr * rsc[j] + rsh[j];
        if (r_relu) rr = fmaxf(rr, 0.f);
      }
      float v = vy[j] * ysc[j] + ysh[j];
      v = rr + v;
      if (relu_out) v = fmaxf(v, 0.f);
      o[j] = v;
    }
    T* dst = out + base + (size_t)px * c;
    if constexpr (sizeof(T) == 2) {
      uint32_t w[4];
#pragma unroll
      for (int j = 0; j < 4; ++j) w[j] = pack16<T>(o[2 * j], o[2 * j + 1]);
      *(uint4*)dst = make_uint4(w[0], w[1], w[2], w[3]);
    } else {
      *(float4*)dst = make_float4(o[0], o[1], o[2], o[3]);
    }
  }
}

hipError_t launch_residual(int dtype, const void* y, const float2* ys, const void* r, const float2* rs,
                           int r_relu, int relu_out, void* out, int n, int hw, int c, hipStream_t st) {
  const int cpc = f32_storage(dtype) ? 4 : 8;
  const int cv_n = c / cpc;
  if (c % cpc != 0 || cv_n > 256) return hipErrorInvalidValue;
  const int tpp = 256 / cv_n;
  const dim3 grid((unsigned)((hw + tpp * RES_UNROLL - 1) / (tpp * RES_UNROLL)), (unsigned)n);
  const dim3 block((unsigned)(tpp * cv_n));
  if (dtype == NST_DT_BF16)
    hipLaunchKernelGGL(residual_kernel<__bf16>, grid, block, 0, st, (const __bf16*)y, ys, (const __bf16*)r, rs,
                       r_relu, relu_out, (__bf16*)out, hw, c);
  else if (dtype == NST_DT_F16)
    hipLaunchKernelGGL(residual_kernel<_Float16>, grid, block, 0, st, (const _Float16*)y, ys, (const _Float16*)r, rs,
                       r_relu, relu_out, (_Float16*)out, hw, c);
  else
    hipLaunchKernelGGL(residual_kernel<float>, grid, block, 0, st, (const float*)y, ys, (const float*)r, rs, r_relu,
                       relu_out, (float*)out, hw, c);
  return hipGetLastError();
}

__global__ __launch_bounds__(256) void residual_f32_to_f16_kernel(const float* __restrict__ y, const float2* __restrict__ ys,
                                                                  const float* __restrict__ r, const float2* __restrict__ rs,
                                                                  int r_relu, int relu_out, _Float16* __restrict__ out,
                                                                  int hw, int c) {
  const int cv_n = c / 8;
  const int tpp = blockDim.x / cv_n;
  const int cv = threadIdx.x % cv_n, pl = threadIdx.x / cv_n;
  const int n = blockIdx.y, ch0 = cv * 8;
  float ysc[8], ysh[8], rsc[8], rsh[8];
#pragma unroll
  for (int j = 0; j < 8; ++j) {
    const float2 a = ys[(size_t)n * c + ch0 + j];
    ysc[j] = a.x; ysh[j] = a.y;
    rsc[j] = 1.f; rsh[j] = 0.f;
    if (rs) { const float2 b = rs[(size_t)n * c + ch0 + j]; rsc[j] = b.x; rsh[j] = b.y; }
  }
  const size_t base = (size_t)n * hw * c + ch0;
  for (int px = blockIdx.x * tpp + pl; px < hw; px += gridDim.x * tpp) {
    const float4* yp = (const float4*)(y + base + (size_t)px * c);
    const float4* rp = (const float4*)(r + base + (size_t)px * c);
    const float4 y0 = yp[0], y1 = yp[1], r0 = rp[0], r1 = rp[1];
    const float vy[8] = {y0.x, y0.y, y0.z, y0.w, y1.x, y1.y, y1.z, y1.w};
    const float vr[8] = {r0.x, r0.y, r0.z, r0.w, r1.x, r1.y, r1.z, r1.w};
    uint32_t w[4];
#pragma unroll
    for (int j = 0; j < 8; j += 2) {
      float o[2];
#pragma unroll
      for (int k = 0; k < 2; ++k) {
        float rr = vr[j + k];
        if (rs) {
          rr = rr * rsc[j + k] + rsh[j + k];
          if (r_relu) rr = fmaxf(rr, 0.f);
        }
        float v = vy[j + k] * ysc[j + k] + ysh[j + k];
        v = rr + v;
        if (relu_out) v = fmaxf(v, 0.f);
        o[k] = v;
      }
      w[j / 2] = pack16<_Float16>(o[0], o[1]);
    }
    *(uint4*)(out + base + (size_t)px * c) = make_uint4(w[0], w[1], w[2], w[3]);
// ... 992 lines not shown
```

Baseline: 1551 frames/s.

## Fold instance-norm statistics finalize into producer and consumer persistent conv kernels

For pairs of consecutive 128-channel reflect-padded convs, the producer kernel now walks tiles per frame and accumulates per-slice double partial sums in LDS. It writes one slot per slice, and the consumer conv reduces those slices itself to build the norm scale/shift table. This removes the separate in_finalize launch and the large per-tile partial buffer round trip between layers. The cost is that block-to-work mapping becomes frame-pinned, which can hurt load balance, and the standalone stats kernel is rewritten to match the same slice summation order.

```diff
diff --git a/include/nst_hip.h b/include/nst_hip.h
--- a/include/nst_hip.h
+++ b/include/nst_hip.h
@@ -70,7 +70,8 @@
 #define NST_KSEL_PAD_DECODER 0x400
 #define NST_KSEL_PAD_ENCODER 0x800
 #define NST_KSEL_PAD_48 0x1000
-#define NST_KSEL_ALL 0x1fff
+#define NST_KSEL_NO_IN_FOLD 0x2000
+#define NST_KSEL_ALL 0x3fff
 int nst_create_ex(int arch, const nst_param* params, int n_params, int compute_dtype, int device,
                   unsigned flags, nst_handle** out);
 void nst_destroy(nst_handle* h);
@@ -107,6 +108,7 @@
   int in_elem_bytes;
   int res_elem_bytes;
   int kernel_dtype;
+  int in_fold;
 } nst_op_desc;
 int nst_num_ops(const nst_handle* h);
 int nst_set_range_check(nst_handle* h, int enable);
diff --git a/neuralstyletransferv1_amd/_lib.py b/neuralstyletransferv1_amd/_lib.py
--- a/neuralstyletransferv1_amd/_lib.py
+++ b/neuralstyletransferv1_amd/_lib.py
@@ -58,7 +58,7 @@
 KSEL = {
     "no_wstat": 0x1, "no_wphase": 0x2, "no_ws2": 0x4, "no_ws9": 0x8, "no_kyrot": 0x10, "no_prepad": 0x20,
     "no_persistent": 0x40, "unfused_residual": 0x80, "no_fold": 0x100, "f16m_two_blocks": 0x200,
-    "pad_decoder": 0x400, "pad_encoder": 0x800, "pad_48": 0x1000,
+    "pad_decoder": 0x400, "pad_encoder": 0x800, "pad_48": 0x1000, "no_in_fold": 0x2000,
 }
 NST_BUF_INPUT, NST_BUF_OUTPUT = -1, -2
 
@@ -71,7 +71,7 @@
     _fields_ = [(n, ctypes.c_int) for n in (
         "kind", "layer", "src", "dst", "in_norm", "in_relu", "res_buf", "res_norm", "res_out", "relu_out",
         "in_h", "in_w", "conv_h", "conv_w", "out_h", "out_w", "cin_stride", "cout_stride", "kernel_mode",
-        "elem_bytes", "in_elem_bytes", "res_elem_bytes", "kernel_dtype")]
+        "elem_bytes", "in_elem_bytes", "res_elem_bytes", "kernel_dtype", "in_fold")]
 
     def as_dict(self):
         return {n: getattr(self, n) for n, _ in self._fields_}
diff --git a/neuralstyletransferv1_amd/csrc/conv_ws_common.h b/neuralstyletransferv1_amd/csrc/conv_ws_common.h
--- a/neuralstyletransferv1_amd/csrc/conv_ws_common.h
+++ b/neuralstyletransferv1_amd/csrc/conv_ws_common.h
@@ -61,6 +61,22 @@
   }
 }
 
+__device__ __forceinline__ double in_fold_add(double acc, float tile_partial) { return acc + (double)tile_partial; }
+__device__ __forceinline__ float2 in_fold_table(const double (&v)[IN_FOLD_MAX_SLICES], int S, bool odd, double count,
+                                                float gamma, float beta, float eps, int frn) {
+  double t = 0.0;
+#pragma unroll
+  for (int s = 0; s < IN_FOLD_MAX_SLICES; ++s) t = s < S ? t + v[s] : t;
+  const double o = __shfl_xor(t, 1);
+  const double s1 = odd ? o : t, s2 = odd ? t : o;
+  const double mean = frn ? 0.0 : s1 / count;
+  double var = s2 / count - mean * mean;
+  var = var < 0.0 ? 0.0 : var;
+  const double rstd = 1.0 / sqrt(var + (double)eps);
+  const double scale = (double)gamma * rstd;
+  return make_float2((float)scale, (float)((double)beta - mean * scale));
+}
+
 constexpr int ST_AUX = 2;
 
 enum WsFill { WF_NORM = 0, WF_RAW = 1, WF_RES = 2, WF_RESRN = 3 };
diff --git a/neuralstyletransferv1_amd/csrc/conv_wst16.hip b/neuralstyletransferv1_amd/csrc/conv_wst16.hip
--- a/neuralstyletransferv1_amd/csrc/conv_wst16.hip
+++ b/neuralstyletransferv1_amd/csrc/conv_wst16.hip
@@ -46,7 +46,8 @@
   static constexpr int BIAS_OFF = NORM_OFF + NORM_TAB;
   static constexpr int DUMMY_OFF = BIAS_OFF + CINP * 4;
   static constexpr int STG_OFF = DUMMY_OFF + 64 * 16;
-  static constexpr int LDS = STG_OFF + NIT * NW * SLOTB;
+  static constexpr int FOLD_OFF = STG_OFF + NIT * NW * SLOTB;
+  static constexpr int LDS = FOLD_OFF + NT * 8;
   static constexpr int SST = TH * TW * 4 / NT;
   static constexpr int EPI = 2 * TH + 1;
   static_assert(LDS <= 160 * 1024, "LDS budget");
@@ -90,18 +91,29 @@
   };
   const int ntile = p.tiles_x * p.tiles_y;
   const int nfr = p.n_work / ntile;
-  auto decode = [&](int wi) {
+  const int G = (int)gridDim.x, b = (int)blockIdx.x;
+  constexpr bool FOLDK = !ZPAD;
+  const int fr = (FOLDK && p.fold != 0) ? b % nfr : -1;
+  const int du = fr >= 0 ? G / nfr : G;
+  auto pos_ok = [&](int c) { return c < (fr >= 0 ? ntile : p.n_work); };
+  auto pos_next = [&](int c) {
+    if (fr < 0) return c + du;
+    const int S = in_fold_slices(ntile);
+    if (c + S < ntile) return c + S;
+    const int sl = (ntile >= IN_FOLD_MAX_SLICES ? c & (IN_FOLD_MAX_SLICES - 1) : c) + du;
+    return sl < S ? sl : ntile;
+  };
+  auto decode = [&](int c) {
     Work r;
-    r.n = wi / ntile;
-    r.tile = wi - r.n * ntile;
+    r.n = fr >= 0 ? fr : c / ntile;
+    r.tile = fr >= 0 ? c : c - r.n * ntile;
     const int ty = r.tile / p.tiles_x;
     r.ty0 = ty * TH;
     r.tx0 = (r.tile - ty * p.tiles_x) * C::TW;
     return r;
   };
-  const int G = (int)gridDim.x, b = (int)blockIdx.x;
-  const int w0 = (G % 8 == 0) ? (b % 8) * (G / 8) + b / 8 : b;
-  if (w0 >= p.n_work) return;
+  const int w0 = fr >= 0 ? b / nfr : (G % 8 == 0) ? (b % 8) * (G / 8) + b / 8 : b;
+  if (!pos_ok(w0)) return;
 
   u32x4_t wa[C::NA];
   u32x4_t wvr[C::NV];
@@ -113,7 +125,24 @@
     for (int s = 0; s < C::NV; ++s) wvr[s] = wsrc[(C::NA + s) * 64];
   }
   float* norm_y = (float*)(smem + C::NORM_OFF);
-  if (FILL != WF_RAW) {
+  if (FOLDK && FILL != WF_RAW && (p.fold & IN_FOLD_CONS)) {
+    static_assert(C::NT == 2 * C::CINP, "one (channel, statistic) per lane");
+    const int S = in_fold_slices(ntile);
+    const __amdgpu_buffer_rsrc_t rrs = __builtin_amdgcn_make_buffer_rsrc(
+        (void*)(p.fold_in + (size_t)fr * S * C::NT), (short)0, IN_FOLD_MAX_SLICES * C::NT * 8, 0x00020000);
+    double v[IN_FOLD_MAX_SLICES];
+#pragma unroll
+    for (int s = 0; s < IN_FOLD_MAX_SLICES; ++s)
+      v[s] = __builtin_bit_cast(double, __builtin_amdgcn_raw_buffer_load_b64(rrs, tid * 8, s * C::NT * 8, 0));
+    const int c = tid >> 1;
+    const float2 r = in_fold_table(v, S, (tid & 1) != 0, p.fold_count, p.fold_gamma[c], p.fold_beta[c], p.fold_eps, p.fold_frn);
+    if ((tid & 1) == 0) {
+      const int o = (fr * 16 + (c >> 3)) * 16 + 4 * ((c & 7) >> 1) + (c & 1);
+      norm_y[o] = r.x;
+      norm_y[o + 2] = r.y;
+      if (b < nfr) const_cast<float2*>(p.in_norm)[(size_t)fr * p.cs + c] = r;
+    }
+  } else if (FILL != WF_RAW) {
     for (int t = tid; t < nfr * C::CINP; t += C::NT) {
       const int f = t / C::CINP, c = t - f * C::CINP;
       const int o = (f * 16 + (c >> 3)) * 16 + 4 * ((c & 7) >> 1) + (c & 1);
@@ -317,16 +346,30 @@
     rs_step<1, 0xb1>(a2, a1, (p16 & 1) != 0);
     const int idx = (p16 >= 8 ? 8 : 0) + ((p16 & 4) ? 4 : 0) + ((p16 & 2) ? 2 : 0) + (p16 & 1);
     const int co = 32 * wv + 16 * (idx >> 3) + 4 * g4 + ((idx >> 1) & 3);
+    uint32_t po = (uint32_t)((co * 2 + (idx & 1)) * 4);
+    const bool fp = FOLDK && (p.fold & IN_FOLD_PROD) != 0;
+    const int S = in_fold_slices(ntile);
+    const int sl = ntile >= IN_FOLD_MAX_SLICES ? wk.tile & (IN_FOLD_MAX_SLICES - 1) : wk.tile;
+    const uint32_t rb = (uint32_t)p.cout_stride * (fp ? 16u : 8u);
+    const size_t row = fp ? (size_t)wk.n * S + sl : (size_t)wk.n * ntile + wk.tile;
     const __amdgpu_buffer_rsrc_t prs = __builtin_amdgcn_make_buffer_rsrc(
-        (void*)(p.partial + ((size_t)wk.n * ntile + wk.tile) * p.cout_stride * 2), (short)0, p.cout_stride * 8, 0x00020000);
-    __builtin_amdgcn_raw_buffer_store_b32(__float_as_uint(a1[0]), prs, (uint32_t)((co * 2 + (idx & 1)) * 4), 0, 0);
+        (fp ? (char*)p.fold_out : (char*)p.partial) + row * rb, (short)0, (int)rb, 0x00020000);
+    if (fp) {
+      asm volatile("" : "+v"(po));
+      double* facc = (double*)(smem + C::FOLD_OFF + 2 * po);
+      const double sum = in_fold_add(wk.tile < S ? 0.0 : *facc, a1[0]);
+      *facc = sum;
+      const u32x2_t bits = __builtin_bit_cast(u32x2_t, sum);
+      __builtin_amdgcn_raw_buffer_store_b64(bits, prs, wk.tile + S >= ntile ? 2 * po : OOB, 0, 0);
+    } else {
+      __builtin_amdgcn_raw_buffer_store_b32(__float_as_uint(a1[0]), prs, po, 0, 0);
+    }
   };
 
   Work cur = decode(w0);
-  int wn = w0 + G;
-  const int last = p.n_work - 1;
+  int pn = pos_next(w0);
   build_maps(cur, 0);
-  build_maps(decode(min(wn, last)), 1);
+  build_maps(pos_ok(pn) ? decode(pn) : cur, 1);
   asm volatile("s_waitcnt vmcnt(0)" ::: "memory");
   __syncthreads();
   uint32_t pad3;
@@ -373,9 +416,10 @@
   };
   for (int it = 0;; ++it) {
     stamp(it, 0);
-    const bool more = wn < p.n_work;
-    const Work nxt = more ? decode(wn) : cur;
-    const Work nxt2 = decode(min(wn + G, last));
+    const bool more = pos_ok(pn);
+    const Work nxt = more ? decode(pn) : cur;
+    const int pn2 = pos_next(pn);
+    const Work nxt2 = pos_ok(pn2) ? decode(pn2) : cur;
     const int cs = it & 1, ns = cs ^ 1;
     kloop(
         acc,
@@ -459,7 +503,7 @@
     stamp(it, 5);
     if (!more) break;
     cur = nxt;
-    wn += G;
+    pn = pn2;
   }
   vm_wait<0>();
 #if NST_WST32_STAMP
@@ -488,7 +532,12 @@
     const int ntile = (int)grid.x, n = (int)grid.y;
     const size_t fin = (size_t)p0.hs * p0.ws * p0.cs * 2, fout = (size_t)p0.oh * p0.ow * p0.cout_stride * 2;
     const int fmax = (int)std::min<size_t>(C::NFMAX, (size_t)OOB / std::max(fin, fout));
-    if (fmax < 1) return;
+    if (fmax < 1 || (p0.fold != 0 && (n > fmax || p0.axis_mode != AX_REFLECT || !in_fold_shape_ok(n, ntile, cus(), C::NFMAX)))) {
+      ConvParams p = p0;
+      p.n_work = 0;
+      go<WF_RAW, false>(p, 0, st);
+      return;
+    }
     for (int f0 = 0; f0 < n; f0 += fmax) {
       const int nf = std::min(fmax, n - f0);
       ConvParams p = p0;
@@ -532,6 +581,7 @@
     k.persistent = 1;
     k.part_rows = 1;
     k.res = RES ? 1 : 0;
+    k.in_fold = W16Cfg<TH, WF_RES>::NFMAX;
     k.launch = &launch;
     return k;
   }
diff --git a/neuralstyletransferv1_amd/csrc/nst_api.cpp b/neuralstyletransferv1_amd/csrc/nst_api.cpp
--- a/neuralstyletransferv1_amd/csrc/nst_api.cpp
+++ b/neuralstyletransferv1_amd/csrc/nst_api.cpp
@@ -255,6 +255,8 @@
 struct nst_handle {
   int arch, dtype, device;
   int* range_flag = nullptr;
+  bool in_fold = true;
+  int cus = 256;
   std::vector<Layer> layers;
   std::vector<Op> prog;
   bool profiling = false;
@@ -609,6 +611,8 @@
   size_t off_buf[NBUF], off_partial, off_seg, off_stats, off_pre = 0;
   size_t pre_bytes = 0;
   size_t off_tail = 0, tail_bytes = 0;
+  std::vector<int> fold;
+  size_t off_fold = 0, fold_bytes = 0;
 };
 
 size_t align256(size_t v) { return (v + 255) / 256 * 256; }
@@ -710,6 +714,34 @@
       bw[op.dst] = bw[op.src];
     }
   }
+  P.fold.assign(nops, 0);
+  const size_t fold_region = align256((size_t)n * IN_FOLD_MAX_SLICES * 128 * 16);
+  for (size_t i = 0; h->in_fold && i + 1 < nops; ++i) {
+    const Op &a = h->prog[i], &c = h->prog[i + 1];
+    if (a.kind != OP_CONV || c.kind != OP_CONV || a.src == B_IMG || c.dst == B_OUT || c.in_norm != a.layer) continue;
+    const Layer &La = h->layers[a.layer], &Lc = h->layers[c.layer];
+    if (!La.k_main || !Lc.k_main || !La.k_main->in_fold || !Lc.k_main->in_fold || La.bn_tab || La.coutp != 128) continue;
+    if (La.d.axis_mode != AX_REFLECT || Lc.d.axis_mode != AX_REFLECT) continue;
+    bool sole = true;
+    for (size_t j = 0; j < nops; ++j) {
+      const Op& o = h->prog[j];
+      const bool reads = o.kind == OP_CONV ? ((j != i + 1 && o.in_norm == a.layer) || (o.res_buf >= 0 && o.r_norm == a.layer))
+                                           : (o.layer == a.layer || o.r_norm == a.layer);
+      if (reads) sole = false;
+    }
+    if (!sole) continue;
+    P.fold_bytes = 2 * fold_region;
+    int tx, ty;
+    tile_grid(*La.k_main, P.ih[i], P.iw[i], P.oh[i], P.ow[i], &tx, &ty);
+    int cx, cy;
+    tile_grid(*Lc.k_main, P.ih[i + 1], P.iw[i + 1], P.oh[i + 1], P.ow[i + 1], &cx, &cy);
+    const size_t fmaxb = std::max({(size_t)P.ih[i] * P.iw[i] * La.cinp * 2, (size_t)P.oh[i] * P.ow[i] * La.coutp * 2,
+                                   (size_t)P.oh[i + 1] * P.ow[i + 1] * Lc.coutp * 2});
+    const int maxfr = std::min(La.k_main->in_fold, Lc.k_main->in_fold);
+    if (tx * ty != cx * cy || (size_t)n * fmaxb > (size_t)0xFFFFFF00u || !in_fold_shape_ok(n, tx * ty, h->cus, maxfr)) continue;
+    P.fold[i] |= IN_FOLD_WALK | IN_FOLD_PROD;
+    P.fold[i + 1] |= IN_FOLD_WALK | IN_FOLD_CONS;
+  }
   size_t off = 0;
   for (int b = 0; b < NBUF; ++b) { P.off_buf[b] = off; off += align256(P.buf_bytes[b]); }
   P.off_partial = off;
@@ -721,6 +753,8 @@
   if (is_torch7(h->arch)) P.tail_bytes = (size_t)n * 3 * P.out_h * P.out_w * 4;
   P.off_tail = off;
   off += align256(P.tail_bytes);
+  P.off_fold = off;
+  off += P.fold_bytes;
   P.off_stats = off;
   for (const Layer& Ly : h->layers) off += align256((size_t)n * Ly.coutp * 8);
   P.ws_bytes = off;
@@ -919,6 +953,12 @@
   DeviceGuard guard(device);
   auto* h = new nst_handle();
   h->arch = arch; h->dtype = compute_dtype; h->device = device;
+  {
+    const char* env = std::getenv("NST_IN_FOLD");
+    h->in_fold = (flags & NST_KSEL_NO_IN_FOLD) == 0 && !(env != nullptr && env[0] == '0');
+    int c = 0;
+    if (hipDeviceGetAttribute(&c, hipDeviceAttributeMultiprocessorCount, device) == hipSuccess && c > 0) h->cus = c;
+  }
   std::vector<LayerDef> defs;
   const bool fuse_res = (flags & NST_KSEL_UNFUSED_RESIDUAL) == 0 && !is_torch7(arch);
   build_program(arch, fuse_res, fuse_res, defs, h->prog, split_blocks);
@@ -1374,6 +1414,18 @@
     }
     if (k->persistent && p.n_cblk != 1) { set_error("conv " + Ly.d.conv + ": persistent kernel needs one channel block"); return NST_E_SHAPE; }
     p.partial = final_out ? nullptr : partial;
+    const int infold = (k == Ly.k_main && !h->range_flag) ? P.fold[i] : 0;
+    if (infold) {
+      const size_t region = P.fold_bytes / 2;
+      p.fold = infold;
+      if (infold & IN_FOLD_PROD) p.fold_out = (double*)(ws + P.off_fold + (i & 1) * region);
+      if (infold & IN_FOLD_CONS) {
+        const Layer& Lp = h->layers[op.in_norm];
+        p.fold_in = (const double*)(ws + P.off_fold + ((i - 1) & 1) * region);
+        p.fold_gamma = Lp.gamma; p.fold_beta = Lp.beta; p.fold_eps = Lp.eps; p.fold_frn = Lp.frn;
+        p.fold_count = (double)P.ch[i - 1] * (double)P.cw[i - 1];
+      }
+    }
     dim3 grid(p.tiles_x * p.tiles_y, n * p.n_cblk);
     nst_handle::Rec rec{op.layer, nullptr, nullptr};
     if (h->profiling) {
@@ -1396,7 +1448,7 @@
     if (!final_out && Ly.bn_tab) {
       e = launch_norm_table_fill(Ly.bn_tab, n, Ly.coutp, tab(op.layer), st);
       if (e != hipSuccess) { set_error(std::string("norm table launch: ") + hipGetErrorString(e)); return NST_E_HIP; }
-    } else if (!final_out) {
+    } else if (!final_out && !(infold & IN_FOLD_PROD)) {
       e = launch_in_finalize(partial, n, p.tiles_x * p.tiles_y * k->part_rows, Ly.coutp, (double)p.hconv * (double)p.wconv,
                              Ly.gamma, Ly.beta, Ly.eps, Ly.frn, tab(op.layer), ws + P.off_seg, st);
       if (e == hipSuccess && h->range_flag)
@@ -1410,8 +1462,11 @@
       if (cap->res && cap->res[i] && op.res_out >= 0)
         NST_HIP_CHECK(hipMemcpyAsync(cap->res[i], bufs[op.res_out], (size_t)n * P.ih[i] * P.iw[i] * Ly.cinp * P.res_esz[i],
                                      hipMemcpyDeviceToDevice, st));
-      if (cap->stats && cap->stats[i])
+      if (cap->stats && cap->stats[i] && !(infold & IN_FOLD_PROD))
         NST_HIP_CHECK(hipMemcpyAsync(cap->stats[i], stats[op.layer], (size_t)n * Ly.coutp * 8, hipMemcpyDeviceToDevice, st));
+      if (cap->stats && (infold & IN_FOLD_CONS) && cap->stats[i - 1])
+        NST_HIP_CHECK(hipMemcpyAsync(cap->stats[i - 1], stats[op.in_norm], (size_t)n * h->layers[op.in_norm].coutp * 8,
+                                     hipMemcpyDeviceToDevice, st));
     }
     return NST_OK;
   };
@@ -1546,6 +1601,7 @@
   out->in_elem_bytes = P.in_esz[op_index];
   out->res_elem_bytes = P.res_esz[op_index];
   out->kernel_dtype = op.kind == OP_CONV ? Ly.kdt : h->dtype;
+  out->in_fold = h->range_flag ? 0 : P.fold[op_index];
   return NST_OK;
 }
 
diff --git a/neuralstyletransferv1_amd/csrc/nst_internal.h b/neuralstyletransferv1_amd/csrc/nst_internal.h
--- a/neuralstyletransferv1_amd/csrc/nst_internal.h
+++ b/neuralstyletransferv1_amd/csrc/nst_internal.h
@@ -90,7 +90,23 @@
   int dec_tanh;
   int seg_len;
   int ph_off[2];
+  int fold;
+  const double* fold_in;
+  double* fold_out;
+  const float* fold_gamma;
+  const float* fold_beta;
+  float fold_eps;
+  int fold_frn;
+  double fold_count;
 };
+enum InFold { IN_FOLD_WALK = 1, IN_FOLD_PROD = 2, IN_FOLD_CONS = 4 };
+constexpr int IN_FOLD_MAX_SLICES = 64;
+constexpr int IN_FOLD_MAX_TILES = 2048;
+__host__ __device__ inline int in_fold_slices(int ntile) { return ntile < IN_FOLD_MAX_SLICES ? ntile : IN_FOLD_MAX_SLICES; }
+inline bool in_fold_shape_ok(int n, int ntile, int cus, int max_frames) {
+  const int G = n * ntile < cus ? n * ntile : cus;
+  return n >= 2 && n <= max_frames && ntile <= IN_FOLD_MAX_TILES && G % n == 0 && n * in_fold_slices(ntile) >= G;
+}
 
 constexpr int NST_MAX_STREAM_SPLIT = 4;
 enum KernelDtype { NST_KDT_SW_O32 = 16, NST_KDT_SW_O16 = 17, NST_KDT_SPLIT_O32 = 18, NST_KDT_SPLIT_O16 = 19,
@@ -111,6 +127,7 @@
   int split_w;
   int cinp_k, bn_k;
   void (*launch)(const ConvParams&, dim3 grid, hipStream_t);
+  int in_fold;
 };
 
 const ConvKernelInfo* find_conv_kernel(int dtype, int mode, int ks, int stride, int cinp, int bn, int in_kind,
diff --git a/neuralstyletransferv1_amd/csrc/nst_ops.hip b/neuralstyletransferv1_amd/csrc/nst_ops.hip
--- a/neuralstyletransferv1_amd/csrc/nst_ops.hip
+++ b/neuralstyletransferv1_amd/csrc/nst_ops.hip
@@ -6,6 +6,7 @@
 #include "nst_hip.h"
 #include "post_common.h"
 #include "conv_impl.h"
+#include "conv_ws_common.h"
 
 namespace nst {
 
@@ -97,59 +98,45 @@
 }
 constexpr int IN_RED_CH = 16, IN_FIN_CH = 4;
 
-constexpr int IN_ONE_MAX_TILES = 2048;
+constexpr int IN_ONE_MAX_TILES = IN_FOLD_MAX_TILES;
 template <int CH>
-__global__ __launch_bounds__(1024) void in_stats_kernel(const float* __restrict__ partial, int tiles, int cstride,
-                                                        double count, const float* __restrict__ gamma,
-                                                        const float* __restrict__ beta, float eps, int frn,
-                                                        float2* __restrict__ out) {
-  constexpr int PH = 1024 / CH, NL = IN_ONE_MAX_TILES / PH;
-  __shared__ double red[16][CH][2];
+__global__ __launch_bounds__(128 * CH) void in_stats_kernel(const float* __restrict__ partial, int tiles, int cstride,
+                                                            double count, const float* __restrict__ gamma,
+                                                            const float* __restrict__ beta, float eps, int frn,
+                                                            float2* __restrict__ out) {
+  constexpr int NV = 2 * CH, UN = 8;
+  __shared__ double red[IN_FOLD_MAX_SLICES][NV];
   const int n = blockIdx.x;
-  const int cl = threadIdx.x & (CH - 1), q = threadIdx.x / CH;
-  const int c = min(blockIdx.y * CH + cl, cstride - 1);
-  const float2* p = (const float2*)partial + (size_t)n * tiles * cstride + c;
-  float2 v[NL];
-#pragma unroll
-  for (int k = 0; k < NL; ++k) v[k] = p[(size_t)min(q + k * PH, tiles - 1) * cstride];
-  double s1 = 0.0, s2 = 0.0;
-#pragma unroll
-  for (int k = 0; k < NL; ++k) {
-    const bool in = q + k * PH < tiles;
-    s1 += in ? (double)v[k].x : 0.0;
-    s2 += in ? (double)v[k].y : 0.0;
-  }
-#pragma unroll
-  for (int o = CH; o < 64; o <<= 1) {
-    s1 += __shfl_xor(s1, o);
-    s2 += __shfl_xor(s2, o);
-  }
-  const int wv = threadIdx.x >> 6;
-  if ((threadIdx.x & 63) < CH) {
-    red[wv][cl][0] = s1;
-    red[wv][cl][1] = s2;
-  }
+  const int j = threadIdx.x & (NV - 1), q = threadIdx.x / NV;
+  const int S = in_fold_slices(tiles);
+  const int c = min(blockIdx.y * CH + (j >> 1), cstride - 1);
+  const float* p = partial + ((size_t)n * tiles * cstride + c) * 2 + (j & 1);
+  double acc = 0.0;
+  if (q < S) {
+    for (int t0 = q; t0 < tiles; t0 += UN * S) {
+      float v[UN];
+#pragma unroll
+      for (int k = 0; k < UN; ++k) v[k] = p[(size_t)min(t0 + k * S, tiles - 1) * cstride * 2];
+#pragma unroll
+      for (int k = 0; k < UN; ++k)
+        if (t0 + k * S < tiles) acc = in_fold_add(acc, v[k]);
+    }
+  }
+  red[q][j] = acc;
   __syncthreads();
-  if (threadIdx.x >= CH || blockIdx.y * CH + cl >= cstride) return;
-  s1 = red[0][cl][0];
-  s2 = red[0][cl][1];
-  for (int w = 1; w < 16; ++w) {
-    s1 += red[w][cl][0];
-    s2 += red[w][cl][1];
-  }
-  const double mean = frn ? 0.0 : s1 / count;
-  double var = s2 / count - mean * mean;
-  var = var < 0.0 ? 0.0 : var;
-  const double rstd = 1.0 / sqrt(var + (double)eps);
-  const double scale = (double)gamma[c] * rstd;
-  out[(size_t)n * cstride + c] = make_float2((float)scale, (float)((double)beta[c] - mean * scale));
+  if (threadIdx.x >= NV) return;
+  double v[IN_FOLD_MAX_SLICES];
+#pragma unroll
+  for (int s = 0; s < IN_FOLD_MAX_SLICES; ++s) v[s] = red[s][j];
+  const float2 r = in_fold_table(v, S, (j & 1) != 0, count, gamma[c], beta[c], eps, frn);
+  if ((j & 1) == 0 && blockIdx.y * CH + (j >> 1) < cstride) out[(size_t)n * cstride + c] = r;
 }
 
 static int in_one_ch() {
   static const int v = [] {
     const char* e = std::getenv("NST_IN_ONE_CH");
     const int x = e ? std::atoi(e) : 4;
-    return (x == 2 || x == 8 || x == 16) ? x : 4;
+    return (x == 2 || x == 8) ? x : 4;
   }();
   return v;
 }
@@ -175,13 +162,11 @@
     const int ch = in_one_ch();
     const dim3 grid(n, (cstride + ch - 1) / ch);
     if (ch == 2)
-      hipLaunchKernelGGL(in_stats_kernel<2>, grid, dim3(1024), 0, st, partial, tiles, cstride, count, gamma, beta, eps, frn, out);
+      hipLaunchKernelGGL(in_stats_kernel<2>, grid, dim3(256), 0, st, partial, tiles, cstride, count, gamma, beta, eps, frn, out);
     else if (ch == 4)
-      hipLaunchKernelGGL(in_stats_kernel<4>, grid, dim3(1024), 0, st, partial, tiles, cstride, count, gamma, beta, eps, frn, out);
-    else if (ch == 8)
+      hipLaunchKernelGGL(in_stats_kernel<4>, grid, dim3(512), 0, st, partial, tiles, cstride, count, gamma, beta, eps, frn, out);
+    else
       hipLaunchKernelGGL(in_stats_kernel<8>, grid, dim3(1024), 0, st, partial, tiles, cstride, count, gamma, beta, eps, frn, out);
-    else
-      hipLaunchKernelGGL(in_stats_kernel<16>, grid, dim3(1024), 0, st, partial, tiles, cstride, count, gamma, beta, eps, frn, out);
     return hipGetLastError();
   }
   const int nseg = in_finalize_segments(tiles);
```

New measurement: 1540 frames/s. About the same (-0.7%).
